# Muennighoff/sgpt

Measured on AMD Instinct MI355X. Metric: encoded sentences/sec (SGPT-125M, seq_len 128, encode + weighted-mean pool + cosine top-10 chunk loop), higher is better.
Workload: dtype f16

## Files before the change

### __graft_entry__.py

```python
import os
import sys

ROOT = os.path.dirname(os.path.abspath(__file__))
if ROOT not in sys.path:
    sys.path.insert(0, ROOT)


def build() -> None:
    from sgpt_amd import build as b
    lib = b.build(force=os.environ.get("SGPT_FORCE_BUILD") == "1", verbose=True)
    assert os.path.exists(lib)
    import sgpt_amd
    from sgpt_amd import _lib
    _lib.load()
    print("built", lib)


def smoke() -> None:
    import numpy as np
    import torch
    assert torch.cuda.is_available(), "smoke() needs cuda:0"
    from oracle import sgpt_oracle as O
    from sgpt_amd import SGPTConfig, SGPTModel, get_context
    kw = dict(vocab_size=211, max_position_embeddings=96, hidden_size=128, num_layers=4, num_heads=2, window_size=8)
    cfg = O.NeoConfig(**kw)
    w = O.synth_weights(cfg, seed=11, std=0.08)
    rng = np.random.default_rng(0)
    seqs = [rng.integers(0, 211, size=int(n)).tolist() for n in (5, 33, 1, 40, 17, 16)]
    want = O.encode(w, cfg, seqs, mode="weightedmean", batch_size=len(seqs))
    for dtype, tol in (("fp32", 1e-3), ("f16", 6e-3), ("bf16", 3.5e-2), ("f16x3", 1e-4)):
        m = (SGPTModel(SGPTConfig(**kw), w, device="cuda:0", dtype="f16", precision="x3") if dtype == "f16x3"
             else SGPTModel(SGPTConfig(**kw), w, device="cuda:0", dtype=dtype))
        got = m.encode_ids(seqs, mode="weightedmean").cpu().numpy()
        err = float(np.abs(got - want).max())
        print(f"smoke encode[{dtype}]: max|emb - oracle| = {err:.3e} (tol {tol:g})")
        assert np.isfinite(got).all() and err < tol
        m.close()
    kw7 = dict(vocab_size=211, max_position_embeddings=96, hidden_size=768, num_layers=2, num_heads=12, window_size=8)
    cfg7 = O.NeoConfig(**kw7)
    w7 = O.synth_weights(cfg7, seed=12, std=0.03)
    m7 = SGPTModel(SGPTConfig(**kw7), w7, device="cuda:0", dtype="f16")
    for qs in ([rng.integers(0, 211, size=18).tolist()], [rng.integers(0, 211, size=int(n)).tolist() for n in (7, 30, 12)]):
        want7 = O.encode(w7, cfg7, qs, mode="weightedmean", batch_size=len(qs), normalize_embeddings=True)
        pb = m7.pack(qs)
        got7 = m7.encode_packed(pb, normalize=True)
        old_policy = m7.ctx.set_tile_policy(2)
        try:
            bulk7 = m7.encode_packed(pb, normalize=True)
        finally:
            m7.ctx.set_tile_policy(old_policy)
        err = float(np.abs(got7.cpu().numpy() - want7).max())
        print(f"smoke query path[f16, {len(qs)} quer{'y' if len(qs) == 1 else 'ies'}, {pb.T_pad} token rows]: max|emb - oracle| = {err:.3e} (tol 1e-3), "
              f"identical to the bulk kernels: {bool(torch.equal(got7, bulk7))}")
        assert pb.T_pad % 32 == 0 and pb.T_pad <= 64 and err < 1e-3 and torch.equal(got7, bulk7)
    m7.close()
    ctx = get_context("cuda:0")
    q = rng.standard_normal((5, 128)).astype(np.float32)
    c = rng.standard_normal((300, 128)).astype(np.float32)
    val, idx, n = ctx.score_topk(ctx.l2_normalize(torch.from_numpy(q)), ctx.l2_normalize(torch.from_numpy(c)), 4)
    ov, oi = O.topk_rows(O.cos_sim(q, c), 4)
    assert n == 4 and np.array_equal(idx.cpu().numpy(), oi) and np.abs(val.cpu().numpy() - ov).max() < 1e-5
    v16, i16, _ = ctx.score_topk(ctx.l2_normalize(torch.from_numpy(q)), ctx.l2_normalize(torch.from_numpy(c)), 4, dtype=torch.float16)
    assert np.abs(v16.cpu().numpy() - ov).max() < 1e-3
    print("smoke score_topk: ok (fp32 exact ids; f16 scores within 1e-3)")


if __name__ == "__main__":
    build()
    if "--smoke" in sys.argv:
        smoke()
```

### include/sgpt_hip.h

```cpp
#ifndef SGPT_HIP_H
#define SGPT_HIP_H

#include <stddef.h>
#include <stdint.h>

#ifdef __cplusplus
extern "C" {
#endif

#define SGPT_ABI_VERSION 19

typedef int sgpt_status;
#define SGPT_OK 0
#define SGPT_ERR_INVALID (-1)
#define SGPT_ERR_HIP (-2)
#define SGPT_ERR_MISSING (-3)
#define SGPT_ERR_OOM (-4)
#define SGPT_ERR_COMM (-6)
#define SGPT_ERR_RANGE (-5)

typedef struct sgpt_ctx sgpt_ctx;
typedef struct sgpt_model sgpt_model;

enum { SGPT_F32 = 0, SGPT_BF16 = 1, SGPT_FP8W = 2, SGPT_F16 = 3, SGPT_FP8M = 4 };
enum { SGPT_ARCH_GPTNEO = 0, SGPT_ARCH_GPTJ = 1, SGPT_ARCH_BLOOM = 2, SGPT_ARCH_BERT = 3, SGPT_ARCH_LLAMA = 4 };
enum { SGPT_POOL_WEIGHTEDMEAN = 0, SGPT_POOL_MEAN = 1, SGPT_POOL_LASTTOKEN = 2, SGPT_POOL_LEARNTMEAN = 3,
       SGPT_POOL_CLS = 4 };
enum { SGPT_COS = 0, SGPT_DOT = 1, SGPT_NEG_L2 = 2 };

typedef struct {
    int32_t arch;
    int32_t n_layers;
    int32_t d_model;
    int32_t n_heads;
    int32_t d_ffn;
    int32_t vocab;
    int32_t max_pos;
    int32_t window;
    float ln_eps;
    float attn_scale;
    int32_t compute_dtype;
    const uint8_t* layer_is_local;
    int32_t rotary_dim;
    int32_t qk_split;
    int32_t split_weights;
    int32_t n_kv_heads;
} sgpt_model_desc;

typedef struct {
    const char* name;
    const float* ptr;
    int64_t numel;
} sgpt_tensor_view;

int sgpt_abi_version(void);
sgpt_status sgpt_ctx_create(int hip_device, sgpt_ctx** out);
void sgpt_ctx_destroy(sgpt_ctx* ctx);
const char* sgpt_last_error(const sgpt_ctx* ctx);

sgpt_status sgpt_model_load(sgpt_ctx* ctx, const sgpt_model_desc* desc,
                            const sgpt_tensor_view* tensors, size_t n_tensors, sgpt_model** out);
void sgpt_model_free(sgpt_model* model);

sgpt_status sgpt_model_calibrate_begin(sgpt_model* model);
sgpt_status sgpt_model_calibrate_end(sgpt_model* model, float margin, float* scales_out);
sgpt_status sgpt_model_set_act_scales(sgpt_model* model, const float* scales, int32_t n_scales);

sgpt_status sgpt_encode(sgpt_model* model, const int32_t* ids, const int32_t* pos,
                        const int32_t* seq_off, const int32_t* seq_len, const int32_t* pad_left,
                        int32_t B, int32_t T_pad, int32_t max_alloc_len,
                        int32_t pool_mode, int32_t n_layers_run, int32_t apply_final_ln,
                        int32_t normalize, float* out, float* hidden_out, void* stream);

sgpt_status sgpt_encode_layers(sgpt_model* model, const int32_t* ids, const int32_t* pos,
                               const int32_t* seq_off, const int32_t* seq_len, const int32_t* pad_left,
                               int32_t B, int32_t T_pad, int32_t max_alloc_len, int32_t pool_mode,
                               int32_t normalize, float* out_layers, float* out_mean, void* stream);

sgpt_status sgpt_model_set_pool_weights(sgpt_model* model, const float* weights, int32_t n);

sgpt_status sgpt_lm_logprobs(sgpt_model* model, const float* hidden, const int32_t* row_idx, const int32_t* targets,
                             int32_t n, float* out_logprob, int32_t* out_greedy, void* stream);

sgpt_status sgpt_pool(sgpt_ctx* ctx, const void* hidden, int32_t hidden_dtype, const int32_t* mask,
                      int32_t B, int32_t S, int32_t d, int32_t pool_mode, float* out, void* stream);
sgpt_status sgpt_pool_learnt(sgpt_ctx* ctx, const void* hidden, int32_t hidden_dtype, const int32_t* mask,
                             int32_t B, int32_t S, int32_t d, const float* pos_weights, float* out, void* stream);

sgpt_status sgpt_l2_normalize(sgpt_ctx* ctx, const float* in, int64_t n, int32_t d,
                              void* out, int32_t out_dtype, void* stream);

sgpt_status sgpt_pairwise_scores(sgpt_ctx* ctx, const float* a, const float* b, int64_t n, int32_t d, int32_t cosine,
                                 float* out, void* stream);
// ... 82 lines not shown
#define SGPT_EVAL_MAX_CUTS 16
sgpt_status sgpt_eval_ranked(sgpt_ctx* ctx, const int64_t* idx, const float* val, int32_t nq, int32_t K,
                             const int32_t* qrel_off, const int64_t* qrel_pos, const int32_t* qrel_rel,
                             const int32_t* ideal_rel, const int32_t* k_values, int32_t nk, int32_t check_order,
                             int32_t* out_hits, int32_t* out_first, float* out_dcg, float* out_idcg, float* out_sp,
                             int32_t* out_R, void* stream);

#define SGPT_EVAL_MAX_GROUP 1024
sgpt_status sgpt_eval_groups(sgpt_ctx* ctx, const float* emb, int32_t n_rows, int32_t d, int32_t mode, const float* scores_in,
                             int32_t G, const int32_t* grp_off, int32_t n_cand, int32_t max_group, const int32_t* q_row,
                             const int32_t* cand_row, const int32_t* cand_rel, const int32_t* R_extra,
                             const int32_t* ideal_off, const int32_t* ideal_rel, int32_t n_ideal, float* out_scores,
                             int32_t* out_order, int32_t* out_hits1, int32_t* out_hits5, int32_t* out_first, int32_t* out_R, float* out_sp,
                             float* out_dcg, float* out_idcg, void* stream);

#define SGPT_EVAL_MAX_PAIRS (1 << 24)
sgpt_status sgpt_eval_pairs(sgpt_ctx* ctx, const float* score, const int32_t* label, int32_t n, int32_t check_nan,
                            int32_t* out_rank2, int64_t* out_n_pos, int64_t* out_n_used, double* out_ap_num, void* stream);

sgpt_status sgpt_linear(sgpt_ctx* ctx, int32_t dtype, int32_t epi, int32_t out_dtype, const void* A, const void* W,
                        const float* bias, const float* resid, void* out, int32_t M, int32_t N, int32_t K, void* stream);

sgpt_status sgpt_linear_query(sgpt_ctx* ctx, int32_t dtype, int32_t epi, const void* A, const float* x, const float* ln_gamma,
                              const float* ln_beta, float ln_eps, const void* W, const float* bias, const float* resid, void* out,
                              void* out_vt, int32_t n_split, int32_t M, int32_t N, int32_t K, void* stream);

sgpt_status sgpt_linear_qkv(sgpt_ctx* ctx, int32_t dtype, const void* A, const void* W, void* out, void* out_vt, int32_t n_split,
                            int32_t M, int32_t N, int32_t K, void* stream);

sgpt_status sgpt_attention(sgpt_ctx* ctx, int32_t dtype, const void* q, const void* k, const void* v, int64_t ldq, int64_t ldvt,
                           void* out, int64_t ldo, const int32_t* seq_off, int32_t B, int32_t T, int32_t H, int32_t dh,
                           int32_t window, float scale, const float* alibi, int32_t max_alloc_len, int32_t out_fp8,
                           float out_scale, int32_t* range_flag, int32_t x3, int64_t qk_lo_delta, int64_t v_lo_delta,
                           int64_t ctx_lo_delta, int64_t ctx_hi2_delta, void* stream);

sgpt_status sgpt_attention_ex(sgpt_ctx* ctx, int32_t dtype, const void* q, const void* k, const void* v, int64_t ldq, int64_t ldvt,
                              void* out, int64_t ldo, const int32_t* seq_off, int32_t B, int32_t T, int32_t H, int32_t dh,
                              int32_t window, float scale, const float* alibi, int32_t max_alloc_len, int32_t out_fp8,
                              float out_scale, int32_t* range_flag, int32_t x3, int64_t qk_lo_delta, int64_t v_lo_delta,
                              int64_t ctx_lo_delta, int64_t ctx_hi2_delta, int32_t causal, const int32_t* seq_len, void* stream);

sgpt_status sgpt_attention_gqa(sgpt_ctx* ctx, int32_t dtype, const void* q, const void* k, const void* v, int64_t ldq, int64_t ldvt,
                               void* out, int64_t ldo, const int32_t* seq_off, int32_t B, int32_t T, int32_t H, int32_t n_kv_heads,
                               int32_t dh, int32_t window, float scale, const float* alibi, int32_t max_alloc_len, int32_t out_fp8,
                               float out_scale, int32_t* range_flag, int32_t x3, int64_t qk_lo_delta, int64_t v_lo_delta,
                               int64_t ctx_lo_delta, int64_t ctx_hi2_delta, void* stream);

sgpt_status sgpt_embed(sgpt_ctx* ctx, const int32_t* ids, const int32_t* pos, const float* wte, const float* wpe, int32_t T,
                       int32_t d, int32_t vocab, int32_t max_pos, float* out, void* stream);
sgpt_status sgpt_layernorm(sgpt_ctx* ctx, const float* x, const float* gamma, const float* beta, int32_t T, int32_t d, float eps,
                           void* out, int32_t out_dtype, float out_mul, int32_t split, void* stream);
sgpt_status sgpt_layernorm_writeback(sgpt_ctx* ctx, float* x, const float* gamma, const float* beta, int32_t T, int32_t d, float eps,
                                     void* out16, int32_t out_dtype, void* stream);
sgpt_status sgpt_rmsnorm(sgpt_ctx* ctx, const float* x, const float* gamma, int32_t T, int32_t d, float eps, void* out, int32_t out_dtype,
                         void* stream);
sgpt_status sgpt_swiglu(sgpt_ctx* ctx, const void* gu, int32_t dtype, int32_t T, int32_t ffn, void* out, void* stream);
sgpt_status sgpt_rope_half(sgpt_ctx* ctx, void* buf, int32_t dtype, int64_t ld, int64_t k_off, const int32_t* pos, const float* sin_t,
                           const float* cos_t, int32_t T, int32_t H, int32_t H_kv, int32_t head_dim, int32_t max_pos, void* stream);
sgpt_status sgpt_qknorm_rope_half(sgpt_ctx* ctx, void* buf, int32_t dtype, int64_t ld, int64_t k_off, const int32_t* pos,
                                  const float* sin_t, const float* cos_t, int32_t T, int32_t H, int32_t H_kv, int32_t head_dim,
                                  int32_t max_pos, const float* q_gamma, const float* k_gamma, float eps, void* stream);
sgpt_status sgpt_lnf_pool_ex(sgpt_ctx* ctx, const float* x, const float* gamma, const float* beta, const int32_t* seq_off,
                             const int32_t* seq_len, const int32_t* pad_left, int32_t B, int32_t d, float eps, int32_t apply_ln,
                             int32_t mode, int32_t normalize, const float* pos_weights, int32_t n_weights, float* out,
                             int32_t* nonfinite_flag, int32_t norm_kind, void* stream);
sgpt_status sgpt_lnf_pool(sgpt_ctx* ctx, const float* x, const float* gamma, const float* beta, const int32_t* seq_off,
                          const int32_t* seq_len, const int32_t* pad_left, int32_t B, int32_t d, float eps, int32_t apply_ln,
                          int32_t mode, int32_t normalize, const float* pos_weights, int32_t n_weights, float* out,
                          int32_t* nonfinite_flag, void* stream);
sgpt_status sgpt_rope(sgpt_ctx* ctx, void* buf, int32_t dtype, int64_t ld, int64_t k_off, const int32_t* pos, const float* sin,
                      const float* cos, int32_t T, int32_t H, int32_t head_dim, int32_t rotary_dim, int32_t max_pos, void* stream);
sgpt_status sgpt_logprob_rows(sgpt_ctx* ctx, const float* logits, int64_t ld, int32_t V, const int32_t* targets, int32_t n,
                              float* out_logprob, int32_t* out_greedy, void* stream);

sgpt_status sgpt_layernorm_fp8(sgpt_ctx* ctx, const float* x, const float* gamma, const float* beta, int32_t T, int32_t d,
                               float eps, uint8_t* codes, float* row_scale, void* stream);
sgpt_status sgpt_linear_fp8(sgpt_ctx* ctx, int32_t epi, int32_t out_dtype, const uint8_t* A, const float* a_scale,
                            float a_scalar, const uint8_t* W, const float* w_scale, const float* bias, const float* resid,
                            void* out, float out_scale, int32_t M, int32_t N, int32_t K, void* stream);

sgpt_status sgpt_prof_enable(sgpt_ctx* ctx, int32_t on);
sgpt_status sgpt_prof_read(sgpt_ctx* ctx, int64_t* launches, double* ms, double* flops, int32_t reset);

int32_t sgpt_ctx_set_gemm_cu_cap(sgpt_ctx* ctx, int32_t n);
int32_t sgpt_ctx_set_low_latency(sgpt_ctx* ctx, int32_t on);
int32_t sgpt_ctx_set_tile_policy(sgpt_ctx* ctx, int32_t policy);
int32_t sgpt_ctx_set_query_tile(sgpt_ctx* ctx, int32_t k);

sgpt_status sgpt_bench_gemm(sgpt_ctx* ctx, int32_t dtype, int32_t epi, int32_t out_dtype,
                            int32_t M, int32_t N, int32_t K, int32_t iters, float* ms_out);

#ifdef __cplusplus
}
#endif
#endif
```

### sgpt_amd/_lib.py

```python
import ctypes as C
import os

HERE = os.path.dirname(os.path.abspath(__file__))
LIB_PATH = os.environ.get("SGPT_HIP_LIB") or os.path.join(HERE, "lib", "libsgpt_hip.so")

SGPT_F32, SGPT_BF16, SGPT_FP8W, SGPT_F16, SGPT_FP8M = 0, 1, 2, 3, 4
SGPT_ABI_VERSION = 19
SGPT_PREC_CLASSES = 5
PC_LN1, PC_ATT, PC_CTX, PC_LN2, PC_H = 0, 1, 2, 3, 4
SGPT_ERR_RANGE = -5
SGPT_ERR_COMM = -6
SGPT_COMM_ID_BYTES = 128
SGPT_EVAL_MAX_CUTS = 16
SGPT_EVAL_MAX_GROUP = 1024
SGPT_EVAL_MAX_PAIRS = 1 << 24
SGPT_COS, SGPT_DOT, SGPT_NEG_L2 = 0, 1, 2
SGPT_ARCH_GPTNEO, SGPT_ARCH_GPTJ, SGPT_ARCH_BLOOM, SGPT_ARCH_BERT, SGPT_ARCH_LLAMA = 0, 1, 2, 3, 4
POOL_MODES = {"weightedmean": 0, "mean": 1, "lasttoken": 2, "learntmean": 3, "cls": 4}
EPI_BIAS_GELU_ERF = 9


class ModelDesc(C.Structure):
    _fields_ = [("arch", C.c_int32), ("n_layers", C.c_int32), ("d_model", C.c_int32), ("n_heads", C.c_int32),
                ("d_ffn", C.c_int32), ("vocab", C.c_int32), ("max_pos", C.c_int32), ("window", C.c_int32),
                ("ln_eps", C.c_float), ("attn_scale", C.c_float), ("compute_dtype", C.c_int32),
                ("layer_is_local", C.POINTER(C.c_uint8)), ("rotary_dim", C.c_int32), ("qk_split", C.c_int32),
                ("split_weights", C.c_int32), ("n_kv_heads", C.c_int32)]


class TensorView(C.Structure):
    _fields_ = [("name", C.c_char_p), ("ptr", C.c_void_p), ("numel", C.c_int64)]


SIGNATURES = {
    "sgpt_abi_version": (C.c_int, []),
    "sgpt_ctx_create": (C.c_int, [C.c_int, C.POINTER(C.c_void_p)]),
    "sgpt_ctx_destroy": (None, [C.c_void_p]),
    "sgpt_last_error": (C.c_char_p, [C.c_void_p]),
    "sgpt_model_load": (C.c_int, [C.c_void_p, C.POINTER(ModelDesc), C.POINTER(TensorView), C.c_size_t,
                                  C.POINTER(C.c_void_p)]),
    "sgpt_model_free": (None, [C.c_void_p]),
    "sgpt_encode": (C.c_int, [C.c_void_p, C.c_void_p, C.c_void_p, C.c_void_p, C.c_void_p, C.c_void_p,
                              C.c_int32, C.c_int32, C.c_int32, C.c_int32, C.c_int32, C.c_int32, C.c_int32,
                              C.c_void_p, C.c_void_p, C.c_void_p]),
    "sgpt_encode_layers": (C.c_int, [C.c_void_p, C.c_void_p, C.c_void_p, C.c_void_p, C.c_void_p, C.c_void_p,
                                     C.c_int32, C.c_int32, C.c_int32, C.c_int32, C.c_int32, C.c_void_p, C.c_void_p,
                                     C.c_void_p]),
    "sgpt_model_set_pool_weights": (C.c_int, [C.c_void_p, C.c_void_p, C.c_int32]),
    "sgpt_pool_learnt": (C.c_int, [C.c_void_p, C.c_void_p, C.c_int32, C.c_void_p, C.c_int32, C.c_int32, C.c_int32,
                                   C.c_void_p, C.c_void_p, C.c_void_p]),
    "sgpt_fp8_quantize_rows": (C.c_int, [C.c_void_p, C.c_void_p, C.c_int64, C.c_int64, C.c_void_p, C.c_void_p,
                                         C.c_void_p]),
    "sgpt_fp8_dequantize_rows": (C.c_int, [C.c_void_p, C.c_void_p, C.c_void_p, C.c_int64, C.c_int64, C.c_void_p,
                                           C.c_int32, C.c_void_p]),
    "sgpt_lm_logprobs": (C.c_int, [C.c_void_p, C.c_void_p, C.c_void_p, C.c_void_p, C.c_int32, C.c_void_p, C.c_void_p,
                                   C.c_void_p]),
    "sgpt_pool": (C.c_int, [C.c_void_p, C.c_void_p, C.c_int32, C.c_void_p, C.c_int32, C.c_int32, C.c_int32,
                            C.c_int32, C.c_void_p, C.c_void_p]),
    "sgpt_l2_normalize": (C.c_int, [C.c_void_p, C.c_void_p, C.c_int64, C.c_int32, C.c_void_p, C.c_int32, C.c_void_p]),
    "sgpt_pairwise_scores": (C.c_int, [C.c_void_p, C.c_void_p, C.c_void_p, C.c_int64, C.c_int32, C.c_int32, C.c_void_p, C.c_void_p]),
    "sgpt_f32_to_bf16": (C.c_int, [C.c_void_p, C.c_void_p, C.c_int64, C.c_void_p, C.c_void_p]),
    "sgpt_f32_to_16": (C.c_int, [C.c_void_p, C.c_void_p, C.c_int64, C.c_void_p, C.c_int32, C.c_void_p]),
    "sgpt_range_check": (C.c_int, [C.c_void_p, C.POINTER(C.c_int32), C.c_int32, C.c_void_p]),
    "sgpt_ctx_generation": (C.c_uint64, [C.c_void_p]),
    "sgpt_ctx_reserve": (C.c_int, [C.c_void_p, C.c_size_t, C.c_size_t]),
    "sgpt_scores": (C.c_int, [C.c_void_p, C.c_void_p, C.c_void_p, C.c_int32, C.c_int64, C.c_int64, C.c_int32,
                              C.c_void_p, C.c_int64, C.c_void_p]),
    "sgpt_score_topk": (C.c_int, [C.c_void_p, C.c_void_p, C.c_void_p, C.c_int32, C.c_int32, C.c_int64, C.c_int32,
                                  C.c_int32, C.c_int64, C.c_void_p, C.c_void_p, C.c_int32, C.POINTER(C.c_int32),
                                  C.c_void_p]),
    "sgpt_score_topk_q8": (C.c_int, [C.c_void_p, C.c_void_p, C.c_void_p, C.c_void_p, C.c_int32, C.c_int64, C.c_int32,
                                     C.c_int32, C.c_int64, C.c_void_p, C.c_void_p, C.c_int32, C.POINTER(C.c_int32),
                                     C.c_void_p]),
    "sgpt_pack_sign_bits": (C.c_int, [C.c_void_p, C.c_void_p, C.c_int64, C.c_int32, C.c_void_p, C.c_void_p, C.c_int64, C.c_void_p]),
    "sgpt_score_topk_bits": (C.c_int, [C.c_void_p, C.c_void_p, C.c_void_p, C.c_int64, C.c_int32, C.c_int64, C.c_int32, C.c_int32,
                                       C.c_int32, C.c_int32, C.c_void_p, C.c_void_p, C.c_int64, C.c_void_p, C.c_void_p, C.c_int32,
                                       C.POINTER(C.c_int32), C.c_void_p]),
    "sgpt_score_overflow_count": (C.c_int, [C.c_void_p, C.POINTER(C.c_int32), C.POINTER(C.c_int32), C.c_void_p]),
    "sgpt_score_topk_refined": (C.c_int, [C.c_void_p, C.c_void_p, C.c_void_p, C.c_void_p, C.c_int32, C.c_int32, C.c_int64, C.c_int32,
                                           C.c_int32, C.c_int64, C.c_float, C.c_void_p, C.c_void_p, C.c_int32, C.c_void_p, C.c_void_p,
                                           C.c_void_p]),
    "sgpt_topk_merge": (C.c_int, [C.c_void_p, C.c_void_p, C.c_void_p, C.c_int32, C.c_int32, C.c_int32, C.c_void_p,
                                  C.c_void_p, C.c_void_p, C.c_void_p]),
    "sgpt_topk": (C.c_int, [C.c_void_p, C.c_void_p, C.c_int32, C.c_int64, C.c_int64, C.c_int32, C.c_int64,
                            C.c_void_p, C.c_void_p, C.c_void_p]),
    "sgpt_eval_ranked": (C.c_int, [C.c_void_p, C.c_void_p, C.c_void_p, C.c_int32, C.c_int32, C.c_void_p, C.c_void_p, C.c_void_p,
                                   C.c_void_p, C.POINTER(C.c_int32), C.c_int32, C.c_int32, C.c_void_p, C.c_void_p, C.c_void_p,
                                   C.c_void_p, C.c_void_p, C.c_void_p, C.c_void_p]),
    "sgpt_eval_groups": (C.c_int, [C.c_void_p, C.c_void_p, C.c_int32, C.c_int32, C.c_int32, C.c_void_p, C.c_int32, C.c_void_p, C.c_int32,
                                   C.c_int32, C.c_void_p, C.c_void_p, C.c_void_p, C.c_void_p, C.c_void_p, C.c_void_p, C.c_int32,
                                   C.c_void_p, C.c_void_p, C.c_void_p, C.c_void_p, C.c_void_p, C.c_void_p, C.c_void_p, C.c_void_p,
                                   C.c_void_p, C.c_void_p]),
    "sgpt_eval_pairs": (C.c_int, [C.c_void_p, C.c_void_p, C.c_void_p, C.c_int32, C.c_int32, C.c_void_p, C.c_void_p, C.c_void_p,
                                  C.c_void_p, C.c_void_p]),
    "sgpt_linear": (C.c_int, [C.c_void_p, C.c_int32, C.c_int32, C.c_int32, C.c_void_p, C.c_void_p, C.c_void_p, C.c_void_p,
                              C.c_void_p, C.c_int32, C.c_int32, C.c_int32, C.c_void_p]),
    "sgpt_linear_query": (C.c_int, [C.c_void_p, C.c_int32, C.c_int32, C.c_void_p, C.c_void_p, C.c_void_p, C.c_void_p, C.c_float, C.c_void_p,
                                    C.c_void_p, C.c_void_p, C.c_void_p, C.c_void_p, C.c_int32, C.c_int32, C.c_int32, C.c_int32, C.c_void_p]),
    "sgpt_linear_qkv": (C.c_int, [C.c_void_p, C.c_int32, C.c_void_p, C.c_void_p, C.c_void_p, C.c_void_p, C.c_int32, C.c_int32, C.c_int32,
                                  C.c_int32, C.c_void_p]),
    "sgpt_model_calibrate_begin": (C.c_int, [C.c_void_p]),
    "sgpt_model_calibrate_end": (C.c_int, [C.c_void_p, C.c_float, C.c_void_p]),
    "sgpt_model_set_act_scales": (C.c_int, [C.c_void_p, C.c_void_p, C.c_int32]),
    "sgpt_layernorm_fp8": (C.c_int, [C.c_void_p, C.c_void_p, C.c_void_p, C.c_void_p, C.c_int32, C.c_int32, C.c_float, C.c_void_p,
                                     C.c_void_p, C.c_void_p]),
    "sgpt_linear_fp8": (C.c_int, [C.c_void_p, C.c_int32, C.c_int32, C.c_void_p, C.c_void_p, C.c_float, C.c_void_p, C.c_void_p,
                                  C.c_void_p, C.c_void_p, C.c_void_p, C.c_float, C.c_int32, C.c_int32, C.c_int32, C.c_void_p]),
    "sgpt_comm_unique_id": (C.c_int, [C.c_void_p]),
    "sgpt_comm_init": (C.c_int, [C.c_void_p, C.c_void_p, C.c_int32, C.c_int32]),
    "sgpt_comm_destroy": (C.c_int, [C.c_void_p]),
    "sgpt_comm_world": (C.c_int32, [C.c_void_p]),
    "sgpt_comm_rank": (C.c_int32, [C.c_void_p]),
    "sgpt_allgather_rows": (C.c_int, [C.c_void_p, C.c_void_p, C.c_void_p, C.c_int64, C.c_void_p, C.c_void_p]),
    "sgpt_allgather_rows_padded": (C.c_int, [C.c_void_p, C.c_void_p, C.c_void_p, C.c_int64, C.c_void_p, C.c_void_p]),
    "sgpt_exchange_topk": (C.c_int, [C.c_void_p, C.c_void_p, C.c_void_p, C.c_int32, C.c_int32, C.c_int32, C.c_void_p,
                                     C.c_void_p, C.c_void_p, C.c_void_p]),
    "sgpt_fold_gathered_topk": (C.c_int, [C.c_void_p, C.c_void_p, C.c_void_p, C.c_int32, C.c_int32, C.c_int32, C.c_int32,
                                          C.c_void_p, C.c_void_p, C.c_void_p, C.c_void_p]),
    "sgpt_ctx_set_low_latency": (C.c_int32, [C.c_void_p, C.c_int32]),
    "sgpt_ctx_set_tile_policy": (C.c_int32, [C.c_void_p, C.c_int32]),
    "sgpt_ctx_set_gemm_cu_cap": (C.c_int32, [C.c_void_p, C.c_int32]),
    "sgpt_ctx_set_query_tile": (C.c_int32, [C.c_void_p, C.c_int32]),
    "sgpt_model_range_check": (C.c_int, [C.c_void_p, C.POINTER(C.c_int32), C.c_int32, C.c_void_p]),
    "sgpt_model_range_adapt": (C.c_int, [C.c_void_p, C.POINTER(C.c_int32), C.c_void_p]),
    "sgpt_model_get_range_shifts": (C.c_int, [C.c_void_p, C.c_void_p, C.c_int32]),
    "sgpt_model_set_range_shifts": (C.c_int, [C.c_void_p, C.c_void_p, C.c_int32]),
    "sgpt_model_set_precision": (C.c_int, [C.c_void_p, C.c_void_p, C.c_int32]),
    "sgpt_model_get_precision": (C.c_int, [C.c_void_p, C.c_void_p, C.c_int32]),
    "sgpt_model_release_split_weights": (C.c_int, [C.c_void_p, C.c_void_p]),
    "sgpt_model_precision_probe_begin": (C.c_int, [C.c_void_p]),
    "sgpt_model_precision_probe_end": (C.c_int, [C.c_void_p, C.c_void_p]),
    "sgpt_row_crest": (C.c_int, [C.c_void_p, C.c_void_p, C.c_int32, C.c_int64, C.c_int32, C.c_int64, C.POINTER(C.c_float), C.c_void_p]),
    "sgpt_split16": (C.c_int, [C.c_void_p, C.c_void_p, C.c_int64, C.c_int32, C.c_int32, C.c_void_p, C.c_int32, C.c_void_p]),
    "sgpt_linear_split": (C.c_int, [C.c_void_p, C.c_int32, C.c_int32, C.c_void_p, C.c_void_p, C.c_void_p, C.c_void_p,
                                    C.c_int64, C.c_int64, C.c_int64, C.c_int32, C.c_int32, C.c_int32, C.c_void_p]),
    "sgpt_attention": (C.c_int, [C.c_void_p, C.c_int32, C.c_void_p, C.c_void_p, C.c_void_p, C.c_int64, C.c_int64,
                                 C.c_void_p, C.c_int64, C.c_void_p, C.c_int32, C.c_int32, C.c_int32, C.c_int32,
                                 C.c_int32, C.c_float, C.c_void_p, C.c_int32, C.c_int32,
                                 C.c_float, C.c_void_p, C.c_int32, C.c_int64, C.c_int64,
                                 C.c_int64, C.c_int64, C.c_void_p]),
    "sgpt_attention_ex": (C.c_int, [C.c_void_p, C.c_int32, C.c_void_p, C.c_void_p, C.c_void_p, C.c_int64, C.c_int64,
                                    C.c_void_p, C.c_int64, C.c_void_p, C.c_int32, C.c_int32, C.c_int32, C.c_int32,
                                    C.c_int32, C.c_float, C.c_void_p, C.c_int32, C.c_int32,
                                    C.c_float, C.c_void_p, C.c_int32, C.c_int64, C.c_int64,
                                    C.c_int64, C.c_int64, C.c_int32, C.c_void_p, C.c_void_p]),
    "sgpt_attention_gqa": (C.c_int, [C.c_void_p, C.c_int32, C.c_void_p, C.c_void_p, C.c_void_p, C.c_int64, C.c_int64,
                                     C.c_void_p, C.c_int64, C.c_void_p, C.c_int32, C.c_int32, C.c_int32, C.c_int32, C.c_int32,
                                     C.c_int32, C.c_float, C.c_void_p, C.c_int32, C.c_int32,
                                     C.c_float, C.c_void_p, C.c_int32, C.c_int64, C.c_int64,
                                     C.c_int64, C.c_int64, C.c_void_p]),
    "sgpt_rmsnorm": (C.c_int, [C.c_void_p, C.c_void_p, C.c_void_p, C.c_int32, C.c_int32, C.c_float, C.c_void_p, C.c_int32, C.c_void_p]),
    "sgpt_swiglu": (C.c_int, [C.c_void_p, C.c_void_p, C.c_int32, C.c_int32, C.c_int32, C.c_void_p, C.c_void_p]),
    "sgpt_rope_half": (C.c_int, [C.c_void_p, C.c_void_p, C.c_int32, C.c_int64, C.c_int64, C.c_void_p, C.c_void_p, C.c_void_p,
                                 C.c_int32, C.c_int32, C.c_int32, C.c_int32, C.c_int32, C.c_void_p]),
    "sgpt_qknorm_rope_half": (C.c_int, [C.c_void_p, C.c_void_p, C.c_int32, C.c_int64, C.c_int64, C.c_void_p, C.c_void_p, C.c_void_p,
                                        C.c_int32, C.c_int32, C.c_int32, C.c_int32, C.c_int32, C.c_void_p, C.c_void_p, C.c_float,
                                        C.c_void_p]),
    "sgpt_lnf_pool_ex": (C.c_int, [C.c_void_p, C.c_void_p, C.c_void_p, C.c_void_p, C.c_void_p, C.c_void_p, C.c_void_p, C.c_int32,
                                   C.c_int32, C.c_float, C.c_int32, C.c_int32, C.c_int32, C.c_void_p, C.c_int32, C.c_void_p,
                                   C.c_void_p, C.c_int32, C.c_void_p]),
    "sgpt_layernorm_writeback": (C.c_int, [C.c_void_p, C.c_void_p, C.c_void_p, C.c_void_p, C.c_int32, C.c_int32, C.c_float, C.c_void_p,
                                           C.c_int32, C.c_void_p]),
    "sgpt_embed": (C.c_int, [C.c_void_p, C.c_void_p, C.c_void_p, C.c_void_p, C.c_void_p, C.c_int32, C.c_int32, C.c_int32, C.c_int32,
                             C.c_void_p, C.c_void_p]),
    "sgpt_layernorm": (C.c_int, [C.c_void_p, C.c_void_p, C.c_void_p, C.c_void_p, C.c_int32, C.c_int32, C.c_float, C.c_void_p,
                                 C.c_int32, C.c_float, C.c_int32, C.c_void_p]),
    "sgpt_lnf_pool": (C.c_int, [C.c_void_p, C.c_void_p, C.c_void_p, C.c_void_p, C.c_void_p, C.c_void_p, C.c_void_p, C.c_int32,
                                C.c_int32, C.c_float, C.c_int32, C.c_int32, C.c_int32, C.c_void_p, C.c_int32, C.c_void_p,
                                C.c_void_p, C.c_void_p]),
    "sgpt_rope": (C.c_int, [C.c_void_p, C.c_void_p, C.c_int32, C.c_int64, C.c_int64, C.c_void_p, C.c_void_p, C.c_void_p,
                            C.c_int32, C.c_int32, C.c_int32, C.c_int32, C.c_int32, C.c_void_p]),
    "sgpt_logprob_rows": (C.c_int, [C.c_void_p, C.c_void_p, C.c_int64, C.c_int32, C.c_void_p, C.c_int32, C.c_void_p, C.c_void_p,
                                    C.c_void_p]),
    "sgpt_bench_gemm": (C.c_int, [C.c_void_p, C.c_int32, C.c_int32, C.c_int32, C.c_int32, C.c_int32, C.c_int32,
                                  C.c_int32, C.POINTER(C.c_float)]),
    "sgpt_prof_enable": (C.c_int, [C.c_void_p, C.c_int32]),
    "sgpt_prof_read": (C.c_int, [C.c_void_p, C.POINTER(C.c_int64), C.POINTER(C.c_double), C.POINTER(C.c_double),
                                 C.c_int32]),
}

_lib = None


class SgptHipError(RuntimeError):
    pass


class SgptRangeError(SgptHipError):
    """dtype='f16': a weight is outside the IEEE-half range, or an activation class is beyond every power-of-two range
    shift (use dtype='bf16'); dtype='fp8mfma': an e4m3 code saturated (re-calibrate)."""

EXPERIMENT_SIGNATURES = {
    "sgpt_exp_set_gemm_skew": (C.c_int32, [C.c_int32]),
    "sgpt_exp_set_gemm_w": (C.c_int32, [C.c_int32]),
}


def load():
    global _lib
    if _lib is not None:
        return _lib
    if not os.path.exists(LIB_PATH):
        raise SgptHipError(f"{LIB_PATH} is missing: build it with `python -m sgpt_amd.build` "
                           "(hipcc --offload-arch=gfx950); there is no CPU/PyTorch fallback")
    lib = C.CDLL(LIB_PATH)
# ... 26 lines not shown
```

### sgpt_amd/beir.py

```python
import logging
import os
import pathlib
import pickle
from concurrent.futures import ThreadPoolExecutor
from typing import Dict, List, Optional, Tuple, Union

import numpy as np
import torch

from .model import SGPTModel
from .runtime import get_context
from .families import family_of
from .tokenization import TextPipeline, load_tokenizer

logger = logging.getLogger(__name__)

SCORE_SPLIT_CREST = 10.0
SINGLE_LAYER_METHODS = ("mean", "weightedmean", "lasttoken", "cls")
ALL_LAYER_METHODS = {"meanmean": "mean", "lasttokenmean": "lasttoken"}


class CustomEmbedder:

    def __init__(self, model_name="EleutherAI/gpt-neo-1.3B", batch_size=250, device="cuda:0", save_emb=False,
# ... 17 lines not shown
        self.base_path = f"embeddings/{model_name.split('/')[-1]}/{self.method}/{dataset}"
        if save_emb:
            pathlib.Path(self.base_path).parent.mkdir(parents=True, exist_ok=True)

    def tokenize(self, sentences: List[str], is_query: bool) -> List[List[int]]:
        before = (self.pipe.docs_truncated, self.pipe.toks_truncated)
        seqs = self.pipe.batch(sentences, is_query)
        if self.pipe.docs_truncated > before[0]:
            logging.warning(f"Truncated {self.pipe.docs_truncated - before[0]} out of {len(sentences)} documents "
                            f"by {self.pipe.toks_truncated - before[1]} tokens.")
        return seqs

    def tokenize_corpus(self, corpus) -> List[List[int]]:
        return self.tokenize([t for (_, t) in self._corpus_texts(corpus)], False)

    def embed_device(self, sentences: List[str], is_query: bool, normalize: bool = False) -> torch.Tensor:
        return self.embed_ids_device(self.tokenize(sentences, is_query), normalize=normalize)

    def embed_ids_device(self, seqs: List[List[int]], normalize: bool = False) -> torch.Tensor:
        L = self.model.cfg.num_layers
        if abs(self.layeridx) > L + 1:
            raise ValueError(f"Layer Idx {self.layeridx} is larger than the {L + 1} hidden states")
        if self.method in SINGLE_LAYER_METHODS:
            return self.model.encode_ids(seqs, mode=self.method, normalize=normalize, layer_idx=self.layeridx)
        acc = self.model.encode_ids_all_layers(seqs, mode=ALL_LAYER_METHODS[self.method])
        return get_context(self.model.device).l2_normalize(acc) if normalize else acc

    def embed_batcher(self, texts: List[Tuple[int, str]], is_query, out_name=None, **kwargs) -> Dict:
        ids, sentences = zip(*texts)
        emb = self.embed_device(list(sentences), is_query).cpu().numpy()
        all_embeddings = {i: e for i, e in zip(ids, emb)}
        assert len(texts) == len(all_embeddings)
        if self.save_emb:
            pickle.dump(all_embeddings, open(out_name, "wb"))
        return all_embeddings

    def encode_queries(self, queries: List[Tuple[str, str]], batch_size: int = None, **kwargs) -> np.ndarray:
        path = f"{self.base_path}_queries.pickle"
        if os.path.exists(path):
            embeddings = pickle.load(open(path, "rb"))
        else:
            embeddings = self.embed_batcher(texts=queries, out_name=path, is_query=True, **kwargs)
        embeddings = np.array([embeddings[i] for (i, _) in queries])
        logger.info(f"Produced embeddings of shape {embeddings.shape}")
        return embeddings

    @staticmethod
    def _corpus_texts(corpus):
        return [(i, (d["title"] + " " + d["text"]).strip() if "title" in d else d["text"].strip()) for (i, d) in corpus]

    def encode_corpus(self, corpus: List[Tuple[str, Dict[str, str]]], batch_size: int = None, batch_num="",
                      **kwargs) -> np.ndarray:
        path = f"{self.base_path}_corpus{batch_num}.pickle"
        if os.path.exists(path):
            embeddings = pickle.load(open(path, "rb"))
        else:
            embeddings = self.embed_batcher(texts=self._corpus_texts(corpus), out_name=path, is_query=False, **kwargs)
        embeddings = np.array([embeddings[i] for (i, _) in corpus])
        logger.info(f"Produced embeddings of shape {embeddings.shape}")
        return embeddings

    def encode_queries_device(self, queries, normalize=False, use_cache=True):
        if use_cache and (os.path.exists(f"{self.base_path}_queries.pickle") or self.save_emb):
            emb = torch.from_numpy(self.encode_queries(queries)).to(self.model.device)
            return get_context(self.model.device).l2_normalize(emb) if normalize else emb
        return self.embed_device([q for (_, q) in queries], True, normalize=normalize)

    def uses_embedding_cache(self, batch_num="") -> bool:
        return os.path.exists(f"{self.base_path}_corpus{batch_num}.pickle") or self.save_emb

    def encode_corpus_device(self, corpus, batch_num="", normalize=False, seqs=None):
        if self.uses_embedding_cache(batch_num):
            emb = torch.from_numpy(self.encode_corpus(corpus, batch_num=batch_num)).to(self.model.device)
            return get_context(self.model.device).l2_normalize(emb) if normalize else emb
        if seqs is None:
            seqs = self.tokenize_corpus(corpus)
        return self.embed_ids_device(seqs, normalize=normalize)


class DenseRetrievalExactSearch:

    def __init__(self, model, batch_size: int = 128, corpus_chunk_size: int = 50000, score_dtype=torch.float32,
                 prefetch_tokenize: bool = True, ctx=None, group=None, distributed: Optional[bool] = None,
                 score_split: Optional[bool] = None, exact_scorer: str = "brute", **kwargs):
        self.model = model
        self.prefetch_tokenize = prefetch_tokenize
        self.batch_size = batch_size
        self.score_function_desc = {"cos_sim": "Cosine Similarity", "dot": "Dot Product"}
        self.corpus_chunk_size = corpus_chunk_size
        self.show_progress_bar = True
        self.convert_to_tensor = True
        self.score_dtype = score_dtype
        if exact_scorer not in ("refined", "brute"):
            raise ValueError("exact_scorer must be 'refined' or 'brute'")
        self.exact_scorer = exact_scorer
        self.ctx = ctx
        self.group = group
        self.distributed = distributed
        self.score_split = score_split
        self.last_score_split = False
        self.results = {}
        self.last_shard = None

    def _to_dev(self, ctx, x):
        if not isinstance(x, torch.Tensor):
            x = torch.as_tensor(np.asarray(x))
        return x.to(device=ctx.device, dtype=torch.float32)

    def _encode_queries(self, ctx, qlist, use_cache=True):
        if not qlist:
            return None
        if hasattr(self.model, "encode_queries_device"):
            q_emb = self.model.encode_queries_device(qlist, use_cache=use_cache)
        else:
            q_emb = self.model.encode_queries(qlist, batch_size=self.batch_size,
                                              show_progress_bar=self.show_progress_bar,
                                              convert_to_tensor=self.convert_to_tensor)
        return self._to_dev(ctx, q_emb)

    def search(self, corpus: Dict[str, Dict[str, str]], queries: Dict[str, str], top_k: int, score_function: str,
               return_sorted: bool = False, **kwargs) -> Dict[str, Dict[str, float]]:
        self.results = {qid: {} for qid in queries}
        ranked = self.search_ranked(corpus, queries, top_k, score_function, **kwargs)
        if ranked.val.shape[1] > 0:
            self.results = assemble_results(ranked.query_ids, ranked.corpus_ids, ranked.val.cpu().numpy(), ranked.idx.cpu().numpy())
        return self.results

    def search_ranked(self, corpus: Dict[str, Dict[str, str]], queries: Dict[str, str], top_k: int, score_function: str,
                      **kwargs):
        if score_function not in self.score_function_desc:
            raise ValueError(
                "score function: {} must be either (cos_sim) for cosine similarity or (dot) for dot product".format(
                    score_function))
        from .dist import balanced_cuts, get_comm, is_distributed
        ctx = self.ctx if self.ctx is not None else get_context(getattr(getattr(self.model, "model", None), "device", None))
        import torch.distributed as tdist
        sharded = is_distributed(self.group) if self.distributed is None else (
            bool(self.distributed) and tdist.is_available() and tdist.is_initialized())
        comm = get_comm(ctx, self.group) if sharded else None
        world, rank = (comm.world, comm.rank) if comm is not None else (1, 0)

        logger.info("Encoding Queries...")
        query_ids = list(queries.keys())
        nq = len(query_ids)
        qlist = [(qid, queries[qid]) for qid in queries]
        sgpt = getattr(self.model, "model", None)
        if comm is not None and hasattr(sgpt, "sync_precision") and hasattr(self.model, "tokenize") and qlist:
            from .dist import max_reducer
            own = qlist[rank::world][:64] or qlist[:64]
            sgpt.sync_precision(self.model.tokenize([q for (_, q) in own], True), max_reducer(ctx, self.group))
        if getattr(sgpt, "precision_report", None):
            rep = sgpt.precision_report
            logger.info("Encoder precision: %s (%s; %d operand classes flagged)", rep["decided"], rep["probed"], rep["flagged"])
        if comm is not None and (nq >= 4 * world or world == 1):
            qcuts = balanced_cuts([len(q[1]) + 1 for q in qlist], world, min_one=True)
            q_loc = self._encode_queries(ctx, qlist[qcuts[rank]: qcuts[rank + 1]], use_cache=False)
            q_emb = comm.all_gather_rows(q_loc, np.diff(qcuts).tolist())
        else:
            q_emb = self._encode_queries(ctx, qlist)
        if score_function == "cos_sim":
            q_emb = ctx.l2_normalize(q_emb)
        split = False
        if self.score_dtype in (torch.float16, torch.bfloat16) and score_function == "cos_sim" and hasattr(ctx, "split16"):
            split = (ctx.row_crest(q_emb) > SCORE_SPLIT_CREST) if self.score_split is None else bool(self.score_split)
        self.last_score_split = split
        q_op = ctx.split16(q_emb, "query", self.score_dtype) if split else q_emb

        logger.info("Sorting Corpus by document length (Longest first)...")
        doc_len = {k: len(corpus[k].get("title", "") + corpus[k].get("text", "")) for k in corpus}
        corpus_ids = sorted(corpus, key=doc_len.__getitem__, reverse=True)
        pos_of = {cid: i for i, cid in enumerate(corpus_ids)}
        self_idx = torch.tensor([pos_of.get(qid, -1) for qid in query_ids], dtype=torch.int64, device=ctx.device)
        if comm is not None:
            ccuts = balanced_cuts([doc_len[c] + 1 for c in corpus_ids], world)
            lo, hi = int(ccuts[rank]), int(ccuts[rank + 1])
        else:
            lo, hi = 0, len(corpus_ids)
        self.last_shard = (rank, world, lo, hi)
        clist = [(cid, corpus[cid]) for cid in corpus_ids[lo:hi]]

        run_val = run_idx = None
        itr = range(0, len(clist), self.corpus_chunk_size)
        ahead = self.prefetch_tokenize and hasattr(self.model, "tokenize_corpus")
        pool = ThreadPoolExecutor(max_workers=1) if ahead else None
        fut = None
        tag = (lambda b: b) if comm is None else (lambda b: f"_r{rank}of{world}_{b}")

        def tokens_for(batch_num, start):
            if not ahead or self.model.uses_embedding_cache(tag(batch_num)) or start >= len(clist):
                return None
            return pool.submit(self.model.tokenize_corpus, clist[start: start + self.corpus_chunk_size])
        try:
            fut = tokens_for(0, 0)
            for batch_num, start in enumerate(itr):
                logger.info("Encoding Batch {}/{}...".format(batch_num + 1, len(itr)))
                end = min(start + self.corpus_chunk_size, len(clist))
                if ahead:
                    seqs = fut.result() if fut is not None else None
                    fut = tokens_for(batch_num + 1, end)
                    sub = self.model.encode_corpus_device(clist[start:end], batch_num=tag(batch_num), seqs=seqs)
                elif hasattr(self.model, "encode_corpus_device"):
                    sub = self.model.encode_corpus_device(clist[start:end], batch_num=tag(batch_num))
                else:
                    sub = self.model.encode_corpus(clist[start:end], batch_size=self.batch_size,
                                                   show_progress_bar=self.show_progress_bar,
                                                   convert_to_tensor=self.convert_to_tensor, batch_num=tag(batch_num))
                sub = self._to_dev(ctx, sub)
                kk = min(top_k + 1, end - start)
                refined = (self.score_dtype == torch.float32 and self.exact_scorer == "refined" and score_function == "cos_sim"
                           and hasattr(ctx, "score_topk_refined") and sub.shape[1] % 8 == 0)
                if score_function == "cos_sim":
                    sub = (ctx.split16(ctx.l2_normalize(sub), "doc", self.score_dtype) if split
                           else ctx.l2_normalize(sub, out_dtype=self.score_dtype))
                if refined:
                    val, idx, _ = ctx.score_topk_refined(q_op, sub, None, kk, idx_base=lo + start)
                else:
                    val, idx, _ = ctx.score_topk(q_op, sub, kk, idx_base=lo + start, dtype=self.score_dtype)
                if run_val is None:
                    cand_v, cand_i = val, idx
                else:
                    cand_v, cand_i = torch.cat([run_val, val], dim=1), torch.cat([run_idx, idx], dim=1)
                keep = min(top_k + 1, cand_v.shape[1])
                run_val, run_idx = ctx.topk_merge(cand_v, cand_i, keep, exclude_idx=self_idx)
        finally:
            if pool is not None:
                if fut is not None:
                    fut.cancel()
                pool.shutdown(wait=True)

        if comm is not None:
            k1 = top_k + 1
            pv = torch.full((nq, k1), float("-inf"), dtype=torch.float32, device=ctx.device)
            pi = torch.full((nq, k1), -1, dtype=torch.int64, device=ctx.device)
            if run_val is not None:
                pv[:, : run_val.shape[1]] = run_val
                pi[:, : run_idx.shape[1]] = run_idx
            run_val, run_idx = comm.exchange_topk(pv, pi, min(k1, len(corpus_ids)), exclude_idx=self_idx)
        if run_val is None:
            run_val = torch.empty((nq, 0), dtype=torch.float32, device=ctx.device)
            run_idx = torch.empty((nq, 0), dtype=torch.int64, device=ctx.device)
        from .evaluation import RankedLists
        return RankedLists(query_ids, corpus_ids, run_val, run_idx, pos_of)


def _host_ext():
    global _HOST_EXT
    if _HOST_EXT is None:
        _HOST_EXT = False
        path = os.path.join(os.path.dirname(os.path.abspath(__file__)), "lib", "_sgpt_host.so")
        if os.path.exists(path):
            import importlib.util
            try:
                spec = importlib.util.spec_from_file_location("_sgpt_host", path)
                mod = importlib.util.module_from_spec(spec)
                spec.loader.exec_module(mod)
                _HOST_EXT = mod
            except Exception as e:
                logger.warning("host extension %s not loadable (%s): result dicts are assembled in Python", path, e)
    return _HOST_EXT or None


_HOST_EXT = None


def assemble_results(query_ids, corpus_ids, vals: np.ndarray, idxs: np.ndarray, native: Optional[bool] = None) -> Dict[str, Dict[str, float]]:
    ext = _host_ext() if native in (None, True) else None
    if native is True and ext is None:
        raise RuntimeError("assemble_results(native=True): sgpt_amd/lib/_sgpt_host.so is not built (python -m sgpt_amd.build)")
    if ext is not None and len(query_ids) > 0:
        qs = query_ids if isinstance(query_ids, list) else list(query_ids)
        cs = corpus_ids if isinstance(corpus_ids, list) else list(corpus_ids)
        return ext.assemble(qs, cs, np.ascontiguousarray(vals, dtype=np.float32), np.ascontiguousarray(idxs, dtype=np.int64))
    cid = np.asarray(corpus_ids, dtype=object)
    ok_all = idxs >= 0
    full = bool(ok_all.all())
    out = {}
    for qi, qid in enumerate(query_ids):
        if full:
            out[qid] = dict(zip(cid[idxs[qi]].tolist(), vals[qi].tolist()))
        else:
            ok = ok_all[qi]
            out[qid] = dict(zip(cid[idxs[qi][ok]].tolist(), vals[qi][ok].tolist()))
    return out


class SentenceBERTBOSEOS:

    def __init__(self, model_path=None, sep: str = " ", speca=False, specb=False, model: Optional[SGPTModel] = None,
                 tokenizer=None, max_seq_length: int = 300, method: str = "weightedmean", dtype="f16",
                 device="cuda:0", frame=None, **kwargs):
        self.sep = sep
        self.speca, self.specb = speca, specb
        if not (specb or speca):
            raise NameError("name 'sentences' is not defined")
        self.model = model if model is not None else SGPTModel.from_pretrained(model_path, device=device, dtype=dtype)
        tok = tokenizer if tokenizer is not None else load_tokenizer(model_path)
        self.pipe = TextPipeline(tok, max_seq_length, specb=specb and not speca, speca=speca, st_path=True,
                                 family=family_of(self.model), frame=frame)
        if speca and max(self.pipe.bos_q + self.pipe.eos_q + self.pipe.bos_d + self.pipe.eos_d) >= self.model.cfg.vocab_size:
            raise ValueError("speca: the checkpoint's embedding table has no rows for the added [SOS]/[EOS]/{SOS}/{EOS} ids")
# ... 54 lines not shown
```

### sgpt_amd/csrc/common.h

```cpp
#pragma once
#include <hip/hip_runtime.h>
#include <stdint.h>

typedef uint16_t bf16_t;
struct f16_t { uint16_t bits; };
typedef __attribute__((ext_vector_type(8))) __bf16 bf16x8;
typedef __attribute__((ext_vector_type(8))) _Float16 f16x8;
typedef __attribute__((ext_vector_type(4))) float f32x4;
typedef __attribute__((ext_vector_type(16))) float f32x16;

constexpr int DT_F32 = 0, DT_BF16 = 1, DT_FP8W = 2, DT_F16 = 3;
__host__ __device__ constexpr bool dt_is16(int dt) { return dt == DT_BF16 || dt == DT_F16; }

#define WAVE 64

typedef uint2 __attribute__((may_alias)) uint2_a;
typedef uint4 __attribute__((may_alias)) uint4_a;
typedef float4 __attribute__((may_alias)) float4_a;

__device__ __forceinline__ float bf16_to_f32(bf16_t v) { return __uint_as_float(((uint32_t)v) << 16); }

typedef __attribute__((ext_vector_type(2))) __bf16 bf16x2_t;
typedef __attribute__((ext_vector_type(2))) float f32x2_t;
__device__ __forceinline__ uint32_t pack_bf16x2(float lo, float hi) {
// ... 252 lines not shown
bool score64q8_shape_ok(int M, long N, int K, const void* codes, long ldw);
void launch_score64q8(int epi, const Score8Args& a, hipStream_t s);
void launch_scorebits(int epi, const GemmArgs& g, int d, int qw, long ldb, hipStream_t s, bool spread = false);
void launch_gemm256w(int dtype, int epi, const GemmArgs& a, hipStream_t s, bool deep_a);

struct AttnArgs {
    const void* q;
    const void* k;
    const void* v;
    void* ctx;
    const int* seq_off;
    int B, H, dh;
    long ldq, ldvt, ldo;
    int window;
    float scale;
    int max_alloc_len;
    const float* alibi;
    int dtype;
    int out_fp8;
    float out_scale;
    int* range_flag;
    int x3;
    long qk_lo_delta, v_lo_delta, ctx_lo_delta, ctx_hi2_delta;
    int noncausal;
    const int* seq_len;
    int kv_group = 1;
};
inline bool attn_x3_supported(int dh) { return dh == 64 || dh == 128; }
void launch_attn_bf16(const AttnArgs& a, hipStream_t s);
void launch_attn_f32(const AttnArgs& a, hipStream_t s);

void launch_embed(const int* ids, const int* pos, const float* wte, const float* wpe, float* x, int T, int d, int vocab,
                  int max_pos, hipStream_t s);
void launch_layernorm(const float* x, const float* g, const float* b, void* out, int out_dtype, int T, int d,
                      float eps, hipStream_t s, float out_mul = 1.0f);
void launch_layernorm_writeback(float* x, const float* g, const float* b, void* out16, int out_dtype, int T, int d, float eps,
                                int* range_flag, hipStream_t s);
void launch_layernorm_split(const float* x, const float* g, const float* b, void* out, int out_dtype, int T, int d,
                            float eps, hipStream_t s, float out_mul);
void launch_rmsnorm(const float* x, const float* g, void* out, int out_dtype, int T, int d, float eps, int* range_flag, hipStream_t s);
void launch_swiglu(const void* gu, void* h, int dtype, int T, int ffn, int* range_flag, hipStream_t s);
void launch_pack_split_rows(const float* src, long rows, long cols, void* dst, int out_dtype, hipStream_t s);
void launch_crest16(const void* in, int T, int cols, long ld, int dtype, unsigned* out_bits, hipStream_t s);
void launch_split16_rows(const float* in, long n, int d, int layout, void* out, int out_dtype, hipStream_t s);
void launch_layernorm_q8(const float* x, const float* g, const float* b, void* q, float* scale, void* out16, int out16_dtype,
                         int T, int d, float eps, hipStream_t s);
void launch_absmax16(const void* in, long numel, int dtype, unsigned* out_bits, hipStream_t s);
void launch_lnf_pool(const float* x, const float* g, const float* b, const int* seq_off, const int* seq_len,
                     const int* pad_left, int B, int d, float eps, int apply_ln, int mode, int normalize,
                     const float* pos_weights, int pos_weights_n, float* out, hipStream_t s,
                     int* nonfinite_flag = nullptr,
                     int norm_kind = 0);
void launch_pool(const void* hidden, int dtype, const int* mask, int B, int S, int d, int mode,
                 const float* pos_weights, float* out, hipStream_t s);
void launch_fp8_quant_rows(const float* w, long rows, long cols, void* q, float* scale, hipStream_t s);
void launch_fp8_dequant_rows(const void* q, const float* scale, long rows, long cols, void* out, int out_dtype,
                             hipStream_t s);
void launch_l2norm(const float* in, long n, int d, void* out, int out_dtype, hipStream_t s);
void launch_pack_sign_bits(const float* x, long n, int d, const float* center, uint8_t* bits, long ldb, hipStream_t s);
void launch_pairwise(const float* a, const float* b, long n, int d, bool cosine, float* out, hipStream_t s);
void launch_gather_rows(const float* src, const int* row_idx, int n, int d, float* dst, hipStream_t s);
void launch_logprob_rows(const float* logits, long ld, int V, const int* targets, int n, float* out_lp, int* out_arg,
                         hipStream_t s);
void launch_mean_over_axis0(const float* in, int n0, long n, float* out, hipStream_t s);
void launch_f32_to_bf16(const float* in, long numel, void* out, hipStream_t s);
void launch_f32_to_16(const float* in, long numel, void* out, int out_dtype, hipStream_t s);
void launch_absmax(const float* in, long numel, unsigned* out_bits, hipStream_t s);
void launch_fill_f32(float* p, long n, float v, hipStream_t s);
void launch_rope(void* qk, int dtype, long ld, long k_off, const int* pos, const float* sin_t, const float* cos_t, int T,
                 int H, int dh, int rotary_dim, int max_pos, hipStream_t s);
void launch_rope_half(void* qk, int dtype, long ld, long k_off, const int* pos, const float* sin_t, const float* cos_t, int T,
                      int H, int H_kv, int dh, int max_pos, hipStream_t s);
void launch_qknorm_rope_half(void* qk, int dtype, long ld, long k_off, const int* pos, const float* sin_t, const float* cos_t,
                             const float* q_g, const float* k_g, float eps, int T, int H, int H_kv, int dh, int max_pos, int* range_flag,
                             hipStream_t s);
void launch_qkv_deinterleave(const float* src, float* dst, int H, int dh, long row_len, hipStream_t s);
void launch_fill_rand(void* p, long n, int dtype, unsigned seed, float scale, hipStream_t s);

void launch_topk_select(const float* scores, long ld, long n, long idx_base, const float* prev_val,
                        const int64_t* prev_idx, int n_prev, long prev_ld, int nq, int k, int nan_to_m1,
                        const int64_t* exclude_idx, float* out_val, int64_t* out_idx, hipStream_t s,
                        const int* pred = nullptr, float* thr_out = nullptr,
                        int gather_k = 0);
void launch_rescore(const float* q, const float* corpus, const int64_t* idx, long ld_idx, int nq, int m, int d, long idx_base,
                    long n_docs, float* out_val, int64_t* out_idx, long ld_out, hipStream_t s);
void launch_rescore_bits(int mode, const float* q, const uint8_t* bits, long ldb, const uint8_t* codes, long ld8, const float* scale,
                         const float* val1, const int64_t* idx, long ld_idx, int nq, int m, int d, long idx_base, long n_docs,
                         float* out_val, int64_t* out_idx, long ld_out, hipStream_t s);
void launch_refine_check(const float* v16, int k, int kp, float margin, int nq, int* flag, hipStream_t s);
void launch_list_append(const float* in_val, const int64_t* in_idx, long ld_in, int n_run, int nq, float* out_val, int64_t* out_idx,
                        long ld_out, int col0, hipStream_t s);
void launch_score_prep(const void* q, void* qpad, long q_bytes, long qpad_bytes, int* counters, long n_counters, long long* idx_list,
                       long n_idx, hipStream_t s);
void launch_thr_below(const float* list, int k, int nq, float* thr, hipStream_t s);
void launch_cand_merge(const float* run_val, const int64_t* run_idx, const float* cand_val, const int64_t* cand_idx,
                       int* cand_cnt, int cap, int nq, int k, float* out_val, int64_t* out_idx, int* overflow,
                       hipStream_t s, float* thr_io = nullptr);
```

### sgpt_amd/csrc/ctx.h

```cpp
#pragma once
#include <hip/hip_runtime.h>

#include <string>
#include <utility>
#include <vector>

struct sgpt_ctx {
    int device = 0;
    std::string err;
    void* ws = nullptr; size_t ws_bytes = 0;
    void* ws2 = nullptr; size_t ws2_bytes = 0;
    void* ws3 = nullptr; size_t ws3_bytes = 0;
    void* ws4 = nullptr; size_t ws4_bytes = 0;
    void* ws5 = nullptr; size_t ws5_bytes = 0;
    void* ws6 = nullptr; size_t ws6_bytes = 0;
    size_t filt_flag_off = 0; int filt_chunks = 0;
    void* comm = nullptr;
    int comm_rank = 0, comm_world = 0;
    uint64_t generation = 0;
    int* range_flag = nullptr;
    int kgroups = 1;
    int force256 = 0;
    int no_qpath = 0;
    int cu_cap = 0;
    int qtile = 0;
    bool prof = false;
    std::vector<std::pair<hipEvent_t, hipEvent_t>> ev_pool;
    size_t ev_used = 0;
    std::vector<double> ev_flops;
    int64_t prof_launches = 0; double prof_ms = 0, prof_flops = 0;
};
```

### sgpt_amd/csrc/ctx.hip

```cpp
#include "host.h"

namespace sgpt_host {

sgpt_status ensure(sgpt_ctx* c, void** p, size_t* have, size_t need) {
    if (*have >= need) return SGPT_OK;
    if (*p) { HIPC(c, hipDeviceSynchronize()); HIPC(c, hipFree(*p)); *p = nullptr; *have = 0; }
    need = align_up(need + (need >> 3), 1 << 20);
    if (hipMalloc(p, need) != hipSuccess) { *p = nullptr; return fail(c, SGPT_ERR_OOM, "hipMalloc workspace failed"); }
    HIPC(c, hipMemset(*p, 0, need));
    *have = need;
    c->generation++;
    return SGPT_OK;
}

void gemm(sgpt_ctx* c, int dtype, int epi, int out_dtype, const GemmArgs& a0, hipStream_t s) {
    Prof p(c, s, 2.0 * (double)a0.m_valid * a0.N * (a0.k_algo > 0 ? a0.k_algo : a0.K));
    GemmArgs a = a0;
    a.kgroups = c->kgroups; a.force256 = c->force256; a.cu_cap = c->cu_cap;
    launch_gemm(dtype, epi, out_dtype, a, s);
}

bool qgemm(sgpt_ctx* c, int dtype, int epi, int out_dtype, const QGemmArgs& a, hipStream_t s) {
    Prof p(c, s, 2.0 * (double)a.g.m_valid * a.g.N * a.g.K);
    return launch_qgemm(dtype, epi, out_dtype, a, s);
}

}

extern "C" {

int sgpt_abi_version(void) { return SGPT_ABI_VERSION; }

sgpt_status sgpt_ctx_create(int hip_device, sgpt_ctx** out) {
    if (!out) return SGPT_ERR_INVALID;
    *out = nullptr;
    int n = 0;
    if (hipGetDeviceCount(&n) != hipSuccess || hip_device < 0 || hip_device >= n) return SGPT_ERR_HIP;
    if (hipSetDevice(hip_device) != hipSuccess) return SGPT_ERR_HIP;
    sgpt_ctx* c = new sgpt_ctx();
    c->device = hip_device;
    if (hipMalloc((void**)&c->range_flag, 256) != hipSuccess || hipMemset(c->range_flag, 0, 256) != hipSuccess) {
        delete c;
        return SGPT_ERR_OOM;
    }
    *out = c;
    return SGPT_OK;
}

void sgpt_ctx_destroy(sgpt_ctx* c) {
    if (!c) return;
    (void)hipSetDevice(c->device);
    (void)hipDeviceSynchronize();
    if (c->ws) (void)hipFree(c->ws);
    if (c->ws2) (void)hipFree(c->ws2);
    (void)sgpt_comm_destroy(c);
    if (c->ws3) (void)hipFree(c->ws3);
    if (c->ws4) (void)hipFree(c->ws4);
    if (c->ws5) (void)hipFree(c->ws5);
    if (c->ws6) (void)hipFree(c->ws6);
    if (c->range_flag) (void)hipFree(c->range_flag);
    for (auto& e : c->ev_pool) { (void)hipEventDestroy(e.first); (void)hipEventDestroy(e.second); }
    delete c;
}

const char* sgpt_last_error(const sgpt_ctx* c) { return c ? c->err.c_str() : "null ctx"; }

uint64_t sgpt_ctx_generation(const sgpt_ctx* c) { return c ? c->generation : 0; }

sgpt_status sgpt_ctx_reserve(sgpt_ctx* c, size_t encode_bytes, size_t score_bytes) {
    if (!c) return SGPT_ERR_INVALID;
    HIPC(c, hipSetDevice(c->device));
    sgpt_status st = ensure(c, &c->ws, &c->ws_bytes, encode_bytes);
    if (st != SGPT_OK) return st;
    return ensure(c, &c->ws2, &c->ws2_bytes, score_bytes);
}

sgpt_status sgpt_range_check(sgpt_ctx* c, int32_t* flagged, int32_t reset, void* stream) {
    if (!c || !flagged) return SGPT_ERR_INVALID;
    HIPC(c, hipSetDevice(c->device));
    hipStream_t s = (hipStream_t)stream;
    int h = 0;
    HIPC(c, hipMemcpyAsync(&h, c->range_flag, sizeof(int), hipMemcpyDeviceToHost, s));
    HIPC(c, hipStreamSynchronize(s));
    if (reset && h) HIPC(c, hipMemsetAsync(c->range_flag, 0, sizeof(int), s));
    *flagged = h;
    return SGPT_OK;
}

sgpt_status sgpt_prof_enable(sgpt_ctx* c, int32_t on) {
    if (!c) return SGPT_ERR_INVALID;
    c->prof = on != 0;
    return SGPT_OK;
}

sgpt_status sgpt_prof_read(sgpt_ctx* c, int64_t* launches, double* ms, double* flops, int32_t reset) {
    if (!c) return SGPT_ERR_INVALID;
    HIPC(c, hipSetDevice(c->device));
    HIPC(c, hipDeviceSynchronize());
    for (size_t i = 0; i < c->ev_used; ++i) {
        float t = 0;
        HIPC(c, hipEventElapsedTime(&t, c->ev_pool[i].first, c->ev_pool[i].second));
        c->prof_ms += t;
        c->prof_flops += c->ev_flops[i];
        c->prof_launches++;
    }
    c->ev_used = 0;
    if (launches) *launches = c->prof_launches;
    if (ms) *ms = c->prof_ms;
    if (flops) *flops = c->prof_flops;
    if (reset) { c->prof_launches = 0; c->prof_ms = 0; c->prof_flops = 0; }
    return SGPT_OK;
}

int32_t sgpt_ctx_set_low_latency(sgpt_ctx* c, int32_t on) {
    if (!c) return 0;
    const int old = c->kgroups > 1 ? 1 : 0;
    c->kgroups = on ? 2 : 1;
    return old;
}
int32_t sgpt_ctx_set_gemm_cu_cap(sgpt_ctx* c, int32_t n) {
    if (!c) return 0;
    const int old = c->cu_cap;
    c->cu_cap = n > 0 ? n : 0;
    return old;
}
int32_t sgpt_ctx_set_tile_policy(sgpt_ctx* c, int32_t policy) {
    if (!c) return 0;
    const int old = c->force256 ? 1 : c->no_qpath ? 2 : 0;
    c->force256 = policy == 1 ? 1 : 0;
    c->no_qpath = policy == 2 ? 1 : 0;
    return old;
}
int32_t sgpt_ctx_set_query_tile(sgpt_ctx* c, int32_t k) {
    if (!c || k < 0 || k > 7) return -1;
    const int old = c->qtile;
    c->qtile = k;
    return old;
}
#ifdef SGPT_EXPERIMENTS
int32_t sgpt_exp_set_gemm_skew(int32_t cycles) { return set_gemm_skew(cycles); }
int32_t sgpt_exp_set_gemm_w(int32_t on) { return set_gemm_use_w(on); }
#endif

}
```

### sgpt_amd/csrc/elementwise.hip

```cpp
#include "common.h"
#include "rowln.h"


namespace {

__global__ __launch_bounds__(256) void embed_kernel(const int* __restrict__ ids, const int* __restrict__ pos,
                                                    const float* __restrict__ wte, const float* __restrict__ wpe,
                                                    float* __restrict__ x, int T, int d, int vocab, int max_pos) {
    const int row = blockIdx.x * 4 + (threadIdx.x >> 6);
    if (row >= T) return;
    const int lane = threadIdx.x & 63;
    int id = ids[row]; id = id < 0 ? 0 : (id >= vocab ? vocab - 1 : id);
    const float4* a = reinterpret_cast<const float4*>(wte + (long)id * d);
    float4* o = reinterpret_cast<float4*>(x + (long)row * d);
    if (wpe == nullptr) {
        for (int c = lane; c < d / 4; c += 64) o[c] = a[c];
        return;
    }
    int ps = pos[row]; ps = ps < 0 ? 0 : (ps >= max_pos ? max_pos - 1 : ps);
    const float4* b = reinterpret_cast<const float4*>(wpe + (long)ps * d);
    for (int c = lane; c < d / 4; c += 64) {
        const float4 u = a[c], v = b[c];
        o[c] = make_float4(u.x + v.x, u.y + v.y, u.z + v.z, u.w + v.w);
    }
// ... 492 lines not shown
__device__ __forceinline__ uint32_t e4m3fn_encode(float x) {
    const uint32_t sign = (__float_as_uint(x) >> 24) & 0x80u;
    const float a = fabsf(x);
    if (!(a < 464.f)) return sign | (a != a ? 0x7fu : 0x7eu);
    if (a < 0.015625f) return sign | (uint32_t)rintf(a * 512.f);
    uint32_t u = __float_as_uint(a);
    u += 0x7ffffu + ((u >> 20) & 1u);
    u >>= 20;
    const uint32_t code = u - (120u << 3);
    return sign | (code > 0x7eu ? 0x7eu : code);
}
__device__ __forceinline__ float e4m3fn_decode(uint32_t c) {
    const uint32_t e = (c >> 3) & 15u, m = c & 7u;
    const float a = e ? __uint_as_float(((e + 120u) << 23) | (m << 20)) : (float)m * 0.001953125f;
    if ((c & 0x7fu) == 0x7fu) return __uint_as_float(0x7fc00000u);
    return (c & 0x80u) ? -a : a;
}

__global__ __launch_bounds__(256) void fp8_quant_rows_kernel(const float* __restrict__ w, long rows, long cols,
                                                             uint8_t* __restrict__ q, float* __restrict__ scale) {
    const long row = (long)blockIdx.x * 4 + (threadIdx.x >> 6);
    if (row >= rows) return;
    const int lane = threadIdx.x & 63;
    const float* wr = w + row * cols;
    float amax = 0.f;
    for (long c = lane; c < cols; c += 64) amax = fmaxf(amax, fabsf(wr[c]));
#pragma unroll
    for (int off = 32; off > 0; off >>= 1) amax = fmaxf(amax, __shfl_xor(amax, off));
    float sc = 1.0f;
    if (amax > 0.f && amax < 3.0e38f) {
        const uint32_t u = __float_as_uint(amax);
        const int e = (int)((u >> 23) & 0xffu) - 127;
        const uint32_t frac = u & 0x7fffffu;
        int k = e - (frac > 0x600000u ? 7 : 8);
        k = k < -126 ? -126 : (k > 127 ? 127 : k);
        sc = __uint_as_float((uint32_t)(k + 127) << 23);
    }
    if (lane == 0) scale[row] = sc;
    const float inv = 1.0f / sc;
    for (long c = lane; c < cols; c += 64) q[row * cols + c] = (uint8_t)e4m3fn_encode(wr[c] * inv);
}

__global__ __launch_bounds__(256) void pack_sign_bits_kernel(const float* __restrict__ x, long n, int d, const float* __restrict__ center,
                                                             uint8_t* __restrict__ bits, long ldb) {
    const long total = n * ldb, stride = (long)gridDim.x * 256;
    for (long o = (long)blockIdx.x * 256 + threadIdx.x; o < total; o += stride) {
        const long r = o / ldb;
        const int i0 = (int)(o - r * ldb) * 8;
        const float* xr = x + r * d;
        uint32_t b = 0;
#pragma unroll
        for (int j = 0; j < 8; ++j) {
            const int i = i0 + j;
            if (i < d) {
                const float v = center ? xr[i] - center[i] : xr[i];
                const uint32_t u = __float_as_uint(v);
                b |= (u - 1u < 0x7f800000u ? 1u : 0u) << (7 - j);
            }
        }
        bits[o] = (uint8_t)b;
    }
}

template <typename OutT>
__global__ __launch_bounds__(256) void fp8_dequant_rows_kernel(const uint8_t* __restrict__ q, const float* __restrict__ scale,
                                                               long rows, long cols, OutT* __restrict__ out) {
    const long n4 = rows * cols / 4, stride = (long)gridDim.x * 256;
    for (long i = (long)blockIdx.x * 256 + threadIdx.x; i < n4; i += stride) {
        const uint32_t u = reinterpret_cast<const uint32_t*>(q)[i];
        const float sc = scale[i * 4 / cols];
        const float v0 = e4m3fn_decode(u & 0xffu) * sc, v1 = e4m3fn_decode((u >> 8) & 0xffu) * sc;
        const float v2 = e4m3fn_decode((u >> 16) & 0xffu) * sc, v3 = e4m3fn_decode(u >> 24) * sc;
        if constexpr (sizeof(OutT) == 4) reinterpret_cast<float4*>(out)[i] = make_float4(v0, v1, v2, v3);
        else reinterpret_cast<uint2*>(out)[i] = make_uint2(Half<OutT>::pack2(v0, v1), Half<OutT>::pack2(v2, v3));
    }
}

template <typename H>
__global__ __launch_bounds__(256) void cvt16_kernel(const float* __restrict__ in, long numel, uint16_t* __restrict__ out) {
    const long stride = (long)gridDim.x * 256;
    for (long i = (long)blockIdx.x * 256 + threadIdx.x; i < numel; i += stride) out[i] = f32_to_h<H>(in[i]);
}

__global__ __launch_bounds__(256) void absmax_kernel(const float* __restrict__ in, long numel, unsigned* __restrict__ out_bits) {
    const long stride = (long)gridDim.x * 256;
    unsigned m = 0;
    for (long i = (long)blockIdx.x * 256 + threadIdx.x; i < numel; i += stride) {
        const unsigned b = __float_as_uint(in[i]) & 0x7fffffffu;
        m = b > m ? b : m;
    }
#pragma unroll
    for (int o = 32; o > 0; o >>= 1) { const unsigned t = __shfl_xor(m, o, 64); m = t > m ? t : m; }
    if ((threadIdx.x & 63) == 0 && m) atomicMax(out_bits, m);
}

__global__ __launch_bounds__(256) void mean_axis0_kernel(const float* __restrict__ in, int n0, long n,
                                                         float* __restrict__ out) {
    const long i = (long)blockIdx.x * 256 + threadIdx.x;
    if (i >= n) return;
    float acc = 0.f;
    for (int j = 0; j < n0; ++j) acc += in[(long)j * n + i];
    out[i] = acc / (float)n0;
}

__global__ __launch_bounds__(256) void gather_rows_kernel(const float* __restrict__ src, const int* __restrict__ row_idx, int n,
                                                          int d, float* __restrict__ dst) {
    const int r = blockIdx.x * 4 + (threadIdx.x >> 6);
    if (r >= n) return;
    const int lane = threadIdx.x & 63;
    const float4* s4 = reinterpret_cast<const float4*>(src + (long)row_idx[r] * d);
    float4* d4 = reinterpret_cast<float4*>(dst + (long)r * d);
    for (int c = lane; c < d / 4; c += 64) d4[c] = s4[c];
}

__global__ __launch_bounds__(256) void logprob_rows_kernel(const float* __restrict__ logits, long ld, int V,
                                                           const int* __restrict__ targets, float* __restrict__ out_lp,
                                                           int* __restrict__ out_arg) {
    __shared__ float s_f[4];
    __shared__ int s_i[4];
    const int r = blockIdx.x, t = threadIdx.x, lane = t & 63, wave = t >> 6;
    const float* x = logits + (long)r * ld;
    float mx = -INFINITY;
    int am = 0x7fffffff;
    for (int i = t; i < V; i += 256) {
        const float v = x[i];
        if (v > mx || (v == mx && i < am)) { mx = v; am = i; }
    }
#pragma unroll
    for (int o = 32; o > 0; o >>= 1) {
        const float ov = __shfl_xor(mx, o, 64);
        const int oi = __shfl_xor(am, o, 64);
        if (ov > mx || (ov == mx && oi < am)) { mx = ov; am = oi; }
    }
    if (lane == 0) { s_f[wave] = mx; s_i[wave] = am; }
    __syncthreads();
    mx = s_f[0]; am = s_i[0];
#pragma unroll
    for (int w = 1; w < 4; ++w)
        if (s_f[w] > mx || (s_f[w] == mx && s_i[w] < am)) { mx = s_f[w]; am = s_i[w]; }
    __syncthreads();
    float sum = 0.f;
    for (int i = t; i < V; i += 256) sum += expf(x[i] - mx);
    sum = wave_sum(sum);
    if (lane == 0) s_f[wave] = sum;
    __syncthreads();
    if (t == 0) {
        const float tot = (s_f[0] + s_f[1]) + (s_f[2] + s_f[3]);
        int tg = targets[r]; tg = tg < 0 ? 0 : (tg >= V ? V - 1 : tg);
        out_lp[r] = (x[tg] - mx) - logf(tot);
        if (out_arg) out_arg[r] = am;
    }
}

__global__ __launch_bounds__(256) void fill_kernel(float* __restrict__ p, long n, float v) {
    const long stride = (long)gridDim.x * 256;
    for (long i = (long)blockIdx.x * 256 + threadIdx.x; i < n; i += stride) p[i] = v;
}

template <typename T>
__global__ __launch_bounds__(256) void fill_rand_kernel(T* __restrict__ p, long n, unsigned seed, float scale) {
    const long stride = (long)gridDim.x * 256;
    for (long i = (long)blockIdx.x * 256 + threadIdx.x; i < n; i += stride) {
        unsigned h = (unsigned)i * 2654435761u ^ seed;
        h ^= h >> 16; h *= 0x85ebca6bu; h ^= h >> 13; h *= 0xc2b2ae35u; h ^= h >> 16;
        const float v = ((float)(h >> 8) * (1.0f / 8388608.0f) - 1.0f) * scale;
        if constexpr (sizeof(T) == 4) p[i] = v; else reinterpret_cast<uint16_t*>(p)[i] = f32_to_h<T>(v);
// ... 182 lines not shown
#define LP_CASE(NV)                                                                                              \
    if (norm_kind == 1)                                                                                          \
        hipLaunchKernelGGL((lnf_pool_kernel<NV, true>), dim3(B), dim3(256), sm, s, x, g, b, seq_off, seq_len, pad_left, d, \
                           eps, apply_ln, mode, normalize, pos_weights, pos_weights_n, out, nonfinite_flag);     \
    else                                                                                                         \
    hipLaunchKernelGGL((lnf_pool_kernel<NV>), dim3(B), dim3(256), sm, s, x, g, b, seq_off, seq_len, pad_left, d, \
                       eps, apply_ln, mode, normalize, pos_weights, pos_weights_n, out, nonfinite_flag);
    const int nv = (d + 255) / 256;
    if (nv <= 1) { LP_CASE(1) } else if (nv <= 2) { LP_CASE(2) } else if (nv <= 3) { LP_CASE(3) }
    else if (nv <= 4) { LP_CASE(4) } else if (nv <= 8) { LP_CASE(8) } else if (nv <= 10) { LP_CASE(10) }
    else { LP_CASE(16) }
#undef LP_CASE
}

void launch_pool(const void* hidden, int dtype, const int* mask, int B, int S, int d, int mode,
                 const float* pos_weights, float* out, hipStream_t s) {
    dim3 grid(B, (d / 4 + 255) / 256);
    if (dtype == DT_BF16)
        hipLaunchKernelGGL(pool_kernel<bf16_t>, grid, dim3(256), 0, s, (const bf16_t*)hidden, mask, S, d, mode, pos_weights, out);
    else if (dtype == DT_F16)
        hipLaunchKernelGGL(pool_kernel<f16_t>, grid, dim3(256), 0, s, (const f16_t*)hidden, mask, S, d, mode, pos_weights, out);
    else
        hipLaunchKernelGGL(pool_kernel<float>, grid, dim3(256), 0, s, (const float*)hidden, mask, S, d, mode, pos_weights, out);
}

void launch_pack_sign_bits(const float* x, long n, int d, const float* center, uint8_t* bits, long ldb, hipStream_t s) {
    const long blocks = (n * ldb + 255) / 256;
    hipLaunchKernelGGL(pack_sign_bits_kernel, dim3((unsigned)(blocks < 1 ? 1 : (blocks > 65536 ? 65536 : blocks))), dim3(256), 0, s, x, n, d,
                       center, bits, ldb);
}

void launch_fp8_quant_rows(const float* w, long rows, long cols, void* q, float* scale, hipStream_t s) {
    hipLaunchKernelGGL(fp8_quant_rows_kernel, dim3((unsigned)((rows + 3) / 4)), dim3(256), 0, s, w, rows, cols,
                       (uint8_t*)q, scale);
}

void launch_fp8_dequant_rows(const void* q, const float* scale, long rows, long cols, void* out, int out_dtype,
                             hipStream_t s) {
    const int grid = cap_grid((rows * cols / 4 + 255) / 256);
    if (out_dtype == 1)
        hipLaunchKernelGGL(fp8_dequant_rows_kernel<bf16_t>, dim3(grid), dim3(256), 0, s, (const uint8_t*)q, scale, rows,
                           cols, (bf16_t*)out);
    else if (out_dtype == DT_F16)
        hipLaunchKernelGGL(fp8_dequant_rows_kernel<f16_t>, dim3(grid), dim3(256), 0, s, (const uint8_t*)q, scale, rows,
                           cols, (f16_t*)out);
    else
        hipLaunchKernelGGL(fp8_dequant_rows_kernel<float>, dim3(grid), dim3(256), 0, s, (const uint8_t*)q, scale, rows,
                           cols, (float*)out);
}

void launch_gather_rows(const float* src, const int* row_idx, int n, int d, float* dst, hipStream_t s) {
    hipLaunchKernelGGL(gather_rows_kernel, dim3((n + 3) / 4), dim3(256), 0, s, src, row_idx, n, d, dst);
}

void launch_logprob_rows(const float* logits, long ld, int V, const int* targets, int n, float* out_lp, int* out_arg,
                         hipStream_t s) {
    hipLaunchKernelGGL(logprob_rows_kernel, dim3(n), dim3(256), 0, s, logits, ld, V, targets, out_lp, out_arg);
}

void launch_mean_over_axis0(const float* in, int n0, long n, float* out, hipStream_t s) {
    hipLaunchKernelGGL(mean_axis0_kernel, dim3((unsigned)((n + 255) / 256)), dim3(256), 0, s, in, n0, n, out);
}

void launch_pairwise(const float* a, const float* b, long n, int d, bool cosine, float* out, hipStream_t s) {
    const unsigned grid = (unsigned)((n + 3) / 4);
    if (cosine) hipLaunchKernelGGL(pairwise_kernel<true>, dim3(grid), dim3(256), 0, s, a, b, n, d, out);
    else hipLaunchKernelGGL(pairwise_kernel<false>, dim3(grid), dim3(256), 0, s, a, b, n, d, out);
}

void launch_l2norm(const float* in, long n, int d, void* out, int out_dtype, hipStream_t s) {
    const int grid = (int)((n + 3) / 4);
    if (out_dtype == DT_BF16) hipLaunchKernelGGL(l2norm_kernel<bf16_t>, dim3(grid), dim3(256), 0, s, in, n, d, (bf16_t*)out);
    else if (out_dtype == DT_F16) hipLaunchKernelGGL(l2norm_kernel<f16_t>, dim3(grid), dim3(256), 0, s, in, n, d, (f16_t*)out);
    else hipLaunchKernelGGL(l2norm_kernel<float>, dim3(grid), dim3(256), 0, s, in, n, d, (float*)out);
}

void launch_f32_to_16(const float* in, long numel, void* out, int out_dtype, hipStream_t s) {
    const int grid = cap_grid((numel + 255) / 256);
    if (out_dtype == DT_F16) hipLaunchKernelGGL(cvt16_kernel<f16_t>, dim3(grid), dim3(256), 0, s, in, numel, (uint16_t*)out);
    else hipLaunchKernelGGL(cvt16_kernel<bf16_t>, dim3(grid), dim3(256), 0, s, in, numel, (uint16_t*)out);
}
void launch_f32_to_bf16(const float* in, long numel, void* out, hipStream_t s) { launch_f32_to_16(in, numel, out, DT_BF16, s); }

void launch_absmax(const float* in, long numel, unsigned* out_bits, hipStream_t s) {
    hipLaunchKernelGGL(absmax_kernel, dim3(cap_grid((numel + 255) / 256)), dim3(256), 0, s, in, numel, out_bits);
}

void launch_fill_f32(float* p, long n, float v, hipStream_t s) {
    hipLaunchKernelGGL(fill_kernel, dim3(cap_grid((n + 255) / 256)), dim3(256), 0, s, p, n, v);
}

void launch_fill_rand(void* p, long n, int dtype, unsigned seed, float scale, hipStream_t s) {
    if (dtype == DT_BF16)
        hipLaunchKernelGGL(fill_rand_kernel<bf16_t>, dim3(cap_grid((n + 255) / 256)), dim3(256), 0, s, (bf16_t*)p, n, seed, scale);
    else if (dtype == DT_F16)
        hipLaunchKernelGGL(fill_rand_kernel<f16_t>, dim3(cap_grid((n + 255) / 256)), dim3(256), 0, s, (f16_t*)p, n, seed, scale);
    else
        hipLaunchKernelGGL(fill_rand_kernel<float>, dim3(cap_grid((n + 255) / 256)), dim3(256), 0, s, (float*)p, n, seed, scale);
}

void launch_rope(void* qk, int dtype, long ld, long k_off, const int* pos, const float* sin_t, const float* cos_t, int T,
                 int H, int dh, int rotary_dim, int max_pos, hipStream_t s) {
    const int half = rotary_dim / 2;
    const long n = (long)T * H * half;
    const int grid = (int)((n + 255) / 256);
    if (dtype == DT_BF16)
        hipLaunchKernelGGL(rope_kernel<bf16_t>, dim3(grid), dim3(256), 0, s, (bf16_t*)qk, ld, k_off, pos, sin_t, cos_t, T, H, dh, half, max_pos);
    else if (dtype == DT_F16)
        hipLaunchKernelGGL(rope_kernel<f16_t>, dim3(grid), dim3(256), 0, s, (f16_t*)qk, ld, k_off, pos, sin_t, cos_t, T, H, dh, half, max_pos);
    else
        hipLaunchKernelGGL(rope_kernel<float>, dim3(grid), dim3(256), 0, s, (float*)qk, ld, k_off, pos, sin_t, cos_t, T, H, dh, half, max_pos);
}

void launch_rope_half(void* qk, int dtype, long ld, long k_off, const int* pos, const float* sin_t, const float* cos_t, int T,
                      int H, int H_kv, int dh, int max_pos, hipStream_t s) {
    const long n = (long)T * (H + H_kv) * (dh / 8);
    const int grid = (int)((n + 255) / 256);
    if (dtype == DT_BF16)
        hipLaunchKernelGGL(rope_half_kernel<bf16_t>, dim3(grid), dim3(256), 0, s, (bf16_t*)qk, ld, k_off, pos, sin_t, cos_t, T, H, H_kv, dh, max_pos);
    else if (dtype == DT_F16)
        hipLaunchKernelGGL(rope_half_kernel<f16_t>, dim3(grid), dim3(256), 0, s, (f16_t*)qk, ld, k_off, pos, sin_t, cos_t, T, H, H_kv, dh, max_pos);
    else
        hipLaunchKernelGGL(rope_half_kernel<float>, dim3(grid), dim3(256), 0, s, (float*)qk, ld, k_off, pos, sin_t, cos_t, T, H, H_kv, dh, max_pos);
}

void launch_qknorm_rope_half(void* qk, int dtype, long ld, long k_off, const int* pos, const float* sin_t, const float* cos_t,
                             const float* q_g, const float* k_g, float eps, int T, int H, int H_kv, int dh, int max_pos, int* range_flag,
                             hipStream_t s) {
    const long n = (long)T * (H + H_kv) * (dh / 8);
    const int grid = (int)((n + 255) / 256);
#define SGPT_QKNORM(TT, DH)                                                                                                          \
    hipLaunchKernelGGL((qknorm_rope_half_kernel<TT, DH>), dim3(grid), dim3(256), 0, s, (TT*)qk, ld, k_off, pos, sin_t, cos_t, q_g, k_g, \
                       eps, T, H, H_kv, max_pos, range_flag)
    if (dh != 64 && dh != 128) return;
    if (dtype == DT_BF16) { if (dh == 64) SGPT_QKNORM(bf16_t, 64); else SGPT_QKNORM(bf16_t, 128); }
    else if (dtype == DT_F16) { if (dh == 64) SGPT_QKNORM(f16_t, 64); else SGPT_QKNORM(f16_t, 128); }
    else { if (dh == 64) SGPT_QKNORM(float, 64); else SGPT_QKNORM(float, 128); }
#undef SGPT_QKNORM
}

void launch_qkv_deinterleave(const float* src, float* dst, int H, int dh, long row_len, hipStream_t s) {
    hipLaunchKernelGGL(qkv_deinterleave_kernel, dim3(3 * H * dh), dim3(256), 0, s, src, dst, H, dh, row_len);
}
```

### sgpt_amd/csrc/score.hip

```cpp
#include "host.h"
#include "score_plan.h"

extern "C" {

sgpt_status sgpt_l2_normalize(sgpt_ctx* c, const float* in, int64_t n, int32_t d, void* out, int32_t out_dtype,
                              void* stream) {
    if (!c || !in || !out || n <= 0 || d <= 0) return fail(c, SGPT_ERR_INVALID, "sgpt_l2_normalize: bad arguments");
    HIPC(c, hipSetDevice(c->device));
    launch_l2norm(in, n, d, out, out_dtype, (hipStream_t)stream);
    HIPC(c, hipGetLastError());
    return SGPT_OK;
}

sgpt_status sgpt_pairwise_scores(sgpt_ctx* c, const float* a, const float* b, int64_t n, int32_t d, int32_t cosine, float* out,
                                 void* stream) {
    if (!c || !a || !b || !out || n <= 0 || d <= 0) return fail(c, SGPT_ERR_INVALID, "sgpt_pairwise_scores: bad arguments");
    HIPC(c, hipSetDevice(c->device));
    launch_pairwise(a, b, n, d, cosine != 0, out, (hipStream_t)stream);
    HIPC(c, hipGetLastError());
    return SGPT_OK;
}

static sgpt_status check_score_dims(sgpt_ctx* c, int dtype, int d) {
    if (dtype != SGPT_F32 && dtype != SGPT_BF16 && dtype != SGPT_F16) return fail(c, SGPT_ERR_INVALID, "score: bad dtype");
// ... 63 lines not shown
    const void *q, *qpad;
    int nq, d, k; long idx_base;
    float* sc;
    float* tv[2]; int64_t* ti[2];
    float* sav_v; int64_t* sav_i;
};

static void score_tile(const ScoreRun& r, long c0, long nc, long ld, const int* pred, long row_stride = 1, bool sample = false) {
    GemmArgs g{};
    g.A = r.q; g.lda = r.d; g.M = r.nq; g.m_valid = r.nq; g.K = r.d; g.pred = pred;
    g.W = (const char*)r.cp.base + (size_t)c0 * r.cp.rowb; g.ldw = r.cp.ldw1 * row_stride; g.N = (int)nc;
    g.out = r.sc; g.ldo = ld;
    if (r.p.any_n) { corpus_gemm(r.c, r.cp, EPI_SCORE, g, c0, row_stride, sample, r.s); return; }
    const long na = r.p.fast ? nc / 256 * 256 : 0;
    const bool fold = r.p.tile_folds(na, nc, ld, row_stride, r.d);
    if (na > 0) {
        GemmArgs h = g;
        h.A = r.qpad; h.M = r.p.nq_pad; h.N = (int)(fold ? na + 256 : na); h.n_valid = fold ? (int)nc : 0;
        corpus_gemm(r.c, r.cp, EPI_SCORE, h, c0, row_stride, false, r.s);
    }
    if (na < nc && !fold) {
        g.W = (const char*)r.cp.base + (size_t)(c0 + na) * r.cp.rowb; g.N = (int)(nc - na); g.out = r.sc + na;
        corpus_gemm(r.c, r.cp, EPI_SCORE, g, c0 + na, 1, false, r.s);
    }
}

static sgpt_status classic(const ScoreRun& r, long lo, long hi, const float* pv, const int64_t* pi, int have, float* fin_v, int64_t* fin_i,
                           const int* pred) {
    sgpt_ctx* c = r.c;
    const long chunk = r.p.chunk;
    const int nq = r.nq, k = r.k;
    int cur = (pv == r.tv[0]) ? 1 : 0;
    for (long c0 = lo; c0 < hi; c0 += chunk) {
        const long nc = (hi - c0) < chunk ? (hi - c0) : chunk;
        score_tile(r, c0, nc, chunk, pred);
        const bool last = c0 + nc >= hi;
        if (last && pv == fin_v) {
            launch_topk_select(r.sc, chunk, nc, r.idx_base + c0, pv, pi, have, k, nq, k, 0, nullptr, r.tv[cur], r.ti[cur], r.s, pred);
            HIPC(c, hipMemcpyAsync(fin_v, r.tv[cur], (size_t)nq * k * 4, hipMemcpyDeviceToDevice, r.s));
            HIPC(c, hipMemcpyAsync(fin_i, r.ti[cur], (size_t)nq * k * 8, hipMemcpyDeviceToDevice, r.s));
        } else {
            launch_topk_select(r.sc, chunk, nc, r.idx_base + c0, pv, pi, have, k, nq, k, 0, nullptr,
                               last ? fin_v : r.tv[cur], last ? fin_i : r.ti[cur], r.s, pred);
        }
        pv = r.tv[cur]; pi = r.ti[cur];
        have = k;
        cur ^= 1;
    }
    return SGPT_OK;
}

static void recompute(const ScoreRun& r, long lo, long hi, const float* pv, const int64_t* pi, float* fin_v, int64_t* fin_i, const int* pred) {
    const long fchunk = r.p.fchunk;
    const long P = (hi - lo + fchunk - 1) / fchunk;
    for (long pc = 0; pc < P; ++pc) {
        const long c0 = lo + pc * fchunk, nc = (hi - c0) < fchunk ? (hi - c0) : fchunk;
        const bool to_fin = (P - 1 - pc) % 2 == 0;
        float* dv = to_fin ? fin_v : r.sav_v;
        int64_t* di = to_fin ? fin_i : r.sav_i;
        score_tile(r, c0, nc, fchunk, pred);
        launch_topk_select(r.sc, fchunk, nc, r.idx_base + c0, pv, pi, r.k, r.k, r.nq, r.k, 0, nullptr, dv, di, r.s, pred);
        pv = dv; pi = di;
    }
}

static inline int32_t list_fill(int32_t n_run, int64_t N, int32_t k) { const int64_t tot = (int64_t)n_run + N; return (int32_t)(tot < k ? tot : k); }

#ifndef SGPT_SAMPLE_MULT
#define SGPT_SAMPLE_MULT 1.0
#endif
#ifndef SGPT_FOLD_TAIL_SCORE
#define SGPT_FOLD_TAIL_SCORE 1
#endif
#ifndef SGPT_FOLD_TAIL
#define SGPT_FOLD_TAIL 1
#endif
#ifndef SGPT_SAMPLE_TOP2
#define SGPT_SAMPLE_TOP2 1
#endif
#ifndef SGPT_CAP_SHORT
#define SGPT_CAP_SHORT 512
#endif

static sgpt_status score_topk_impl(sgpt_ctx* c, const void* q, const Corpus& cp, int32_t nq, int64_t N, int32_t k, int64_t idx_base,
                                   const float* in_val, const int64_t* in_idx, float* run_val, int64_t* run_idx, int32_t n_run,
                                   int32_t* n_out, void* stream, const int* pred_all) {
    const int d = cp.d;
    if (!c || !q || !cp.base || !run_val || !run_idx || nq <= 0 || N <= 0 || k <= 0 || n_run < 0 || n_run > k)
        return fail(c, SGPT_ERR_INVALID, "sgpt_score_topk: bad arguments");
    sgpt_status st = cp.kind == SCORE_CORPUS_BITS ? SGPT_OK : check_score_dims(c, cp.dtype, d);
    if (st != SGPT_OK) return st;
    if (cp.kind == SCORE_CORPUS_BITS && (nq > 64 || d <= 0)) return fail(c, SGPT_ERR_INVALID, "score (binary corpus): at most 64 queries per pass");
    if (cp.kind == SCORE_CORPUS_FP8 && !(nq <= 64 && score64q8_shape_ok(64, 256, d, cp.base, d)))
        return fail(c, SGPT_ERR_INVALID, "score (fp8 corpus): shape not served by the streaming tile");
    HIPC(c, hipSetDevice(c->device));
    hipStream_t s = (hipStream_t)stream;
    static const ScoreSwitches sw{exp_env("SGPT_SCORE_NO64") != nullptr, exp_env("SGPT_SCORE_CLASSIC") != nullptr, exp_env("SGPT_GEMM128") != nullptr,
                                  SGPT_SAMPLE_MULT, SGPT_FOLD_TAIL != 0, SGPT_FOLD_TAIL_SCORE != 0, SGPT_SAMPLE_TOP2 != 0, SGPT_CAP_SHORT};
    ScorePlan p;
    plan_score_topk(ScorePlanIn{nq, (long)N, d, k, n_run, cp.kind, pred_all != nullptr, sw}, p);

    st = ensure(c, &c->ws2, &c->ws2_bytes, p.total);
    if (st != SGPT_OK) return st;
    if (cp.ws6_bytes) {
        st = ensure(c, &c->ws6, &c->ws6_bytes, cp.ws6_bytes);
        if (st != SGPT_OK) return st;
    }
    char* base = (char*)c->ws2;
    auto at = [&](const ScorePlan::Region& r) { return r.bytes ? base + r.off : nullptr; };
    void* qpad = p.pad_queries ? at(p.qpad) : (p.fast ? const_cast<void*>(q) : nullptr);
    const ScoreRun r{c, s, p, cp, q, qpad, nq, d, k, (long)idx_base, (float*)at(p.sc), {(float*)at(p.tv[0]), (float*)at(p.tv[1])},
                     {(int64_t*)at(p.ti[0]), (int64_t*)at(p.ti[1])}, (float*)at(p.sav_v), (int64_t*)at(p.sav_i)};
    float* const* tv = r.tv; int64_t* const* ti = r.ti;
    float* cand_v = (float*)at(p.cand_v);
    long long* cand_i = (long long*)at(p.cand_i);
    int* cand_cnt = (int*)at(p.cand_cnt);
    int* flag = p.filt ? cand_cnt + p.nq_pad : nullptr;
    float* th_v = (float*)at(p.th_v); int64_t* th_i = (int64_t*)at(p.th_i);
    float* thr_dense = (float*)at(p.thr);
    const int nq_pad = p.nq_pad;
    const long n_clear = p.filt ? (long)(nq_pad + p.n_flags) : 0;
    if (p.fast && (!p.pad_queries || (d % 8 == 0 && ((size_t)q & 15) == 0))) {
        launch_score_prep(q, qpad, p.pad_queries ? (long)nq * d * 2 : 0, p.pad_queries ? (long)nq_pad * d * 2 : 0, cand_cnt, n_clear,
                          p.fresh_list ? (long long*)ti[0] : nullptr, p.fresh_list ? (long)nq * k : 0, s);
    } else {
        if (p.pad_queries) {
            if (nq_pad > nq) HIPC(c, hipMemsetAsync((char*)qpad + (size_t)nq * d * 2, 0, (size_t)(nq_pad - nq) * d * 2, s));
            HIPC(c, hipMemcpyAsync(qpad, q, (size_t)nq * d * 2, hipMemcpyDeviceToDevice, s));
        }
        if (p.filt) HIPC(c, hipMemsetAsync(cand_cnt, 0, (size_t)n_clear * 4, s));
        if (p.fresh_list) HIPC(c, hipMemsetAsync(ti[0], 0xff, (size_t)nq * k * 8, s));
    }

    const float* bv = n_run > 0 ? in_val : nullptr;
    const int64_t* bi = n_run > 0 ? in_idx : nullptr;
    int have = n_run;
    c->filt_chunks = 0;
    if (p.filt) {
        static const bool no_fallback = exp_env("SGPT_SCORE_NOFALLBACK") != nullptr;
        int cur = 0, chunk_i = 0;
        if (p.sampled) {
            if (n_run > 0) {
                launch_topk_select(in_val, k, 0, 0, in_val, in_idx, n_run, k, nq, k, 0, nullptr, tv[0], ti[0], s);
            }
            if (p.sample_top2) {
                const long ld2 = 8 * (p.S / 256);
                GemmArgs h{};
                h.A = qpad; h.lda = d; h.M = nq_pad; h.m_valid = nq; h.K = d;
                h.W = cp.base; h.ldw = cp.ldw1 * p.s_stride; h.N = (int)p.S; h.out = r.sc; h.ldo = ld2;
                corpus_gemm(c, cp, EPI_SCORE_TOP2, h, 0, p.s_stride, true, s);
                launch_topk_select(r.sc, ld2, ld2, 0, tv[0], ti[0], k, k, nq, k, 0, nullptr, th_v, th_i, s, nullptr, thr_dense);
            } else {
                score_tile(r, 0, p.S, p.S, nullptr, p.s_stride, true);
                launch_topk_select(r.sc, p.S, p.S, 0, tv[0], ti[0], k, k, nq, k, 0, nullptr, th_v, th_i, s, nullptr, thr_dense);
            }
        } else {
            st = classic(r, 0, p.first, bv, bi, n_run, tv[0], ti[0], nullptr);
            if (st != SGPT_OK) return st;
        }
        for (const ScoreChunk& ch : p.chunks) {
            GemmArgs g{};
            g.A = qpad; g.lda = d; g.M = nq_pad; g.m_valid = nq; g.K = d;
            g.W = (const char*)cp.base + (size_t)ch.doc0 * cp.rowb; g.ldw = cp.ldw1;
            g.N = (int)(ch.fold_tail ? (p.any_n ? ch.n_valid : ch.len + 256) : ch.len); g.n_valid = (int)ch.n_valid;
            if (p.sampled) { g.thr = thr_dense; g.thr_ld = 1; }
            else { g.thr = tv[cur] + (k - 1); g.thr_ld = k; }
            g.cand_val = cand_v; g.cand_idx = cand_i; g.cand_cnt = cand_cnt; g.cand_cap = p.cap; g.idx_base = idx_base + ch.doc0;
            corpus_gemm(c, cp, EPI_SCORE_FILTER, g, ch.doc0, 1, false, s);
            g.n_valid = 0;
            long seen = ch.fold_tail ? (long)N : ch.doc0 + ch.len;
            if (ch.tail_launch) {
                g.W = (const char*)cp.base + (size_t)seen * cp.rowb; g.N = (int)(N - seen); g.idx_base = idx_base + seen;
                corpus_gemm(c, cp, EPI_SCORE_FILTER, g, seen, 1, false, s);
                seen = N;
            }
            const bool fin = seen >= N;
            int* cflag = flag + (chunk_i < p.n_flags ? chunk_i : p.n_flags - 1);
            float* ov = fin ? run_val : tv[cur ^ 1];
            int64_t* oi = fin ? run_idx : ti[cur ^ 1];
            launch_cand_merge(tv[cur], ti[cur], cand_v, (const int64_t*)cand_i, cand_cnt, p.cap, nq, k, ov, oi, cflag, s,
                              p.sampled ? thr_dense : nullptr);
            if (!no_fallback) recompute(r, ch.doc0, seen, tv[cur], ti[cur], ov, oi, cflag);
            cur ^= 1;
            ++chunk_i;
        }
        c->filt_flag_off = (size_t)((char*)flag - base); c->filt_chunks = (int)(chunk_i < p.n_flags ? (long)chunk_i : p.n_flags);
        bv = tv[cur]; bi = ti[cur]; have = k;
    }
    if (p.rest > 0) {
        st = classic(r, N - p.rest, N, bv, bi, have, run_val, run_idx, pred_all);
        if (st != SGPT_OK) return st;
    }
    if (n_out) *n_out = list_fill(n_run, N, k);
    HIPC(c, hipGetLastError());
    return SGPT_OK;
}

sgpt_status sgpt_score_topk(sgpt_ctx* c, const void* q, const void* corpus, int32_t dtype, int32_t nq, int64_t N,
                            int32_t d, int32_t k, int64_t idx_base, float* run_val, int64_t* run_idx, int32_t n_run,
                            int32_t* n_out, void* stream) {
    return score_topk_impl(c, q, corpus_rows(corpus, dtype, d), nq, N, k, idx_base, run_val, run_idx, run_val, run_idx, n_run, n_out, stream, nullptr);
}

sgpt_status sgpt_score_topk_q8(sgpt_ctx* c, const void* q, const uint8_t* codes, const float* scale, int32_t nq, int64_t N, int32_t d,
                               int32_t k, int64_t idx_base, float* run_val, int64_t* run_idx, int32_t n_run, int32_t* n_out, void* stream) {
    if (!c || !q || !codes || !scale || !run_val || !run_idx || nq <= 0 || N <= 0 || d <= 0 || d % 8 || k <= 0 || n_run < 0 || n_run > k ||
        ((size_t)q & 15) || ((size_t)codes & 3))
        return fail(c, SGPT_ERR_INVALID, "sgpt_score_topk_q8: bad arguments (d % 8 == 0, 0 <= n_run <= k, q 16-byte aligned)");
    if (nq <= 64 && score64q8_shape_ok(64, 256, d, codes, d))
        return score_topk_impl(c, q, corpus_fp8(codes, scale, d), nq, N, k, idx_base, run_val, run_idx, run_val, run_idx, n_run, n_out, stream, nullptr);
    const int64_t blk = 131072;
    HIPC(c, hipSetDevice(c->device));
    sgpt_status st = ensure(c, &c->ws6, &c->ws6_bytes, (size_t)(N < blk ? N : blk) * d * 2);
    if (st != SGPT_OK) return st;
    int32_t have = n_run;
    for (int64_t b0 = 0; b0 < N; b0 += blk) {
        const int64_t nb = N - b0 < blk ? N - b0 : blk;
        launch_fp8_dequant_rows(codes + (size_t)b0 * d, scale + b0, nb, d, c->ws6, SGPT_F16, (hipStream_t)stream);
        st = score_topk_impl(c, q, corpus_rows(c->ws6, SGPT_F16, d), nq, nb, k, idx_base + b0, run_val, run_idx, run_val, run_idx, have, &have, stream, nullptr);
        if (st != SGPT_OK) return st;
    }
    if (n_out) *n_out = have;
    return SGPT_OK;
}

struct TwoStage {
    char *head, *tail;
    float* lv; int64_t* li;
    float* cv; int64_t* ci;
    int ldc;
};
static sgpt_status two_stage_carve(sgpt_ctx* c, size_t head_b, size_t tail_b, int nq, int kp, int k, TwoStage& t) {
    t.ldc = kp + k;
    const size_t lv_b = align_up((size_t)nq * kp * 4, 256), li_b = align_up((size_t)nq * kp * 8, 256);
    const size_t cv_b = align_up((size_t)nq * t.ldc * 4, 256), ci_b = align_up((size_t)nq * t.ldc * 8, 256);
    sgpt_status st = ensure(c, &c->ws4, &c->ws4_bytes, head_b + lv_b + li_b + cv_b + ci_b + tail_b);
    if (st != SGPT_OK) return st;
    char* b = (char*)c->ws4;
    t.head = b; b += head_b;
    t.lv = (float*)b; b += lv_b;
    t.li = (int64_t*)b; b += li_b;
    t.cv = (float*)b; b += cv_b;
    t.ci = (int64_t*)b; b += ci_b;
    t.tail = b;
    return SGPT_OK;
}
static void two_stage_finish(const TwoStage& t, float* run_val, int64_t* run_idx, int k, int n_run, int nq, int kp, hipStream_t s) {
    launch_list_append(run_val, run_idx, k, n_run, nq, t.cv, t.ci, t.ldc, kp, s);
    launch_topk_select(t.cv, t.ldc, 0, 0, t.cv, t.ci, kp + n_run, t.ldc, nq, k, 0, nullptr, run_val, run_idx, s);
}

sgpt_status sgpt_score_topk_bits(sgpt_ctx* c, const float* q, const uint8_t* bits, int64_t ldb, int32_t nq, int64_t N, int32_t d, int32_t k,
                                 int32_t kp, int32_t mode, const uint8_t* codes, const float* scale, int64_t idx_base, float* run_val,
                                 int64_t* run_idx, int32_t n_run, int32_t* n_out, void* stream) {
    if (!c || !q || !bits || !run_val || !run_idx || nq <= 0 || N <= 0 || d <= 0 || ldb % 4 || ldb < 4 * (((int64_t)d + 31) / 32) ||
        k <= 0 || kp < k || kp > 1024 || mode < 0 || mode > 2 || (mode == 0 && kp != k) || (mode == 2 && (!codes || !scale)) ||
        n_run < 0 || n_run > k || ((size_t)bits & 3))
        return fail(c, SGPT_ERR_INVALID, "sgpt_score_topk_bits: bad arguments (ldb % 4 == 0, ldb >= 4 ceil(d / 32), 0 < k <= kp <= 1024, "
                                         "mode 0 with kp == k, mode 2 with codes and scale, 0 <= n_run <= k)");
    HIPC(c, hipSetDevice(c->device));
    hipStream_t s = (hipStream_t)stream;
    const int qw = (d + 127) / 128 * 4;
    TwoStage t;
    sgpt_status st = two_stage_carve(c, align_up((size_t)nq * qw * 4, 256), 0, nq, kp, k, t);
    if (st != SGPT_OK) return st;
    uint32_t* qbits = (uint32_t*)t.head;
    launch_pack_sign_bits(q, nq, d, nullptr, (uint8_t*)qbits, (long)qw * 4, s);
    const int64_t blk = (int64_t)1 << 30;
    for (int32_t g0 = 0; g0 < nq; g0 += 64) {
        const int32_t gn = nq - g0 < 64 ? nq - g0 : 64;
        float* gv = t.lv + (size_t)g0 * kp;
        int64_t* gi = t.li + (size_t)g0 * kp;
        int32_t have = 0;
        for (int64_t b0 = 0; b0 < N; b0 += blk) {
            const int64_t nb = N - b0 < blk ? N - b0 : blk;
            st = score_topk_impl(c, qbits + (size_t)g0 * qw, corpus_bits(bits + (size_t)b0 * ldb, (long)ldb, qw, d), gn, nb, kp, idx_base + b0,
                                 gv, gi, gv, gi, have, &have, stream, nullptr);
            if (st != SGPT_OK) return st;
        }
    }
    launch_rescore_bits(mode, q, bits, (long)ldb, codes, ((long)d + 7) / 8 * 8, scale, t.lv, t.li, kp, nq, kp, d, idx_base, N, t.cv, t.ci, t.ldc, s);
    two_stage_finish(t, run_val, run_idx, k, n_run, nq, kp, s);
    if (n_out) *n_out = list_fill(n_run, N, k);
    HIPC(c, hipGetLastError());
    return SGPT_OK;
}

sgpt_status sgpt_pack_sign_bits(sgpt_ctx* c, const float* x, int64_t n, int32_t d, const float* center, uint8_t* bits, int64_t ldb,
                                void* stream) {
    if (!c || !x || !bits || n <= 0 || d <= 0 || ldb % 4 || ldb < 4 * (((int64_t)d + 31) / 32))
        return fail(c, SGPT_ERR_INVALID, "sgpt_pack_sign_bits: bad arguments (ldb % 4 == 0, ldb >= 4 ceil(d / 32))");
    HIPC(c, hipSetDevice(c->device));
    launch_pack_sign_bits(x, n, d, center, bits, ldb, (hipStream_t)stream);
    HIPC(c, hipGetLastError());
    return SGPT_OK;
}

sgpt_status sgpt_score_overflow_count(sgpt_ctx* c, int32_t* n_chunks, int32_t* n_overflowed, void* stream) {
    if (!c || !n_chunks || !n_overflowed) return fail(c, SGPT_ERR_INVALID, "sgpt_score_overflow_count: bad arguments");
    HIPC(c, hipSetDevice(c->device));
    *n_chunks = c->filt_chunks; *n_overflowed = 0;
    if (c->ws2 && c->filt_chunks > 0) {
        std::vector<int> f(c->filt_chunks);
        HIPC(c, hipMemcpyAsync(f.data(), (const char*)c->ws2 + c->filt_flag_off, (size_t)c->filt_chunks * 4, hipMemcpyDeviceToHost, (hipStream_t)stream));
        HIPC(c, hipStreamSynchronize((hipStream_t)stream));
        for (int v : f) *n_overflowed += v != 0;
    }
    return SGPT_OK;
}

sgpt_status sgpt_score_topk_refined(sgpt_ctx* c, const float* q, const float* corpus32, const void* corpus16, int32_t dtype16,
                                    int32_t nq, int64_t N, int32_t d, int32_t k, int64_t idx_base, float margin,
                                    float* run_val, int64_t* run_idx, int32_t n_run, int32_t* n_out, int32_t* fallback_flag_out,
                                    void* stream) {
    if (!c || !q || !corpus32 || !corpus16 || !run_val || !run_idx || nq <= 0 || N <= 0 || k <= 0 || n_run < 0 || n_run > k ||
        !(margin > 0.f) || (dtype16 != SGPT_F16 && dtype16 != SGPT_BF16) || d % 8)
        return fail(c, SGPT_ERR_INVALID, "sgpt_score_topk_refined: bad arguments (16-bit stage-1 rows, d % 8 == 0, margin > 0)");
    HIPC(c, hipSetDevice(c->device));
    hipStream_t s = (hipStream_t)stream;
    const Corpus rows32 = corpus_rows(corpus32, SGPT_F32, d);
    int kp = k <= 56 ? 64 : k + (k / 8 > 8 ? k / 8 : 8);
    if (kp > 1024 && k <= 1024) kp = 1024;
    if ((int64_t)kp > N) kp = (int)N;
    if (kp <= k || kp > 1024) {
        if (fallback_flag_out) *fallback_flag_out = -1;
        return score_topk_impl(c, q, rows32, nq, N, k, idx_base, run_val, run_idx, run_val, run_idx, n_run, n_out, stream, nullptr);
    }
    const size_t sv_b = align_up((size_t)nq * k * 4, 256), si_b = align_up((size_t)nq * k * 8, 256);
    TwoStage t;
    sgpt_status st = two_stage_carve(c, align_up((size_t)nq * d * 2, 256), sv_b + si_b + 256, nq, kp, k, t);
    if (st != SGPT_OK) return st;
    void* q16 = t.head;
    float* sv = (float*)t.tail;
    int64_t* si = (int64_t*)(t.tail + sv_b);
    int* flag = (int*)(t.tail + sv_b + si_b);
    HIPC(c, hipMemsetAsync(flag, 0, 4, s));
    launch_f32_to_16(q, (int64_t)nq * d, q16, dtype16, s);
    int32_t n1 = 0;
    st = score_topk_impl(c, q16, corpus_rows(corpus16, dtype16, d), nq, N, kp, idx_base, t.lv, t.li, t.lv, t.li, 0, &n1, stream, nullptr);
    if (st != SGPT_OK) return st;
    launch_refine_check(t.lv, k, kp, margin, nq, flag, s);
    if (n_run > 0) {
        HIPC(c, hipMemcpy2DAsync(sv, (size_t)k * 4, run_val, (size_t)k * 4, (size_t)n_run * 4, nq, hipMemcpyDeviceToDevice, s));
        HIPC(c, hipMemcpy2DAsync(si, (size_t)k * 8, run_idx, (size_t)k * 8, (size_t)n_run * 8, nq, hipMemcpyDeviceToDevice, s));
    }
    launch_rescore(q, corpus32, t.li, kp, nq, kp, d, idx_base, N, t.cv, t.ci, t.ldc, s);
    two_stage_finish(t, run_val, run_idx, k, n_run, nq, kp, s);
    st = score_topk_impl(c, q, rows32, nq, N, k, idx_base, sv, si, run_val, run_idx, n_run, nullptr, stream, flag);
    if (st != SGPT_OK) return st;
    if (fallback_flag_out) {
        HIPC(c, hipMemcpyAsync(fallback_flag_out, flag, 4, hipMemcpyDeviceToHost, s));
        HIPC(c, hipStreamSynchronize(s));
    }
    if (n_out) *n_out = list_fill(n_run, N, k);
    HIPC(c, hipGetLastError());
    return SGPT_OK;
}

sgpt_status sgpt_topk_merge(sgpt_ctx* c, const float* val, const int64_t* idx, int32_t nq, int32_t mcand, int32_t k,
                            const int64_t* exclude_idx, float* out_val, int64_t* out_idx, void* stream) {
    if (!c || !val || !idx || !out_val || !out_idx || nq <= 0 || mcand <= 0 || k <= 0)
        return fail(c, SGPT_ERR_INVALID, "sgpt_topk_merge: bad arguments");
    HIPC(c, hipSetDevice(c->device));
    launch_topk_select(val, mcand, 0, 0, val, idx, mcand, mcand, nq, k, 0, exclude_idx, out_val, out_idx,
                       (hipStream_t)stream);
    HIPC(c, hipGetLastError());
    return SGPT_OK;
}

sgpt_status sgpt_topk(sgpt_ctx* c, const float* scores, int32_t nq, int64_t n, int64_t ld, int32_t k, int64_t idx_base,
                      float* out_val, int64_t* out_idx, void* stream) {
    if (!c || !scores || !out_val || !out_idx || nq <= 0 || n <= 0 || ld < n || k <= 0)
        return fail(c, SGPT_ERR_INVALID, "sgpt_topk: bad arguments");
    HIPC(c, hipSetDevice(c->device));
    launch_topk_select(scores, ld, n, idx_base, nullptr, nullptr, 0, 0, nq, k, 1, nullptr, out_val, out_idx,
                       (hipStream_t)stream);
    HIPC(c, hipGetLastError());
    return SGPT_OK;
}

}
```

### sgpt_amd/csrc/topk.hip

```cpp
#include <cstdlib>

#include "common.h"

namespace {

__device__ __forceinline__ uint32_t f2key(float f) {
    const uint32_t u = __float_as_uint(f);
    return (u & 0x80000000u) ? ~u : (u | 0x80000000u);
}
__device__ __forceinline__ uint32_t f2key_order(float f) { return f2key(f + 0.0f); }

constexpr int TK_THREADS = 256;
constexpr int TK_SORT_MAX = 2048;
constexpr int TK_FAST_KMAX = 64;
constexpr int TK_MERGE_KMAX = 1024;
constexpr long TK_FAST_MIN_ROW = 4096;

struct Row {
    const float* sc; long n; long idx_base;
    const float* pv; const int64_t* pi; int n_prev; int nan_to_m1; int64_t excl;
    int gk; long gstride;
    __device__ __forceinline__ long total() const { return n + n_prev; }
    __device__ __forceinline__ long paddr(long j) const { return gk > 0 ? (j / gk) * gstride + (j % gk) : j; }
    __device__ __forceinline__ float val(long i) const {
        const bool isp = i >= n;
        const long j = isp ? i - n : 0;
        float v;
        if (isp) {
            const long a = paddr(j);
            const int64_t id = pi[a];
            v = (id < 0 || id == excl) ? -INFINITY : pv[a];
        } else {
            v = sc[i];
        }
        if (nan_to_m1 && v != v) v = -1.0f;
        return v;
    }
    __device__ __forceinline__ int64_t idx(long i) const {
        if (i < n) return idx_base + i;
        const int64_t id = pi[paddr(i - n)];
        return id == excl ? -1 : id;
    }
};

__device__ __forceinline__ bool is_score(float v) { return v > -INFINITY || v != v; }
__device__ __forceinline__ int64_t out_id(float v, int64_t id) { return is_score(v) ? id : (int64_t)-1; }

__device__ __forceinline__ bool sorts_before(float va, int64_t ia, float vb, int64_t ib) {
    const uint32_t ka = f2key(va + 0.0f), kb = f2key(vb + 0.0f);
    return ka > kb || (ka == kb && ia < ib);
}

template <int CTRL>
__device__ __forceinline__ void argmax_step_dpp(float& bv, int64_t& bi, int& bp) {
    const float ov = __uint_as_float((unsigned)__builtin_amdgcn_update_dpp(0, (int)__float_as_uint(bv), CTRL, 0xf, 0xf, false));
    const unsigned lo = (unsigned)__builtin_amdgcn_update_dpp(0, (int)(unsigned)((unsigned long long)bi & 0xffffffffull), CTRL, 0xf, 0xf, false);
    const unsigned hi = (unsigned)__builtin_amdgcn_update_dpp(0, (int)(unsigned)((unsigned long long)bi >> 32), CTRL, 0xf, 0xf, false);
    const int op = __builtin_amdgcn_update_dpp(0, bp, CTRL, 0xf, 0xf, false);
    const int64_t oi = (int64_t)(((unsigned long long)hi << 32) | lo);
    if (op >= 0 && (bp < 0 || sorts_before(ov, oi, bv, bi))) { bv = ov; bi = oi; bp = op; }
}
template <bool ROW32>
__device__ __forceinline__ void argmax_step_rows(float& bv, int64_t& bi, int& bp) {
    auto other = [](unsigned x) -> unsigned {
        const auto r = ROW32 ? __builtin_amdgcn_permlane32_swap(x, x, false, false) : __builtin_amdgcn_permlane16_swap(x, x, false, false);
        const unsigned lane = __builtin_amdgcn_mbcnt_hi(~0u, __builtin_amdgcn_mbcnt_lo(~0u, 0u));
        const bool upper = ROW32 ? (lane & 32u) != 0 : (lane & 16u) != 0;
        return upper ? r[0] : r[1];
    };
    const float ov = __uint_as_float(other(__float_as_uint(bv)));
    const unsigned lo = other((unsigned)((unsigned long long)bi & 0xffffffffull));
    const unsigned hi = other((unsigned)((unsigned long long)bi >> 32));
    const int op = (int)other((unsigned)bp);
    const int64_t oi = (int64_t)(((unsigned long long)hi << 32) | lo);
    if (op >= 0 && (bp < 0 || sorts_before(ov, oi, bv, bi))) { bv = ov; bi = oi; bp = op; }
}
__device__ __forceinline__ void wave_argmax(float& bv, int64_t& bi, int& bp) {
    argmax_step_dpp<0xB1>(bv, bi, bp);
    argmax_step_dpp<0x4E>(bv, bi, bp);
    argmax_step_dpp<0x141>(bv, bi, bp);
    argmax_step_dpp<0x140>(bv, bi, bp);
    argmax_step_rows<false>(bv, bi, bp);
    argmax_step_rows<true>(bv, bi, bp);
}

// ... 389 lines not shown
                                                               int* __restrict__ overflow, float* __restrict__ thr_io) {
    __shared__ float s_val[TK_SORT_MAX];
    __shared__ int64_t s_idx[TK_SORT_MAX];
    __shared__ float r_val[TK_MERGE_KMAX];
    __shared__ int64_t r_idx[TK_MERGE_KMAX];
    const int q = blockIdx.x, t = threadIdx.x;
    const int raw = cand_cnt[q];
    const int cnt = raw < cap ? raw : cap;
    int np2 = 1;
    while (np2 < cnt) np2 <<= 1;
    for (int i = t; i < np2; i += TK_THREADS) {
        const bool ok = i < cnt;
        s_val[i] = ok ? cand_val[(long)q * cap + i] : -INFINITY;
        s_idx[i] = ok ? cand_idx[(long)q * cap + i] : 0x7fffffffffffffffLL;
    }
    int nrun = 0;
    for (int i = t; i < k; i += TK_THREADS) {
        const int64_t id = run_idx[(long)q * k + i];
        r_val[i] = id >= 0 ? run_val[(long)q * k + i] : -INFINITY;
        r_idx[i] = id >= 0 ? id : 0x7fffffffffffffffLL;
    }
    __syncthreads();
    if (t == 0) {
        cand_cnt[q] = 0;
        if (raw > cap) atomicOr(overflow, 1);
    }
    const float* cv = s_val;
    const int64_t* ci = s_idx;
    int ccnt = cnt;
    if (k <= TK_FAST_KMAX && cnt > 2 * k) {
        float* tv_ = r_val + TK_MERGE_KMAX / 2;
        int64_t* ti_ = r_idx + TK_MERGE_KMAX / 2;
        const bool keys_ok = idx_fit_keys(s_idx, cnt, t, TK_THREADS);
        if (t < 64 && keys_ok) {
            wave_topk_keys_any(s_val, s_idx, cnt, k, t, [&](int round, float bv, int64_t bi, bool valid) {
                tv_[round] = valid ? bv : -INFINITY; ti_[round] = valid ? bi : 0x7fffffffffffffffLL;
            });
        } else if (t < 64) {
            for (int round = 0; round < k; ++round) {
                float bv = -INFINITY; int64_t bi = 0x7fffffffffffffffLL; int bp = -1;
                for (int c0 = t; c0 < cnt; c0 += 64) {
                    const float v = s_val[c0]; const int64_t id = s_idx[c0];
                    if (sorts_before(v, id, bv, bi)) { bv = v; bi = id; bp = c0; }
                }
                wave_argmax(bv, bi, bp);
                if (t == 0) { tv_[round] = bv; ti_[round] = bi; if (bp >= 0) { s_val[bp] = -INFINITY; s_idx[bp] = 0x7fffffffffffffffLL; } }
            }
        }
        __syncthreads();
        cv = tv_; ci = ti_; ccnt = k;
    } else if (cnt > 1) {
        bitonic_desc<true>(s_val, s_idx, np2, t);
    }
    nrun = count_before(r_val, r_idx, k, -INFINITY, 0x7fffffffffffffffLL);
    const int total = nrun + ccnt;
    for (int i = t; i < nrun; i += TK_THREADS) {
        const int pos = i + count_before(cv, ci, ccnt, r_val[i], r_idx[i]);
        if (pos < k) { out_val[(long)q * k + pos] = r_val[i]; out_idx[(long)q * k + pos] = r_idx[i]; }
        if (pos == k - 1 && thr_io != nullptr && r_val[i] > thr_io[q]) thr_io[q] = r_val[i];
    }
    for (int j = t; j < ccnt; j += TK_THREADS) {
        const int pos = j + count_before(r_val, r_idx, nrun, cv[j], ci[j]);
        if (pos < k) { out_val[(long)q * k + pos] = cv[j]; out_idx[(long)q * k + pos] = ci[j]; }
        if (pos == k - 1 && thr_io != nullptr && cv[j] > thr_io[q]) thr_io[q] = cv[j];
    }
    for (int i = total + t; i < k; i += TK_THREADS) { out_val[(long)q * k + i] = -INFINITY; out_idx[(long)q * k + i] = -1; }
}

__global__ __launch_bounds__(256) void thr_below_kernel(const float* __restrict__ list, int k, int nq, float* __restrict__ thr) {
    const int q = blockIdx.x * 256 + threadIdx.x;
    if (q >= nq) return;
    thr[q] = thr_below(list[(long)q * k + (k - 1)]);
}

__global__ __launch_bounds__(256) void score_prep_kernel(const uint4* __restrict__ q, uint4* __restrict__ qpad, long q_vec, long qpad_vec,
                                                         int* __restrict__ counters, long n_counters, long long* __restrict__ idx_list,
                                                         long n_idx) {
    const long stride = (long)gridDim.x * 256;
    for (long i = (long)blockIdx.x * 256 + threadIdx.x; i < qpad_vec; i += stride) qpad[i] = i < q_vec ? q[i] : make_uint4(0, 0, 0, 0);
    for (long i = (long)blockIdx.x * 256 + threadIdx.x; i < n_counters; i += stride) counters[i] = 0;
    for (long i = (long)blockIdx.x * 256 + threadIdx.x; i < n_idx; i += stride) idx_list[i] = -1;
}

__global__ __launch_bounds__(256) void rescore_kernel(const float* __restrict__ q, const float* __restrict__ corpus,
                                                      const int64_t* __restrict__ idx, long ld_idx, int m, int d, long idx_base,
                                                      long n_docs, float* __restrict__ out_val, int64_t* __restrict__ out_idx, long ld_out) {
    const int j = blockIdx.x * 4 + (threadIdx.x >> 6), qi = blockIdx.y, lane = threadIdx.x & 63;
    if (j >= m) return;
    const int64_t id = idx[(long)qi * ld_idx + j];
    const long row = (long)(id - idx_base);
    float v = -INFINITY;
    if (id >= 0 && row >= 0 && row < n_docs) {
        const float4* a = reinterpret_cast<const float4*>(q + (long)qi * d);
        const float4* b = reinterpret_cast<const float4*>(corpus + row * d);
        float acc = 0.f;
        for (int c = lane; c < d / 4; c += 64) {
            const float4 x = a[c], y = b[c];
            acc = __builtin_fmaf(x.x, y.x, acc); acc = __builtin_fmaf(x.y, y.y, acc);
            acc = __builtin_fmaf(x.z, y.z, acc); acc = __builtin_fmaf(x.w, y.w, acc);
        }
#pragma unroll
        for (int o = 32; o > 0; o >>= 1) acc += __shfl_xor(acc, o, 64);
        v = acc != acc ? -1.0f : acc;
    }
    if (lane == 0) {
        out_val[(long)qi * ld_out + j] = v;
        out_idx[(long)qi * ld_out + j] = v > -INFINITY ? id : (int64_t)-1;
    }
}

template <int MODE>
__global__ __launch_bounds__(256) void rescore_bits_kernel(const float* __restrict__ q, const uint8_t* __restrict__ rows, long ld_rows,
                                                           const float* __restrict__ scale, const int64_t* __restrict__ idx, long ld_idx,
                                                           int m, int d, long idx_base, long n_docs, float* __restrict__ out_val,
                                                           int64_t* __restrict__ out_idx, long ld_out) {
    const int j = blockIdx.x * 4 + (threadIdx.x >> 6), qi = blockIdx.y, lane = threadIdx.x & 63;
    if (j >= m) return;
    const int64_t id = idx[(long)qi * ld_idx + j];
    const long row = (long)(id - idx_base);
    float v = -INFINITY;
    if (id >= 0 && row >= 0 && row < n_docs) {
        const float* a = q + (long)qi * d;
        const uint8_t* b = rows + row * ld_rows;
        float acc = 0.f;
        for (int i = lane; i < d; i += 64) {
            if constexpr (MODE == 1) {
                const bool pos = (b[i >> 3] >> (7 - (i & 7))) & 1;
                acc += pos ? a[i] : -a[i];
            } else {
                acc = __builtin_fmaf(a[i], __builtin_amdgcn_cvt_f32_fp8((int)b[i], 0), acc);
            }
        }
#pragma unroll
        for (int o = 32; o > 0; o >>= 1) acc += __shfl_xor(acc, o, 64);
        if constexpr (MODE == 1) acc = acc / sqrtf((float)d);
        else acc *= scale[row];
        v = acc != acc ? -1.0f : acc;
    }
    if (lane == 0) {
        out_val[(long)qi * ld_out + j] = v;
        out_idx[(long)qi * ld_out + j] = v > -INFINITY ? id : (int64_t)-1;
    }
}

__global__ __launch_bounds__(256) void agreement_div_kernel(const float* __restrict__ val1, const int64_t* __restrict__ idx, long ld_idx,
                                                            int nq, int m, int d, float* __restrict__ out_val,
                                                            int64_t* __restrict__ out_idx, long ld_out) {
    const long i = (long)blockIdx.x * 256 + threadIdx.x;
    if (i >= (long)nq * m) return;
    const long qi = i / m, j = i - qi * m;
    const int64_t id = idx[qi * ld_idx + j];
    out_val[qi * ld_out + j] = id >= 0 ? __fdiv_rn(val1[qi * ld_idx + j], (float)d) : -INFINITY;
    out_idx[qi * ld_out + j] = id >= 0 ? id : (int64_t)-1;
}

__global__ __launch_bounds__(256) void refine_check_kernel(const float* __restrict__ v16, int k, int kp, float margin, int nq,
                                                           int* __restrict__ flag) {
    const int qi = blockIdx.x * 256 + threadIdx.x;
    if (qi >= nq) return;
    const float t = v16[(long)qi * kp + (k - 1)], u = v16[(long)qi * kp + (kp - 1)];
    if (u > -INFINITY && !(u < t - margin)) atomicOr(flag, 1);
}

__global__ __launch_bounds__(256) void list_append_kernel(const float* __restrict__ in_val, const int64_t* __restrict__ in_idx, long ld_in,
                                                          int n_run, int nq, float* __restrict__ out_val, int64_t* __restrict__ out_idx,
                                                          long ld_out, int col0) {
    const long i = (long)blockIdx.x * 256 + threadIdx.x;
    if (i >= (long)nq * n_run) return;
    const long qi = i / n_run, j = i - qi * n_run;
    out_val[qi * ld_out + col0 + j] = in_val[qi * ld_in + j];
    out_idx[qi * ld_out + col0 + j] = in_idx[qi * ld_in + j];
}

}

void launch_rescore(const float* q, const float* corpus, const int64_t* idx, long ld_idx, int nq, int m, int d, long idx_base,
                    long n_docs, float* out_val, int64_t* out_idx, long ld_out, hipStream_t s) {
    hipLaunchKernelGGL(rescore_kernel, dim3((m + 3) / 4, nq), dim3(256), 0, s, q, corpus, idx, ld_idx, m, d, idx_base, n_docs,
                       out_val, out_idx, ld_out);
}

void launch_rescore_bits(int mode, const float* q, const uint8_t* bits, long ldb, const uint8_t* codes, long ld8, const float* scale,
                         const float* val1, const int64_t* idx, long ld_idx, int nq, int m, int d, long idx_base, long n_docs,
                         float* out_val, int64_t* out_idx, long ld_out, hipStream_t s) {
    if (mode == 0)
        hipLaunchKernelGGL(agreement_div_kernel, dim3((unsigned)(((long)nq * m + 255) / 256)), dim3(256), 0, s, val1, idx, ld_idx, nq, m, d,
                           out_val, out_idx, ld_out);
    else if (mode == 1)
        hipLaunchKernelGGL(rescore_bits_kernel<1>, dim3((m + 3) / 4, nq), dim3(256), 0, s, q, bits, ldb, (const float*)nullptr, idx, ld_idx,
                           m, d, idx_base, n_docs, out_val, out_idx, ld_out);
    else
        hipLaunchKernelGGL(rescore_bits_kernel<2>, dim3((m + 3) / 4, nq), dim3(256), 0, s, q, codes, ld8, scale, idx, ld_idx, m, d,
                           idx_base, n_docs, out_val, out_idx, ld_out);
}

void launch_refine_check(const float* v16, int k, int kp, float margin, int nq, int* flag, hipStream_t s) {
    hipLaunchKernelGGL(refine_check_kernel, dim3((nq + 255) / 256), dim3(256), 0, s, v16, k, kp, margin, nq, flag);
}

void launch_list_append(const float* in_val, const int64_t* in_idx, long ld_in, int n_run, int nq, float* out_val, int64_t* out_idx,
                        long ld_out, int col0, hipStream_t s) {
    if (n_run <= 0) return;
    hipLaunchKernelGGL(list_append_kernel, dim3((unsigned)(((long)nq * n_run + 255) / 256)), dim3(256), 0, s, in_val, in_idx, ld_in,
                       n_run, nq, out_val, out_idx, ld_out, col0);
}

void launch_score_prep(const void* q, void* qpad, long q_bytes, long qpad_bytes, int* counters, long n_counters, long long* idx_list,
                       long n_idx, hipStream_t s) {
    long work = qpad_bytes / 16;
    if (n_counters > work) work = n_counters;
    if (n_idx > work) work = n_idx;
    const long blocks = (work + 255) / 256;
    hipLaunchKernelGGL(score_prep_kernel, dim3((unsigned)(blocks < 1 ? 1 : (blocks > 2048 ? 2048 : blocks))), dim3(256), 0, s,
                       (const uint4*)q, (uint4*)qpad, q_bytes / 16, qpad_bytes / 16, counters, n_counters, idx_list, n_idx);
}

void launch_thr_below(const float* list, int k, int nq, float* thr, hipStream_t s) {
    hipLaunchKernelGGL(thr_below_kernel, dim3((nq + 255) / 256), dim3(256), 0, s, list, k, nq, thr);
}

void launch_topk_select(const float* scores, long ld, long n, long idx_base, const float* prev_val,
                        const int64_t* prev_idx, int n_prev, long prev_ld, int nq, int k, int nan_to_m1,
                        const int64_t* exclude_idx, float* out_val, int64_t* out_idx, hipStream_t s, const int* pred,
                        float* thr_out, int gather_k) {
    hipLaunchKernelGGL(topk_select_kernel, dim3(nq), dim3(TK_THREADS), 0, s, scores, ld, n, idx_base, prev_val,
                       prev_idx, n_prev, prev_ld, k, nan_to_m1, exclude_idx, out_val, out_idx, pred, thr_out, gather_k, nq);
}

void launch_cand_merge(const float* run_val, const int64_t* run_idx, const float* cand_val, const int64_t* cand_idx,
                       int* cand_cnt, int cap, int nq, int k, float* out_val, int64_t* out_idx, int* overflow,
                       hipStream_t s, float* thr_io) {
    hipLaunchKernelGGL(cand_merge_kernel, dim3(nq), dim3(TK_THREADS), 0, s, run_val, run_idx, cand_val, cand_idx, cand_cnt,
                       cap, k, out_val, out_idx, overflow, thr_io);
}
```

### sgpt_amd/runtime.py

```python
import ctypes as C
from dataclasses import dataclass
from typing import Optional, Tuple

import numpy as np
import torch

from . import _lib
from ._lib import SGPT_BF16, SGPT_F16, SGPT_F32, POOL_MODES

DT_CODE = {torch.float32: SGPT_F32, torch.bfloat16: SGPT_BF16, torch.float16: SGPT_F16}


def _stream_ptr(device) -> C.c_void_p:
    return C.c_void_p(torch.cuda.current_stream(device).cuda_stream)


def _p(t: Optional[torch.Tensor]) -> C.c_void_p:
    return C.c_void_p(0 if t is None else t.data_ptr())


@dataclass
class QuantizedCorpus:
    codes: torch.Tensor
    scale: torch.Tensor
# ... 95 lines not shown
        out = torch.empty((B, d), dtype=torch.float32, device=self.device)
        dt = DT_CODE[hidden.dtype]
        if mode == "learntmean":
            if position_weights is None or position_weights.numel() < S:
                raise ValueError("learntmean needs position_weights covering the sequence length")
            pw = position_weights.to(device=self.device, dtype=torch.float32).contiguous()
            self._chk(self.lib.sgpt_pool_learnt(self.handle, _p(hidden), dt, _p(m), B, S, d, _p(pw), _p(out),
                                                _stream_ptr(self.device)), "sgpt_pool_learnt")
            return out
        self._chk(self.lib.sgpt_pool(self.handle, _p(hidden), dt, _p(m), B, S, d, POOL_MODES[mode], _p(out),
                                     _stream_ptr(self.device)), "sgpt_pool")
        return out

    def l2_normalize(self, x: torch.Tensor, out_dtype=torch.float32) -> torch.Tensor:
        x = self._dev_f32(x)
        n, d = x.shape
        out = torch.empty((n, d), dtype=out_dtype, device=self.device)
        self._chk(self.lib.sgpt_l2_normalize(self.handle, _p(x), n, d, _p(out), DT_CODE[out_dtype],
                                             _stream_ptr(self.device)), "sgpt_l2_normalize")
        return out

    def pairwise_scores(self, a: torch.Tensor, b: torch.Tensor, cosine: bool) -> torch.Tensor:
        a, b = self._dev_f32(a), self._dev_f32(b)
        if a.shape != b.shape or a.dim() != 2:
            raise ValueError(f"pairwise scores need two [n, d] matrices of one shape, got {tuple(a.shape)} and {tuple(b.shape)}")
        n, d = a.shape
        out = torch.empty((n,), dtype=torch.float32, device=self.device)
        if n:
            self._chk(self.lib.sgpt_pairwise_scores(self.handle, _p(a), _p(b), n, d, 1 if cosine else 0, _p(out),
                                                    _stream_ptr(self.device)), "sgpt_pairwise_scores")
        return out

    def to_16(self, x: torch.Tensor, dtype=torch.float16, out: Optional[torch.Tensor] = None) -> torch.Tensor:
        x = x.to(device=self.device, dtype=torch.float32).contiguous()
        if out is None:
            out = torch.empty(x.shape, dtype=dtype, device=self.device)
        self._chk(self.lib.sgpt_f32_to_16(self.handle, _p(x), x.numel(), _p(out), DT_CODE[dtype],
                                          _stream_ptr(self.device)), "sgpt_f32_to_16")
        return out

    def row_crest(self, x: torch.Tensor) -> float:
        if x.dtype not in (torch.float16, torch.bfloat16):
            x = self.to_16(self._dev_f32(x), torch.float16)
        x = x.to(self.device).contiguous()
        n, d = x.shape
        out = C.c_float(0)
        self._chk(self.lib.sgpt_row_crest(self.handle, _p(x), DT_CODE[x.dtype], n, d, d, C.byref(out),
                                          _stream_ptr(self.device)), "sgpt_row_crest")
        return float(out.value)

    def split16(self, x: torch.Tensor, role: str, dtype=torch.float16) -> torch.Tensor:
        if role not in ("doc", "query"):
            raise ValueError("role must be 'doc' or 'query'")
        x = self._dev_f32(x)
        n, d = x.shape
        out = torch.empty((n, 3 * d), dtype=dtype, device=self.device)
        self._chk(self.lib.sgpt_split16(self.handle, _p(x), n, d, 0 if role == "doc" else 1, _p(out), DT_CODE[dtype],
                                        _stream_ptr(self.device)), "sgpt_split16")
        return out

    def to_bf16(self, x: torch.Tensor) -> torch.Tensor:
        return self.to_16(x, torch.bfloat16)

    def range_check(self, reset: bool = True) -> int:
        flagged = C.c_int32(0)
        self._chk(self.lib.sgpt_range_check(self.handle, C.byref(flagged), 1 if reset else 0, _stream_ptr(self.device)),
                  "sgpt_range_check")
        return int(flagged.value)

    def generation(self) -> int:
        return int(self.lib.sgpt_ctx_generation(self.handle))

    def set_low_latency(self, on: bool) -> bool:
        return bool(self.lib.sgpt_ctx_set_low_latency(self.handle, 1 if on else 0))

    def set_gemm_cu_cap(self, n: int) -> int:
        return int(self.lib.sgpt_ctx_set_gemm_cu_cap(self.handle, int(n)))

    def set_tile_policy(self, force_256) -> int:
        return int(self.lib.sgpt_ctx_set_tile_policy(self.handle, int(force_256)))

    def set_query_tile(self, k: int) -> int:
        return int(self.lib.sgpt_ctx_set_query_tile(self.handle, int(k)))

    def reserve(self, encode_bytes: int = 0, score_bytes: int = 0) -> None:
        self._chk(self.lib.sgpt_ctx_reserve(self.handle, encode_bytes, score_bytes), "sgpt_ctx_reserve")

    def fp8_quantize_rows(self, w: torch.Tensor) -> Tuple[torch.Tensor, torch.Tensor]:
        w = w.to(device=self.device, dtype=torch.float32).contiguous()
        rows, cols = w.shape
        codes = torch.empty((rows, cols), dtype=torch.uint8, device=self.device)
        scale = torch.empty((rows,), dtype=torch.float32, device=self.device)
        self._chk(self.lib.sgpt_fp8_quantize_rows(self.handle, _p(w), rows, cols, _p(codes), _p(scale),
                                                  _stream_ptr(self.device)), "sgpt_fp8_quantize_rows")
        return codes, scale

    def fp8_dequantize_rows(self, codes: torch.Tensor, scale: torch.Tensor, out_dtype=torch.float32) -> torch.Tensor:
        codes = codes.to(device=self.device, dtype=torch.uint8).contiguous()
        scale = scale.to(device=self.device, dtype=torch.float32).contiguous()
        rows, cols = codes.shape
        out = torch.empty((rows, cols), dtype=out_dtype, device=self.device)
        self._chk(self.lib.sgpt_fp8_dequantize_rows(self.handle, _p(codes), _p(scale), rows, cols, _p(out),
                                                    DT_CODE[out_dtype],
                                                    _stream_ptr(self.device)), "sgpt_fp8_dequantize_rows")
        return out

    def quantize_corpus(self, emb, normalize: bool = True, block_rows: int = 65536) -> QuantizedCorpus:
        if not isinstance(emb, torch.Tensor):
            emb = torch.as_tensor(np.asarray(emb))
        if emb.dim() != 2 or emb.shape[0] == 0 or emb.shape[1] == 0:
            raise ValueError(f"quantize_corpus needs a non-empty [N, d] matrix, got {tuple(emb.shape)}")
        N, d0 = emb.shape
        d = (d0 + 7) // 8 * 8
        codes = torch.empty((N, d), dtype=torch.uint8, device=self.device)
        scale = torch.empty((N,), dtype=torch.float32, device=self.device)
        for r0 in range(0, N, block_rows):
            n = min(block_rows, N - r0)
            blk = self._dev_f32(emb[r0:r0 + n])
            if normalize:
                blk = self.l2_normalize(blk)
            if d != d0:
                blk = torch.nn.functional.pad(blk, (0, d - d0))
            self._chk(self.lib.sgpt_fp8_quantize_rows(self.handle, _p(blk), n, d, _p(codes[r0:r0 + n]), _p(scale[r0:r0 + n]),
                                                      _stream_ptr(self.device)), "sgpt_fp8_quantize_rows")
        return QuantizedCorpus(codes, scale, bool(normalize), d0)

    def pack_sign_bits(self, x, center: Optional[torch.Tensor] = None, out: Optional[torch.Tensor] = None) -> torch.Tensor:
        x = self._dev_f32(x)
        n, d = x.shape
        if n == 0 or d == 0:
            raise ValueError(f"pack_sign_bits needs a non-empty [n, d] matrix, got {tuple(x.shape)}")
        ldb = 4 * ((d + 31) // 32)
        if center is not None:
            center = center.to(device=self.device, dtype=torch.float32).contiguous()
            if tuple(center.shape) != (d,):
                raise ValueError(f"pack_sign_bits: center must be [{d}], got {tuple(center.shape)}")
        if out is None:
            out = torch.empty((n, ldb), dtype=torch.uint8, device=self.device)
        elif (out.dtype != torch.uint8 or tuple(out.shape) != (n, ldb) or out.device != self.device or not out.is_contiguous()):
            raise ValueError(f"pack_sign_bits: out must be a contiguous uint8 [{n}, {ldb}] tensor on {self.device}, got {out.dtype} "
                             f"{tuple(out.shape)} on {out.device}")
        self._chk(self.lib.sgpt_pack_sign_bits(self.handle, _p(x), n, d, _p(center), _p(out), ldb, _stream_ptr(self.device)),
                  "sgpt_pack_sign_bits")
        return out

    def binarize_corpus(self, emb, normalize: bool = True, center=None, keep_fp8: bool = False,
                        block_rows: int = 65536) -> BinaryCorpus:
        if keep_fp8 and center is not None:
            raise ValueError("binarize_corpus: keep_fp8 with a centre is refused -- fp8 re-scoring needs the raw query, the centred bits "
                             "q - center, and the search call takes one query matrix (score_topk)")
        if not normalize:
            raise ValueError("binarize_corpus: normalize=False is refused -- sign bits carry no norms, the search is a cosine search")
        if not isinstance(emb, torch.Tensor):
            emb = torch.as_tensor(np.asarray(emb))
        if emb.dim() != 2 or emb.shape[0] == 0 or emb.shape[1] == 0:
            raise ValueError(f"binarize_corpus needs a non-empty [N, d] matrix, got {tuple(emb.shape)}")
        N, d = emb.shape
        if isinstance(center, str):
            if center != "mean":
                raise ValueError(f"binarize_corpus: center must be None, 'mean' or a [d] tensor, got {center!r}")
            acc = torch.zeros((d,), dtype=torch.float64, device=self.device)
            for r0 in range(0, N, block_rows):
                acc += self.l2_normalize(self._dev_f32(emb[r0:r0 + block_rows])).sum(dim=0, dtype=torch.float64)
            center = (acc / N).to(torch.float32)
        elif center is not None:
            center = torch.as_tensor(center).to(device=self.device, dtype=torch.float32).contiguous()
# ... 239 lines not shown
            if mode not in POOL_MODES:
                raise ValueError(f"unknown pooling mode {mode}")
            B, d = seq_len.numel(), x.shape[1]
            pw = self._f32c(position_weights)
            n_w = (0 if pw is None else pw.numel()) if n_weights is None else int(n_weights)
            out = torch.empty((B, d), dtype=torch.float32, device=self.device)
            self._chk(self.lib.sgpt_lnf_pool_ex(self.handle, _p(x), _p(self._f32c(rms[0])), None, _p(seq_off), _p(seq_len), _p(pad_left), B, d,
                                                float(rms[1]), 1, POOL_MODES[mode], 1 if normalize else 0, _p(pw), n_w, _p(out),
                                                _p(nonfinite_flag), 1, _stream_ptr(self.device)), "sgpt_lnf_pool_ex")
            return out
        if mode not in POOL_MODES:
            raise ValueError(f"unknown pooling mode {mode}")
        B, d = seq_len.numel(), x.shape[1]
        g, b, eps = (self._f32c(ln[0]), self._f32c(ln[1]), float(ln[2])) if ln is not None else (None, None, 0.0)
        pw = self._f32c(position_weights)
        n_w = (0 if pw is None else pw.numel()) if n_weights is None else int(n_weights)
        out = torch.empty((B, d), dtype=torch.float32, device=self.device)
        self._chk(self.lib.sgpt_lnf_pool(self.handle, _p(x), _p(g), _p(b), _p(seq_off), _p(seq_len), _p(pad_left), B, d, eps,
                                         0 if ln is None else 1, POOL_MODES[mode], 1 if normalize else 0, _p(pw), n_w, _p(out),
                                         _p(nonfinite_flag), _stream_ptr(self.device)), "sgpt_lnf_pool")
        return out

    def rope(self, buf: torch.Tensor, pos: torch.Tensor, sin: torch.Tensor, cos: torch.Tensor, H: int, head_dim: int,
             rotary_dim: int, k_off: int, T: Optional[int] = None, max_pos: Optional[int] = None) -> torch.Tensor:
        if buf.dtype not in DT_CODE or buf.stride(1) != 1:
            raise ValueError("rope: buf is fp32, bf16 or f16 with a unit column stride")
        if sin.stride() != (rotary_dim // 2, 1) or cos.stride() != (rotary_dim // 2, 1):
            raise ValueError("rope: sin / cos are row-contiguous [max_pos, rotary_dim / 2]")
        self._chk(self.lib.sgpt_rope(self.handle, _p(buf), DT_CODE[buf.dtype], buf.stride(0), int(k_off), _p(pos), _p(sin), _p(cos),
                                     buf.shape[0] if T is None else int(T), H, head_dim, rotary_dim,
                                     sin.shape[0] if max_pos is None else int(max_pos), _stream_ptr(self.device)), "sgpt_rope")
        return buf

    def logprob_rows(self, logits: torch.Tensor, targets: torch.Tensor, V: Optional[int] = None, greedy: bool = True):
        if logits.dtype != torch.float32 or logits.stride(1) != 1:
            raise ValueError("logprob_rows: logits are fp32 rows with a unit column stride")
        n = logits.shape[0]
        lp = torch.empty((n,), dtype=torch.float32, device=self.device)
        am = torch.empty((n,), dtype=torch.int32, device=self.device) if greedy else None
        self._chk(self.lib.sgpt_logprob_rows(self.handle, _p(logits), logits.stride(0), logits.shape[1] if V is None else int(V),
                                             _p(targets), n, _p(lp), _p(am), _stream_ptr(self.device)), "sgpt_logprob_rows")
        return lp, am

    def layernorm_fp8(self, x: torch.Tensor, gamma: torch.Tensor, beta: torch.Tensor, eps: float = 1e-5):
        x = x.to(device=self.device, dtype=torch.float32).contiguous()
        T, d = x.shape
        codes = torch.empty((T, d), dtype=torch.uint8, device=self.device)
        scale = torch.empty((T,), dtype=torch.float32, device=self.device)
        g = gamma.to(device=self.device, dtype=torch.float32).contiguous()
        b = beta.to(device=self.device, dtype=torch.float32).contiguous()
        self._chk(self.lib.sgpt_layernorm_fp8(self.handle, _p(x), _p(g), _p(b), T, d, eps, _p(codes), _p(scale),
                                              _stream_ptr(self.device)), "sgpt_layernorm_fp8")
        return codes, scale

    def linear_fp8(self, a8: torch.Tensor, w8: torch.Tensor, w_scale: torch.Tensor, bias: torch.Tensor, epi: str,
                   a_scale: Optional[torch.Tensor] = None, a_scalar: float = 1.0, resid: Optional[torch.Tensor] = None,
                   out_scale: float = 1.0, out_dtype=None) -> torch.Tensor:
        M, K = a8.shape
        N = w8.shape[0]
        code = {"store": 0, "gelu": 1, "resid": 2, "vt": 4}[epi]
        odt = {"gelu": torch.uint8, "resid": torch.float32}.get(epi, out_dtype if out_dtype is not None else torch.bfloat16)
        out = torch.empty((N, M) if epi == "vt" else (M, N), dtype=odt, device=self.device)
        r = None if resid is None else resid.to(device=self.device, dtype=torch.float32).contiguous()
        b = None if bias is None else bias.contiguous()
        self._chk(self.lib.sgpt_linear_fp8(self.handle, code, DT_CODE.get(odt, 0), _p(a8.contiguous()), _p(a_scale), a_scalar,
                                           _p(w8.contiguous()), _p(w_scale.contiguous()), _p(b), _p(r), _p(out),
                                           out_scale, M, N, K, _stream_ptr(self.device)), "sgpt_linear_fp8")
        return out

    def scores(self, a: torch.Tensor, b: torch.Tensor, dtype=torch.float32) -> torch.Tensor:
        a, b = self._operand(a, dtype), self._operand(b, dtype)
        na, d = a.shape
        nb, d2 = b.shape
        if d != d2:
            raise ValueError(f"embedding dims differ: {d} vs {d2}")
        ldo = (nb + 3) // 4 * 4
        out = torch.empty((na, ldo), dtype=torch.float32, device=self.device)
        self._chk(self.lib.sgpt_scores(self.handle, _p(a), _p(b), DT_CODE[dtype],
                                       na, nb, d, _p(out), ldo, _stream_ptr(self.device)), "sgpt_scores")
        return out[:, :nb]

    def score_topk(self, q: torch.Tensor, corpus: torch.Tensor, k: int, idx_base: int = 0,
                   run: Optional[Tuple[torch.Tensor, torch.Tensor, int]] = None,
                   dtype=None, rescore: str = "sign", rescore_multiplier=4) -> Tuple[torch.Tensor, torch.Tensor, int]:
        if isinstance(corpus, BinaryCorpus):
            return self._score_topk_bits(q, corpus, k, idx_base, run, rescore, rescore_multiplier)
        if rescore != "sign" or rescore_multiplier != 4:
            raise ValueError("score_topk: rescore / rescore_multiplier apply to a BinaryCorpus only")
        if isinstance(corpus, QuantizedCorpus):
            if dtype not in (None, torch.float16):
                raise ValueError(f"a QuantizedCorpus is scored with f16 queries: dtype must be None or torch.float16, got {dtype}")
            if q.shape[1] != corpus.codes.shape[1] and q.shape[1] == corpus.dim:
                q = torch.nn.functional.pad(q, (0, corpus.codes.shape[1] - q.shape[1]))
            q = self._operand(q, torch.float16)
            codes = corpus.codes.to(self.device).contiguous()
            scale = corpus.scale.to(device=self.device, dtype=torch.float32).contiguous()
            nq, d = q.shape
            N, d2 = codes.shape
            if d != d2:
                raise ValueError(f"embedding dims differ: {d} vs {d2}")
            if run is None:
                val = torch.empty((nq, k), dtype=torch.float32, device=self.device)
                idx = torch.empty((nq, k), dtype=torch.int64, device=self.device)
                n_run = 0
            else:
                val, idx, n_run = run
            n_out = C.c_int32(0)
            self._chk(self.lib.sgpt_score_topk_q8(self.handle, _p(q), _p(codes), _p(scale), nq, N, d, k, idx_base, _p(val), _p(idx),
                                                  n_run, C.byref(n_out), _stream_ptr(self.device)), "sgpt_score_topk_q8")
            return val, idx, int(n_out.value)
        if dtype is None:
            dtype = corpus.dtype if corpus.dtype in DT_CODE else torch.float32
        q, corpus = self._operand(q, dtype), self._operand(corpus, dtype)
        nq, d = q.shape
        N, d2 = corpus.shape
        if d != d2:
            raise ValueError(f"embedding dims differ: {d} vs {d2}")
        if run is None:
            val = torch.empty((nq, k), dtype=torch.float32, device=self.device)
            idx = torch.empty((nq, k), dtype=torch.int64, device=self.device)
            n_run = 0
        else:
            val, idx, n_run = run
        n_out = C.c_int32(0)
        self._chk(self.lib.sgpt_score_topk(self.handle, _p(q), _p(corpus), DT_CODE[dtype], nq, N, d, k,
                                           idx_base, _p(val), _p(idx), n_run, C.byref(n_out),
                                           _stream_ptr(self.device)), "sgpt_score_topk")
        return val, idx, int(n_out.value)

    REFINE_MARGIN_UNIT_F16 = 2.5e-3

    def score_topk_refined(self, q: torch.Tensor, corpus32: torch.Tensor, corpus16: Optional[torch.Tensor], k: int,
                           idx_base: int = 0, run: Optional[Tuple[torch.Tensor, torch.Tensor, int]] = None,
                           margin: Optional[float] = None, report: bool = False):
        q = q.to(device=self.device, dtype=torch.float32).contiguous()
        corpus32 = corpus32.to(device=self.device, dtype=torch.float32).contiguous()
        if corpus16 is None:
            corpus16 = self.to_16(corpus32, torch.float16)
        if corpus16.dtype not in (torch.float16, torch.bfloat16) or corpus16.shape != corpus32.shape or not corpus16.is_contiguous():
            raise ValueError("corpus16 must be the contiguous 16-bit rounding of corpus32")
        if margin is None:
            if corpus16.dtype != torch.float16:
                raise ValueError("the default margin is the bound for IEEE-half copies of unit rows: pass margin= for bf16 copies")
            margin = self.REFINE_MARGIN_UNIT_F16
        nq, d = q.shape
        N = corpus32.shape[0]
        if run is None:
            val = torch.empty((nq, k), dtype=torch.float32, device=self.device)
            idx = torch.empty((nq, k), dtype=torch.int64, device=self.device)
            n_run = 0
        else:
            val, idx, n_run = run
        n_out, fb = C.c_int32(0), C.c_int32(0)
        self._chk(self.lib.sgpt_score_topk_refined(self.handle, _p(q), _p(corpus32), _p(corpus16), DT_CODE[corpus16.dtype], nq, N, d, k,
                                                   idx_base, float(margin), _p(val), _p(idx), n_run, C.byref(n_out),
                                                   C.byref(fb) if report else None, _stream_ptr(self.device)), "sgpt_score_topk_refined")
        return (val, idx, int(n_out.value), int(fb.value)) if report else (val, idx, int(n_out.value))

    def topk_merge(self, val: torch.Tensor, idx: torch.Tensor, k: int,
                   exclude_idx: Optional[torch.Tensor] = None) -> Tuple[torch.Tensor, torch.Tensor]:
        val = val.to(device=self.device, dtype=torch.float32).contiguous()
        idx = idx.to(device=self.device, dtype=torch.int64).contiguous()
        nq, m = val.shape
        ov = torch.empty((nq, k), dtype=torch.float32, device=self.device)
        oi = torch.empty((nq, k), dtype=torch.int64, device=self.device)
        ex = None if exclude_idx is None else exclude_idx.to(device=self.device, dtype=torch.int64).contiguous()
        self._chk(self.lib.sgpt_topk_merge(self.handle, _p(val), _p(idx), nq, m, k, _p(ex), _p(ov), _p(oi),
                                           _stream_ptr(self.device)), "sgpt_topk_merge")
        return ov, oi

    def fold_gathered_topk(self, gathered_val: torch.Tensor, gathered_idx: torch.Tensor, k_out: int,
                           exclude_idx: Optional[torch.Tensor] = None) -> Tuple[torch.Tensor, torch.Tensor]:
        gv = gathered_val.to(device=self.device, dtype=torch.float32).contiguous()
        gi = gathered_idx.to(device=self.device, dtype=torch.int64).contiguous()
        world, nq, k = gv.shape
        ov = torch.empty((nq, k_out), dtype=torch.float32, device=self.device)
        oi = torch.empty((nq, k_out), dtype=torch.int64, device=self.device)
        ex = None if exclude_idx is None else exclude_idx.to(device=self.device, dtype=torch.int64).contiguous()
        self._chk(self.lib.sgpt_fold_gathered_topk(self.handle, _p(gv), _p(gi), world, nq, k, k_out, _p(ex), _p(ov), _p(oi),
                                                   _stream_ptr(self.device)), "sgpt_fold_gathered_topk")
        return ov, oi

    def topk(self, scores: torch.Tensor, k: int, idx_base: int = 0) -> Tuple[torch.Tensor, torch.Tensor]:
        scores = scores.to(device=self.device, dtype=torch.float32)
        if scores.stride(1) != 1:
            scores = scores.contiguous()
        nq, n = scores.shape
        ov = torch.empty((nq, k), dtype=torch.float32, device=self.device)
        oi = torch.empty((nq, k), dtype=torch.int64, device=self.device)
        self._chk(self.lib.sgpt_topk(self.handle, _p(scores), nq, n, scores.stride(0), k, idx_base, _p(ov), _p(oi),
                                     _stream_ptr(self.device)), "sgpt_topk")
        return ov, oi

    def eval_ranked(self, idx: torch.Tensor, val: Optional[torch.Tensor], qrel_off, qrel_pos, qrel_rel, ideal_rel, k_values,
                    check_order: bool = True) -> dict:
        idx = idx.to(device=self.device, dtype=torch.int64).contiguous()
        nq, K = idx.shape
        if val is not None:
            val = val.to(device=self.device, dtype=torch.float32).contiguous()
            if val.shape != idx.shape:
                raise ValueError(f"eval_ranked: val {tuple(val.shape)} and idx {tuple(idx.shape)} differ in shape")
        i32 = lambda a: torch.as_tensor(np.ascontiguousarray(a, dtype=np.int32)).to(self.device) if not isinstance(a, torch.Tensor) \
            else a.to(device=self.device, dtype=torch.int32).contiguous()
        off, rel, ideal = i32(qrel_off), i32(qrel_rel), i32(ideal_rel)
        pos = (qrel_pos if isinstance(qrel_pos, torch.Tensor) else torch.as_tensor(np.ascontiguousarray(qrel_pos, dtype=np.int64)))
        pos = pos.to(device=self.device, dtype=torch.int64).contiguous()
        if off.numel() != nq + 1 or not (pos.numel() == rel.numel() == ideal.numel()):
            raise ValueError("eval_ranked: qrel_off has nq + 1 entries; qrel_pos, qrel_rel and ideal_rel have one length")
        if pos.numel() == 0:
            pos, rel, ideal = (torch.zeros((1,), dtype=t.dtype, device=self.device) for t in (pos, rel, ideal))
# ... 97 lines not shown
```

Before: 38940.

## Add certified two-stage f16 prefilter with fp32 rescore for exact fp32 top-k scoring

Exact fp32 score_topk can now take a two-stage path by default. Each super-chunk of the corpus is converted to f16 together with per-row norm statistics, a wider candidate list is selected with the f16 scorer, and those candidates are rescored in fp32. A per-query error bound checks whether the f16 ranking can be trusted; queries that fail are gathered and rerun with brute-force fp32, or the whole chunk is when too many fail or the f16 conversion overflows. The aim is to replace the full fp32 scoring pass with a cheaper f16 one, at the cost of a conversion pass, extra kernels, a 768 MB workspace and a more complex fallback path. The rescore kernel is also rewritten as a one-thread-per-candidate chain.

```diff
diff --git a/__graft_entry__.py b/__graft_entry__.py
--- a/__graft_entry__.py
+++ b/__graft_entry__.py
@@ -10,6 +10,10 @@
     from sgpt_amd import build as b
     lib = b.build(force=os.environ.get("SGPT_FORCE_BUILD") == "1", verbose=True)
     assert os.path.exists(lib)
+    import subprocess
+    subprocess.run([sys.executable, "-m", "sgpt_amd.build"] + (["--force"] if os.environ.get("SGPT_FORCE_BUILD") == "1" else []),
+                   cwd=ROOT, env={**os.environ, "SGPT_EXPERIMENTS": "1"}, check=True, stdout=subprocess.DEVNULL)
+    assert os.path.exists(os.path.join(ROOT, "sgpt_amd", "lib", "libsgpt_hip_exp.so"))
     import sgpt_amd
     from sgpt_amd import _lib
     _lib.load()
diff --git a/include/sgpt_hip.h b/include/sgpt_hip.h
--- a/include/sgpt_hip.h
+++ b/include/sgpt_hip.h
@@ -8,7 +8,7 @@
 extern "C" {
 #endif
 
-#define SGPT_ABI_VERSION 19
+#define SGPT_ABI_VERSION 20
 
 typedef int sgpt_status;
 #define SGPT_OK 0
@@ -257,6 +257,9 @@
 sgpt_status sgpt_prof_enable(sgpt_ctx* ctx, int32_t on);
 sgpt_status sgpt_prof_read(sgpt_ctx* ctx, int64_t* launches, double* ms, double* flops, int32_t reset);
 
+enum { SGPT_EXACT_AUTO = 0, SGPT_EXACT_BRUTE = 1, SGPT_EXACT_TWO_STAGE = 2 };
+int32_t sgpt_ctx_set_exact_scorer(sgpt_ctx* ctx, int32_t mode);
+sgpt_status sgpt_score_fallback_count(sgpt_ctx* ctx, int32_t* n_super_chunks, int32_t* n_queries, int32_t* n_chunk_wide, void* stream);
 int32_t sgpt_ctx_set_gemm_cu_cap(sgpt_ctx* ctx, int32_t n);
 int32_t sgpt_ctx_set_low_latency(sgpt_ctx* ctx, int32_t on);
 int32_t sgpt_ctx_set_tile_policy(sgpt_ctx* ctx, int32_t policy);
diff --git a/sgpt_amd/_lib.py b/sgpt_amd/_lib.py
--- a/sgpt_amd/_lib.py
+++ b/sgpt_amd/_lib.py
@@ -5,7 +5,7 @@
 LIB_PATH = os.environ.get("SGPT_HIP_LIB") or os.path.join(HERE, "lib", "libsgpt_hip.so")
 
 SGPT_F32, SGPT_BF16, SGPT_FP8W, SGPT_F16, SGPT_FP8M = 0, 1, 2, 3, 4
-SGPT_ABI_VERSION = 19
+SGPT_ABI_VERSION = 20
 SGPT_PREC_CLASSES = 5
 PC_LN1, PC_ATT, PC_CTX, PC_LN2, PC_H = 0, 1, 2, 3, 4
 SGPT_ERR_RANGE = -5
@@ -121,6 +121,8 @@
     "sgpt_ctx_set_tile_policy": (C.c_int32, [C.c_void_p, C.c_int32]),
     "sgpt_ctx_set_gemm_cu_cap": (C.c_int32, [C.c_void_p, C.c_int32]),
     "sgpt_ctx_set_query_tile": (C.c_int32, [C.c_void_p, C.c_int32]),
+    "sgpt_ctx_set_exact_scorer": (C.c_int32, [C.c_void_p, C.c_int32]),
+    "sgpt_score_fallback_count": (C.c_int, [C.c_void_p, C.POINTER(C.c_int32), C.POINTER(C.c_int32), C.POINTER(C.c_int32), C.c_void_p]),
     "sgpt_model_range_check": (C.c_int, [C.c_void_p, C.POINTER(C.c_int32), C.c_int32, C.c_void_p]),
     "sgpt_model_range_adapt": (C.c_int, [C.c_void_p, C.POINTER(C.c_int32), C.c_void_p]),
     "sgpt_model_get_range_shifts": (C.c_int, [C.c_void_p, C.c_void_p, C.c_int32]),
diff --git a/sgpt_amd/beir.py b/sgpt_amd/beir.py
--- a/sgpt_amd/beir.py
+++ b/sgpt_amd/beir.py
@@ -123,7 +123,7 @@
 
     def __init__(self, model, batch_size: int = 128, corpus_chunk_size: int = 50000, score_dtype=torch.float32,
                  prefetch_tokenize: bool = True, ctx=None, group=None, distributed: Optional[bool] = None,
-                 score_split: Optional[bool] = None, exact_scorer: str = "brute", **kwargs):
+                 score_split: Optional[bool] = None, exact_scorer: str = "auto", **kwargs):
         self.model = model
         self.prefetch_tokenize = prefetch_tokenize
         self.batch_size = batch_size
@@ -132,8 +132,8 @@
         self.show_progress_bar = True
         self.convert_to_tensor = True
         self.score_dtype = score_dtype
-        if exact_scorer not in ("refined", "brute"):
-            raise ValueError("exact_scorer must be 'refined' or 'brute'")
+        if exact_scorer not in ("auto", "refined", "brute"):
+            raise ValueError("exact_scorer must be 'auto', 'refined' or 'brute'")
         self.exact_scorer = exact_scorer
         self.ctx = ctx
         self.group = group
@@ -256,7 +256,13 @@
                 if refined:
                     val, idx, _ = ctx.score_topk_refined(q_op, sub, None, kk, idx_base=lo + start)
                 else:
-                    val, idx, _ = ctx.score_topk(q_op, sub, kk, idx_base=lo + start, dtype=self.score_dtype)
+                    brute = self.exact_scorer == "brute" and hasattr(ctx, "set_exact_scorer")
+                    prev = ctx.set_exact_scorer("brute") if brute else None
+                    try:
+                        val, idx, _ = ctx.score_topk(q_op, sub, kk, idx_base=lo + start, dtype=self.score_dtype)
+                    finally:
+                        if brute:
+                            ctx.set_exact_scorer(prev)
                 if run_val is None:
                     cand_v, cand_i = val, idx
                 else:
diff --git a/sgpt_amd/csrc/common.h b/sgpt_amd/csrc/common.h
--- a/sgpt_amd/csrc/common.h
+++ b/sgpt_amd/csrc/common.h
@@ -358,12 +358,20 @@
                         const int64_t* exclude_idx, float* out_val, int64_t* out_idx, hipStream_t s,
                         const int* pred = nullptr, float* thr_out = nullptr,
                         int gather_k = 0);
-void launch_rescore(const float* q, const float* corpus, const int64_t* idx, long ld_idx, int nq, int m, int d, long idx_base,
-                    long n_docs, float* out_val, int64_t* out_idx, long ld_out, hipStream_t s);
 void launch_rescore_bits(int mode, const float* q, const uint8_t* bits, long ldb, const uint8_t* codes, long ld8, const float* scale,
                          const float* val1, const int64_t* idx, long ld_idx, int nq, int m, int d, long idx_base, long n_docs,
                          float* out_val, int64_t* out_idx, long ld_out, hipStream_t s);
 void launch_refine_check(const float* v16, int k, int kp, float margin, int nq, int* flag, hipStream_t s);
+enum { TS_COUNT = 0, TS_FEW = 1, TS_ALL = 2, TS_WORDS = 4 };
+void launch_f32_to_f16_rows_stats(const float* in, long n, int d, void* out, float* row_stats, unsigned* max_stats, hipStream_t s);
+void launch_rescore_chain(const float* q, const float* corpus, const int64_t* idx, long ld_idx, int nq, int m, int d, long idx_base,
+                          long n_docs, float* out_val, int64_t* out_idx, long ld_out, hipStream_t s);
+void launch_two_stage_check(const float* v16, int k, int kp, int d, const float* qstats, const unsigned* qmax, const unsigned* dmax,
+                            int nq, int F, int* state, int* fail_idx, hipStream_t s);
+void launch_two_stage_gather(const float* q, int d, const float* sv, const int64_t* si, int k, int n_run, int F, const unsigned* qmax,
+                             const unsigned* dmax, int* state, const int* fail_idx, int* diag, float* qc, float* cv, int64_t* ci, hipStream_t s);
+void launch_two_stage_scatter(const float* cv, const int64_t* ci, int k, const int* state, const int* fail_idx, int F, float* run_val,
+                              int64_t* run_idx, hipStream_t s);
 void launch_list_append(const float* in_val, const int64_t* in_idx, long ld_in, int n_run, int nq, float* out_val, int64_t* out_idx,
                         long ld_out, int col0, hipStream_t s);
 void launch_score_prep(const void* q, void* qpad, long q_bytes, long qpad_bytes, int* counters, long n_counters, long long* idx_list,
diff --git a/sgpt_amd/csrc/ctx.h b/sgpt_amd/csrc/ctx.h
--- a/sgpt_amd/csrc/ctx.h
+++ b/sgpt_amd/csrc/ctx.h
@@ -14,6 +14,10 @@
     void* ws4 = nullptr; size_t ws4_bytes = 0;
     void* ws5 = nullptr; size_t ws5_bytes = 0;
     void* ws6 = nullptr; size_t ws6_bytes = 0;
+    void* ws7 = nullptr; size_t ws7_bytes = 0;
+    int* ts_diag = nullptr;
+    int ts_chunks = -1;
+    int exact_scorer = 0;
     size_t filt_flag_off = 0; int filt_chunks = 0;
     void* comm = nullptr;
     int comm_rank = 0, comm_world = 0;
diff --git a/sgpt_amd/csrc/ctx.hip b/sgpt_amd/csrc/ctx.hip
--- a/sgpt_amd/csrc/ctx.hip
+++ b/sgpt_amd/csrc/ctx.hip
@@ -58,6 +58,8 @@
     if (c->ws4) (void)hipFree(c->ws4);
     if (c->ws5) (void)hipFree(c->ws5);
     if (c->ws6) (void)hipFree(c->ws6);
+    if (c->ws7) (void)hipFree(c->ws7);
+    if (c->ts_diag) (void)hipFree(c->ts_diag);
     if (c->range_flag) (void)hipFree(c->range_flag);
     for (auto& e : c->ev_pool) { (void)hipEventDestroy(e.first); (void)hipEventDestroy(e.second); }
     delete c;
@@ -131,6 +133,12 @@
     c->no_qpath = policy == 2 ? 1 : 0;
     return old;
 }
+int32_t sgpt_ctx_set_exact_scorer(sgpt_ctx* c, int32_t mode) {
+    if (!c || mode < SGPT_EXACT_AUTO || mode > SGPT_EXACT_TWO_STAGE) return -1;
+    const int old = c->exact_scorer;
+    c->exact_scorer = mode;
+    return old;
+}
 int32_t sgpt_ctx_set_query_tile(sgpt_ctx* c, int32_t k) {
     if (!c || k < 0 || k > 7) return -1;
     const int old = c->qtile;
diff --git a/sgpt_amd/csrc/elementwise.hip b/sgpt_amd/csrc/elementwise.hip
--- a/sgpt_amd/csrc/elementwise.hip
+++ b/sgpt_amd/csrc/elementwise.hip
@@ -598,6 +598,54 @@
     for (long i = (long)blockIdx.x * 256 + threadIdx.x; i < numel; i += stride) out[i] = f32_to_h<H>(in[i]);
 }
 
+__global__ __launch_bounds__(256) void cvt16_rows_stats_kernel(const float* __restrict__ in, long n, int d, uint16_t* __restrict__ out,
+                                                               float* __restrict__ row_stats, unsigned* __restrict__ max_stats) {
+    const int lane = threadIdx.x & 63;
+    const long w0 = (long)blockIdx.x * 4 + (threadIdx.x >> 6), nw = (long)gridDim.x * 4;
+    unsigned m0 = 0, m1 = 0, m2 = 0, bad = 0;
+    for (long r = w0; r < n; r += nw) {
+        typedef uint32_t u32x2_t __attribute__((ext_vector_type(2)));
+        const f32x4* src = reinterpret_cast<const f32x4*>(in + r * d);
+        u32x2_t* dst = reinterpret_cast<u32x2_t*>(out + r * d);
+        const int nch = d / 4;
+        float sx = 0.f, sh = 0.f, sr = 0.f;
+        for (int c0 = lane; c0 < nch; c0 += 256) {
+            f32x4 x[4];
+#pragma unroll
+            for (int u = 0; u < 4; ++u)
+                x[u] = c0 + 64 * u < nch ? __builtin_nontemporal_load(src + c0 + 64 * u) : f32x4{0.f, 0.f, 0.f, 0.f};
+#pragma unroll
+            for (int u = 0; u < 4; ++u) {
+                const u32x2_t p = {pack_f16x2(x[u][0], x[u][1]), pack_f16x2(x[u][2], x[u][3])};
+                if (c0 + 64 * u < nch) __builtin_nontemporal_store(p, dst + c0 + 64 * u);
+                bad |= ((p[0] & 0x7c00u) == 0x7c00u) | ((p[0] & 0x7c000000u) == 0x7c000000u) | ((p[1] & 0x7c00u) == 0x7c00u) |
+                       ((p[1] & 0x7c000000u) == 0x7c000000u);
+                const float h[4] = {Half<f16_t>::lo(p[0]), Half<f16_t>::hi(p[0]), Half<f16_t>::lo(p[1]), Half<f16_t>::hi(p[1])};
+#pragma unroll
+                for (int e = 0; e < 4; ++e) {
+                    const float rr = x[u][e] - h[e];
+                    sx = __builtin_fmaf(x[u][e], x[u][e], sx); sh = __builtin_fmaf(h[e], h[e], sh); sr = __builtin_fmaf(rr, rr, sr);
+                }
+            }
+        }
+#pragma unroll
+        for (int o = 32; o > 0; o >>= 1) { sx += __shfl_xor(sx, o, 64); sh += __shfl_xor(sh, o, 64); sr += __shfl_xor(sr, o, 64); }
+        if (row_stats != nullptr && lane == 0)
+            *reinterpret_cast<float4*>(row_stats + r * 4) = make_float4(sqrtf(sx), sqrtf(sh), sqrtf(sr), 0.f);
+        const unsigned bx = __float_as_uint(sx), bh = __float_as_uint(sh), br = __float_as_uint(sr);
+        m0 = bx > m0 ? bx : m0; m1 = bh > m1 ? bh : m1; m2 = br > m2 ? br : m2;
+    }
+    if (max_stats == nullptr) return;
+#pragma unroll
+    for (int o = 32; o > 0; o >>= 1) bad |= __shfl_xor(bad, o, 64);
+    if (lane == 0) {
+        if (m0) atomicMax(max_stats + 0, m0);
+        if (m1) atomicMax(max_stats + 1, m1);
+        if (m2) atomicMax(max_stats + 2, m2);
+        if (bad) atomicOr(max_stats + 3, 1u);
+    }
+}
+
 __global__ __launch_bounds__(256) void absmax_kernel(const float* __restrict__ in, long numel, unsigned* __restrict__ out_bits) {
     const long stride = (long)gridDim.x * 256;
     unsigned m = 0;
@@ -946,6 +994,12 @@
 }
 void launch_f32_to_bf16(const float* in, long numel, void* out, hipStream_t s) { launch_f32_to_16(in, numel, out, DT_BF16, s); }
 
+void launch_f32_to_f16_rows_stats(const float* in, long n, int d, void* out, float* row_stats, unsigned* max_stats, hipStream_t s) {
+    const long blocks = (n + 3) / 4;
+    hipLaunchKernelGGL(cvt16_rows_stats_kernel, dim3((unsigned)(blocks < 4096 ? blocks : 4096)), dim3(256), 0, s, in, n, d, (uint16_t*)out,
+                       row_stats, max_stats);
+}
+
 void launch_absmax(const float* in, long numel, unsigned* out_bits, hipStream_t s) {
     hipLaunchKernelGGL(absmax_kernel, dim3(cap_grid((numel + 255) / 256)), dim3(256), 0, s, in, numel, out_bits);
 }
diff --git a/sgpt_amd/csrc/score.hip b/sgpt_amd/csrc/score.hip
--- a/sgpt_amd/csrc/score.hip
+++ b/sgpt_amd/csrc/score.hip
@@ -169,6 +169,12 @@
 #define SGPT_CAP_SHORT 512
 #endif
 
+static const ScoreSwitches& score_switches() {
+    static const ScoreSwitches sw{exp_env("SGPT_SCORE_NO64") != nullptr, exp_env("SGPT_SCORE_CLASSIC") != nullptr, exp_env("SGPT_GEMM128") != nullptr,
+                                  SGPT_SAMPLE_MULT, SGPT_FOLD_TAIL != 0, SGPT_FOLD_TAIL_SCORE != 0, SGPT_SAMPLE_TOP2 != 0, SGPT_CAP_SHORT};
+    return sw;
+}
+
 static sgpt_status score_topk_impl(sgpt_ctx* c, const void* q, const Corpus& cp, int32_t nq, int64_t N, int32_t k, int64_t idx_base,
                                    const float* in_val, const int64_t* in_idx, float* run_val, int64_t* run_idx, int32_t n_run,
                                    int32_t* n_out, void* stream, const int* pred_all) {
@@ -182,10 +188,8 @@
         return fail(c, SGPT_ERR_INVALID, "score (fp8 corpus): shape not served by the streaming tile");
     HIPC(c, hipSetDevice(c->device));
     hipStream_t s = (hipStream_t)stream;
-    static const ScoreSwitches sw{exp_env("SGPT_SCORE_NO64") != nullptr, exp_env("SGPT_SCORE_CLASSIC") != nullptr, exp_env("SGPT_GEMM128") != nullptr,
-                                  SGPT_SAMPLE_MULT, SGPT_FOLD_TAIL != 0, SGPT_FOLD_TAIL_SCORE != 0, SGPT_SAMPLE_TOP2 != 0, SGPT_CAP_SHORT};
     ScorePlan p;
-    plan_score_topk(ScorePlanIn{nq, (long)N, d, k, n_run, cp.kind, pred_all != nullptr, sw}, p);
+    plan_score_topk(ScorePlanIn{nq, (long)N, d, k, n_run, cp.kind, pred_all != nullptr, score_switches()}, p);
 
     st = ensure(c, &c->ws2, &c->ws2_bytes, p.total);
     if (st != SGPT_OK) return st;
@@ -283,9 +287,32 @@
     return SGPT_OK;
 }
 
+static int two_stage_kp(int k, int64_t N);
+static sgpt_status score_topk_f32_two_stage(sgpt_ctx* c, const float* q, const float* corpus, int32_t nq, int64_t N, int32_t d, int32_t k,
+                                            int kp, long sc_len, int64_t idx_base, float* run_val, int64_t* run_idx, int32_t n_run,
+                                            int32_t* n_out, void* stream);
+static long two_stage_super_chunk(int64_t N, int d);
+
 sgpt_status sgpt_score_topk(sgpt_ctx* c, const void* q, const void* corpus, int32_t dtype, int32_t nq, int64_t N,
                             int32_t d, int32_t k, int64_t idx_base, float* run_val, int64_t* run_idx, int32_t n_run,
                             int32_t* n_out, void* stream) {
+    if (c && dtype == SGPT_F32) {
+        c->ts_chunks = -1;
+        if (c->exact_scorer != SGPT_EXACT_BRUTE && q && corpus && run_val && run_idx && nq > 0 && N > 0 && d > 0 && d % 8 == 0 && k > 0 &&
+            n_run >= 0 && n_run <= k && (((size_t)q | (size_t)corpus) & 15) == 0) {
+            const long sc_len = two_stage_super_chunk(N, d);
+            const int kp = two_stage_kp(k, sc_len);
+            bool take = kp > k && kp <= 1024;
+            if (take && c->exact_scorer == SGPT_EXACT_AUTO) {
+                ScorePlan p;
+                plan_score_topk(ScorePlanIn{nq, sc_len, d, kp, 0, SCORE_CORPUS_16, false, score_switches()}, p);
+                take = p.filt;
+            }
+            if (take)
+                return score_topk_f32_two_stage(c, (const float*)q, (const float*)corpus, nq, N, d, k, kp, sc_len, idx_base, run_val, run_idx,
+                                                n_run, n_out, stream);
+        }
+    }
     return score_topk_impl(c, q, corpus_rows(corpus, dtype, d), nq, N, k, idx_base, run_val, run_idx, run_val, run_idx, n_run, n_out, stream, nullptr);
 }
 
@@ -431,7 +458,7 @@
         HIPC(c, hipMemcpy2DAsync(sv, (size_t)k * 4, run_val, (size_t)k * 4, (size_t)n_run * 4, nq, hipMemcpyDeviceToDevice, s));
         HIPC(c, hipMemcpy2DAsync(si, (size_t)k * 8, run_idx, (size_t)k * 8, (size_t)n_run * 8, nq, hipMemcpyDeviceToDevice, s));
     }
-    launch_rescore(q, corpus32, t.li, kp, nq, kp, d, idx_base, N, t.cv, t.ci, t.ldc, s);
+    launch_rescore_chain(q, corpus32, t.li, kp, nq, kp, d, idx_base, N, t.cv, t.ci, t.ldc, s);
     two_stage_finish(t, run_val, run_idx, k, n_run, nq, kp, s);
     st = score_topk_impl(c, q, rows32, nq, N, k, idx_base, sv, si, run_val, run_idx, n_run, nullptr, stream, flag);
     if (st != SGPT_OK) return st;
@@ -441,6 +468,129 @@
     }
     if (n_out) *n_out = list_fill(n_run, N, k);
     HIPC(c, hipGetLastError());
+    return SGPT_OK;
+}
+
+constexpr int TS_F = 128;
+#ifndef SGPT_TS_WS_BYTES
+#define SGPT_TS_WS_BYTES ((size_t)768 << 20)
+#endif
+
+static int two_stage_kp(int k, int64_t N) {
+    int kp = k <= 56 ? 64 : k + (k / 8 > 8 ? k / 8 : 8);
+    if (kp > 1024 && k <= 1024) kp = 1024;
+    if ((int64_t)kp > N) kp = (int)N;
+    return kp;
+}
+
+static long two_stage_super_chunk(int64_t N, int d) {
+    long cap_docs = (long)(SGPT_TS_WS_BYTES / ((size_t)d * 2)) / 256 * 256;
+    if (const char* e = exp_env("SGPT_TS_SUPERCHUNK")) cap_docs = atol(e) / 256 * 256;
+    if (cap_docs < 256) cap_docs = 256;
+    const int64_t n_sc = (N + cap_docs - 1) / cap_docs;
+    const int64_t len = ((N + n_sc - 1) / n_sc + 255) / 256 * 256;
+    return (long)(len < N ? len : N);
+}
+
+static sgpt_status score_topk_f32_two_stage(sgpt_ctx* c, const float* q, const float* corpus, int32_t nq, int64_t N, int32_t d, int32_t k,
+                                            int kp, long sc_len, int64_t idx_base, float* run_val, int64_t* run_idx, int32_t n_run,
+                                            int32_t* n_out, void* stream) {
+    HIPC(c, hipSetDevice(c->device));
+    hipStream_t s = (hipStream_t)stream;
+    const bool forced = c->exact_scorer == SGPT_EXACT_TWO_STAGE;
+    const long n_sc = (long)((N + sc_len - 1) / sc_len);
+    {
+        size_t need = 0;
+        ScorePlan p;
+        plan_score_topk(ScorePlanIn{nq, sc_len, d, kp, 0, SCORE_CORPUS_16, false, score_switches()}, p); need = p.total;
+        plan_score_topk(ScorePlanIn{nq, sc_len, d, k, k, SCORE_CORPUS_F32, true, score_switches()}, p); need = p.total > need ? p.total : need;
+        plan_score_topk(ScorePlanIn{TS_F, sc_len, d, k, k, SCORE_CORPUS_F32, true, score_switches()}, p); need = p.total > need ? p.total : need;
+        sgpt_status st = ensure(c, &c->ws2, &c->ws2_bytes, need);
+        if (st != SGPT_OK) return st;
+        st = ensure(c, &c->ws7, &c->ws7_bytes, (size_t)sc_len * d * 2);
+        if (st != SGPT_OK) return st;
+        if (!c->ts_diag) HIPC(c, hipMalloc((void**)&c->ts_diag, 256));
+    }
+    const size_t q16_b = align_up((size_t)nq * d * 2, 256), qs_b = align_up((size_t)nq * 16, 256);
+    const size_t sv_b = align_up((size_t)nq * k * 4, 256), si_b = align_up((size_t)nq * k * 8, 256);
+    const size_t qc_b = align_up((size_t)TS_F * d * 4, 256), fv_b = align_up((size_t)TS_F * k * 4, 256), fi_b = align_up((size_t)TS_F * k * 8, 256);
+    const size_t fl_b = align_up((size_t)TS_F * 4, 256), zero_b = align_up((size_t)(4 + n_sc * (4 + TS_WORDS)) * 4, 256);
+    TwoStage t;
+    sgpt_status st = two_stage_carve(c, q16_b + qs_b, sv_b + si_b + qc_b + 2 * (fv_b + fi_b) + fl_b + zero_b, nq, kp, k, t);
+    if (st != SGPT_OK) return st;
+    void* q16 = t.head;
+    float* qstats = (float*)(t.head + q16_b);
+    char* b = t.tail;
+    float* sv = (float*)b; b += sv_b;
+    int64_t* si = (int64_t*)b; b += si_b;
+    float* qc = (float*)b; b += qc_b;
+    float* gv = (float*)b; b += fv_b;
+    int64_t* gi = (int64_t*)b; b += fi_b;
+    float* ov = (float*)b; b += fv_b;
+    int64_t* oi = (int64_t*)b; b += fi_b;
+    int* fail_idx = (int*)b; b += fl_b;
+    unsigned* qmax = (unsigned*)b;
+    unsigned* dstats = qmax + 4;
+    int* state = (int*)(dstats + 4 * n_sc);
+    HIPC(c, hipMemsetAsync(qmax, 0, zero_b, s));
+    HIPC(c, hipMemsetAsync(c->ts_diag, 0, 8, s));
+    launch_f32_to_f16_rows_stats(q, nq, d, q16, qstats, qmax, s);
+
+    int32_t have = n_run;
+    int pieces = 0;
+    for (long i = 0; i < n_sc; ++i) {
+        const int64_t doc0 = (int64_t)i * sc_len, n = N - doc0 < sc_len ? N - doc0 : sc_len;
+        const float* rows = corpus + (size_t)doc0 * d;
+        const Corpus rows32 = corpus_rows(rows, SGPT_F32, d);
+        bool two = n > kp;
+        if (two && !forced) {
+            ScorePlan p;
+            plan_score_topk(ScorePlanIn{nq, (long)n, d, kp, 0, SCORE_CORPUS_16, false, score_switches()}, p);
+            two = p.filt;
+        }
+        if (!two) {
+            st = score_topk_impl(c, q, rows32, nq, n, k, idx_base + doc0, run_val, run_idx, run_val, run_idx, have, &have, stream, nullptr);
+            if (st != SGPT_OK) return st;
+            continue;
+        }
+        ++pieces;
+        unsigned* dmax = dstats + 4 * i;
+        int* sti = state + TS_WORDS * i;
+        launch_f32_to_f16_rows_stats(rows, n, d, c->ws7, nullptr, dmax, s);
+        int32_t n1 = 0;
+        st = score_topk_impl(c, q16, corpus_rows(c->ws7, SGPT_F16, d), nq, n, kp, idx_base + doc0, t.lv, t.li, t.lv, t.li, 0, &n1, stream, nullptr);
+        if (st != SGPT_OK) return st;
+        launch_two_stage_check(t.lv, k, kp, d, qstats, qmax, dmax, nq, TS_F, sti, fail_idx, s);
+        if (have > 0) {
+            HIPC(c, hipMemcpy2DAsync(sv, (size_t)k * 4, run_val, (size_t)k * 4, (size_t)have * 4, nq, hipMemcpyDeviceToDevice, s));
+            HIPC(c, hipMemcpy2DAsync(si, (size_t)k * 8, run_idx, (size_t)k * 8, (size_t)have * 8, nq, hipMemcpyDeviceToDevice, s));
+        }
+        launch_two_stage_gather(q, d, sv, si, k, have, TS_F, qmax, dmax, sti, fail_idx, c->ts_diag, qc, gv, gi, s);
+        launch_rescore_chain(q, rows, t.li, kp, nq, kp, d, idx_base + doc0, n, t.cv, t.ci, t.ldc, s);
+        two_stage_finish(t, run_val, run_idx, k, have, nq, kp, s);
+        st = score_topk_impl(c, qc, rows32, TS_F, n, k, idx_base + doc0, gv, gi, ov, oi, have, nullptr, stream, sti + TS_FEW);
+        if (st != SGPT_OK) return st;
+        launch_two_stage_scatter(ov, oi, k, sti, fail_idx, TS_F, run_val, run_idx, s);
+        st = score_topk_impl(c, q, rows32, nq, n, k, idx_base + doc0, sv, si, run_val, run_idx, have, nullptr, stream, sti + TS_ALL);
+        if (st != SGPT_OK) return st;
+        have = list_fill(have, n, k);
+    }
+    c->ts_chunks = pieces;
+    if (n_out) *n_out = list_fill(n_run, N, k);
+    HIPC(c, hipGetLastError());
+    return SGPT_OK;
+}
+
+sgpt_status sgpt_score_fallback_count(sgpt_ctx* c, int32_t* n_super_chunks, int32_t* n_queries, int32_t* n_chunk_wide, void* stream) {
+    if (!c || !n_super_chunks || !n_queries || !n_chunk_wide) return fail(c, SGPT_ERR_INVALID, "sgpt_score_fallback_count: bad arguments");
+    HIPC(c, hipSetDevice(c->device));
+    *n_super_chunks = c->ts_chunks; *n_queries = 0; *n_chunk_wide = 0;
+    if (c->ts_chunks > 0 && c->ts_diag) {
+        int h[2] = {0, 0};
+        HIPC(c, hipMemcpyAsync(h, c->ts_diag, 8, hipMemcpyDeviceToHost, (hipStream_t)stream));
+        HIPC(c, hipStreamSynchronize((hipStream_t)stream));
+        *n_queries = h[0]; *n_chunk_wide = h[1];
+    }
     return SGPT_OK;
 }
 
diff --git a/sgpt_amd/csrc/score_bound.h b/sgpt_amd/csrc/score_bound.h
--- /dev/null
+++ b/sgpt_amd/csrc/score_bound.h
@@ -0,0 +1,40 @@
+#pragma once
+#include <cmath>
+
+#ifndef SGPT_BOUND_FN
+#if defined(__HIPCC__) || defined(__CUDACC__)
+#define SGPT_BOUND_FN __host__ __device__ inline
+#else
+#define SGPT_BOUND_FN inline
+#endif
+#endif
+
+struct ScoreBoundIn {
+    int d;
+    float q, q16, qr;
+    float dmax, d16max, rmax;
+};
+
+SGPT_BOUND_FN float score_bound_up(float x) { return x * (1.0f + 0x1p-22f); }
+
+SGPT_BOUND_FN float score_bound_gamma(int d) {
+    const float du = (float)d * 0x1p-24f;
+    return score_bound_up(du / score_bound_up(1.0f - du) * (1.0f + 0x1p-22f));
+}
+
+SGPT_BOUND_FN float score_norm_up(float measured, int d) {
+    const float g = score_bound_gamma(d);
+    return score_bound_up(score_bound_up(measured * (1.0f + g)) + score_bound_up(sqrtf((float)d)) * 0x1p-62f);
+}
+
+SGPT_BOUND_FN float score_bound_eps(const ScoreBoundIn& b) {
+    const float g = score_bound_gamma(b.d);
+    const float conv = score_bound_up(score_bound_up(b.q16 * b.rmax) + score_bound_up(b.qr * b.dmax));
+    const float acc = score_bound_up(g * score_bound_up(score_bound_up(b.q16 * b.d16max) + score_bound_up(b.q * b.dmax)));
+    const float rd = score_bound_up(sqrtf((float)b.d));
+    const float flush = score_bound_up(0x1p-25f * score_bound_up(rd * score_bound_up(b.q16 + b.d16max)));
+    const float sub = (float)b.d * 0x1p-148f;
+    return score_bound_up(score_bound_up(conv + acc) + score_bound_up(flush + sub));
+}
+
+SGPT_BOUND_FN bool score_bound_holds(float u, float t, float eps) { return (double)u < (double)t - 2.0 * (double)eps; }
diff --git a/sgpt_amd/csrc/topk.hip b/sgpt_amd/csrc/topk.hip
--- a/sgpt_amd/csrc/topk.hip
+++ b/sgpt_amd/csrc/topk.hip
@@ -1,6 +1,7 @@
 #include <cstdlib>
 
 #include "common.h"
+#include "score_bound.h"
 
 namespace {
 
@@ -556,10 +557,10 @@
     for (long i = (long)blockIdx.x * 256 + threadIdx.x; i < n_idx; i += stride) idx_list[i] = -1;
 }
 
-__global__ __launch_bounds__(256) void rescore_kernel(const float* __restrict__ q, const float* __restrict__ corpus,
-                                                      const int64_t* __restrict__ idx, long ld_idx, int m, int d, long idx_base,
-                                                      long n_docs, float* __restrict__ out_val, int64_t* __restrict__ out_idx, long ld_out) {
-    const int j = blockIdx.x * 4 + (threadIdx.x >> 6), qi = blockIdx.y, lane = threadIdx.x & 63;
+__global__ __launch_bounds__(64) void rescore_chain_kernel(const float* __restrict__ q, const float* __restrict__ corpus,
+                                                           const int64_t* __restrict__ idx, long ld_idx, int m, int d, long idx_base,
+                                                           long n_docs, float* __restrict__ out_val, int64_t* __restrict__ out_idx, long ld_out) {
+    const int j = blockIdx.x * 64 + threadIdx.x, qi = blockIdx.y;
     if (j >= m) return;
     const int64_t id = idx[(long)qi * ld_idx + j];
     const long row = (long)(id - idx_base);
@@ -567,19 +568,82 @@
     if (id >= 0 && row >= 0 && row < n_docs) {
         const float4* a = reinterpret_cast<const float4*>(q + (long)qi * d);
         const float4* b = reinterpret_cast<const float4*>(corpus + row * d);
+        const int nch = d / 4;
         float acc = 0.f;
-        for (int c = lane; c < d / 4; c += 64) {
-            const float4 x = a[c], y = b[c];
-            acc = __builtin_fmaf(x.x, y.x, acc); acc = __builtin_fmaf(x.y, y.y, acc);
-            acc = __builtin_fmaf(x.z, y.z, acc); acc = __builtin_fmaf(x.w, y.w, acc);
-        }
-#pragma unroll
-        for (int o = 32; o > 0; o >>= 1) acc += __shfl_xor(acc, o, 64);
+        for (int c0 = 0; c0 < nch; c0 += 4) {
+            float4 x[4], y[4];
+#pragma unroll
+            for (int g = 0; g < 4; ++g) {
+                const bool ok = c0 + g < nch;
+                x[g] = ok ? a[c0 + g] : make_float4(0.f, 0.f, 0.f, 0.f);
+                y[g] = ok ? b[c0 + g] : make_float4(0.f, 0.f, 0.f, 0.f);
+            }
+#pragma unroll
+            for (int g = 0; g < 4; ++g) acc = __builtin_fmaf(x[g].x, y[g].x, acc);
+#pragma unroll
+            for (int g = 0; g < 4; ++g) acc = __builtin_fmaf(x[g].y, y[g].y, acc);
+#pragma unroll
+            for (int g = 0; g < 4; ++g) acc = __builtin_fmaf(x[g].z, y[g].z, acc);
+#pragma unroll
+            for (int g = 0; g < 4; ++g) acc = __builtin_fmaf(x[g].w, y[g].w, acc);
+        }
         v = acc != acc ? -1.0f : acc;
     }
-    if (lane == 0) {
-        out_val[(long)qi * ld_out + j] = v;
-        out_idx[(long)qi * ld_out + j] = v > -INFINITY ? id : (int64_t)-1;
+    out_val[(long)qi * ld_out + j] = v;
+    out_idx[(long)qi * ld_out + j] = v > -INFINITY ? id : (int64_t)-1;
+}
+
+__global__ __launch_bounds__(256) void two_stage_check_kernel(const float* __restrict__ v16, int k, int kp, int d, const float* __restrict__ qstats,
+                                                              const unsigned* __restrict__ qmax, const unsigned* __restrict__ dmax, int nq, int F,
+                                                              int* __restrict__ state, int* __restrict__ fail_idx) {
+    const int qi = blockIdx.x * 256 + threadIdx.x;
+    if (qi >= nq) return;
+    if ((qmax[3] | dmax[3]) != 0) return;
+    const float4 st = *reinterpret_cast<const float4*>(qstats + (long)qi * 4);
+    ScoreBoundIn b;
+    b.d = d;
+    b.q = score_norm_up(st.x, d); b.q16 = score_norm_up(st.y, d); b.qr = score_norm_up(st.z, d);
+    b.dmax = score_norm_up(sqrtf(__uint_as_float(dmax[0])), d);
+    b.d16max = score_norm_up(sqrtf(__uint_as_float(dmax[1])), d);
+    b.rmax = score_norm_up(sqrtf(__uint_as_float(dmax[2])), d);
+    const float eps = score_bound_eps(b);
+    const float t = v16[(long)qi * kp + (k - 1)], u = v16[(long)qi * kp + (kp - 1)];
+    if (u > -INFINITY && !score_bound_holds(u, t, eps)) {
+        const int pos = atomicAdd(state + TS_COUNT, 1);
+        if (pos < F) fail_idx[pos] = qi;
+    }
+}
+
+__global__ __launch_bounds__(256) void two_stage_gather_kernel(const float* __restrict__ q, int d, const float* __restrict__ sv,
+                                                               const int64_t* __restrict__ si, int k, int n_run, int F,
+                                                               const unsigned* __restrict__ qmax, const unsigned* __restrict__ dmax,
+                                                               int* __restrict__ state, const int* __restrict__ fail_idx, int* __restrict__ diag,
+                                                               float* __restrict__ qc, float* __restrict__ cv, int64_t* __restrict__ ci) {
+    const int n = state[TS_COUNT];
+    const bool bad = (qmax[3] | dmax[3]) != 0;
+    const bool few = n > 0 && n <= F && !bad, all = n > F || bad;
+    const int b = blockIdx.x;
+    if (b == 0 && threadIdx.x == 0) {
+        state[TS_FEW] = few ? 1 : 0; state[TS_ALL] = all ? 1 : 0;
+        diag[0] += bad ? 0 : n; diag[1] += all ? 1 : 0;
+    }
+    const int src = (few && b < n) ? fail_idx[b] : -1;
+    for (int i = threadIdx.x; i < d; i += 256) qc[(long)b * d + i] = src >= 0 ? q[(long)src * d + i] : 0.f;
+    for (int j = threadIdx.x; j < k; j += 256) {
+        const bool have = src >= 0 && j < n_run;
+        cv[(long)b * k + j] = have ? sv[(long)src * k + j] : -INFINITY;
+        ci[(long)b * k + j] = have ? si[(long)src * k + j] : (int64_t)-1;
+    }
+}
+
+__global__ __launch_bounds__(256) void two_stage_scatter_kernel(const float* __restrict__ cv, const int64_t* __restrict__ ci, int k,
+                                                                const int* __restrict__ state, const int* __restrict__ fail_idx,
+                                                                float* __restrict__ run_val, int64_t* __restrict__ run_idx) {
+    if (state[TS_FEW] == 0 || (int)blockIdx.x >= state[TS_COUNT]) return;
+    const int b = blockIdx.x, dst = fail_idx[b];
+    for (int j = threadIdx.x; j < k; j += 256) {
+        run_val[(long)dst * k + j] = cv[(long)b * k + j];
+        run_idx[(long)dst * k + j] = ci[(long)b * k + j];
     }
 }
 
@@ -648,10 +712,27 @@
 
 }
 
-void launch_rescore(const float* q, const float* corpus, const int64_t* idx, long ld_idx, int nq, int m, int d, long idx_base,
-                    long n_docs, float* out_val, int64_t* out_idx, long ld_out, hipStream_t s) {
-    hipLaunchKernelGGL(rescore_kernel, dim3((m + 3) / 4, nq), dim3(256), 0, s, q, corpus, idx, ld_idx, m, d, idx_base, n_docs,
+void launch_rescore_chain(const float* q, const float* corpus, const int64_t* idx, long ld_idx, int nq, int m, int d, long idx_base,
+                          long n_docs, float* out_val, int64_t* out_idx, long ld_out, hipStream_t s) {
+    hipLaunchKernelGGL(rescore_chain_kernel, dim3((m + 63) / 64, nq), dim3(64), 0, s, q, corpus, idx, ld_idx, m, d, idx_base, n_docs,
                        out_val, out_idx, ld_out);
+}
+
+void launch_two_stage_check(const float* v16, int k, int kp, int d, const float* qstats, const unsigned* qmax, const unsigned* dmax,
+                            int nq, int F, int* state, int* fail_idx, hipStream_t s) {
+    hipLaunchKernelGGL(two_stage_check_kernel, dim3((nq + 255) / 256), dim3(256), 0, s, v16, k, kp, d, qstats, qmax, dmax, nq, F, state,
+                       fail_idx);
+}
+
+void launch_two_stage_gather(const float* q, int d, const float* sv, const int64_t* si, int k, int n_run, int F, const unsigned* qmax,
+                             const unsigned* dmax, int* state, const int* fail_idx, int* diag, float* qc, float* cv, int64_t* ci, hipStream_t s) {
+    hipLaunchKernelGGL(two_stage_gather_kernel, dim3(F), dim3(256), 0, s, q, d, sv, si, k, n_run, F, qmax, dmax, state, fail_idx, diag, qc,
+                       cv, ci);
+}
+
+void launch_two_stage_scatter(const float* cv, const int64_t* ci, int k, const int* state, const int* fail_idx, int F, float* run_val,
+                              int64_t* run_idx, hipStream_t s) {
+    hipLaunchKernelGGL(two_stage_scatter_kernel, dim3(F), dim3(256), 0, s, cv, ci, k, state, fail_idx, run_val, run_idx);
 }
 
 void launch_rescore_bits(int mode, const float* q, const uint8_t* bits, long ldb, const uint8_t* codes, long ld8, const float* scale,
diff --git a/sgpt_amd/runtime.py b/sgpt_amd/runtime.py
--- a/sgpt_amd/runtime.py
+++ b/sgpt_amd/runtime.py
@@ -201,6 +201,20 @@
 
     def set_query_tile(self, k: int) -> int:
         return int(self.lib.sgpt_ctx_set_query_tile(self.handle, int(k)))
+
+    EXACT_SCORERS = {"auto": 0, "brute": 1, "two-stage": 2}
+
+    def set_exact_scorer(self, mode: str) -> str:
+        if mode not in self.EXACT_SCORERS:
+            raise ValueError(f"exact scorer must be one of {sorted(self.EXACT_SCORERS)}, got {mode!r}")
+        old = int(self.lib.sgpt_ctx_set_exact_scorer(self.handle, self.EXACT_SCORERS[mode]))
+        return next(n for n, v in self.EXACT_SCORERS.items() if v == old)
+
+    def score_fallback_count(self) -> Tuple[int, int, int]:
+        n_sc, n_q, n_all = C.c_int32(0), C.c_int32(0), C.c_int32(0)
+        self._chk(self.lib.sgpt_score_fallback_count(self.handle, C.byref(n_sc), C.byref(n_q), C.byref(n_all), _stream_ptr(self.device)),
+                  "sgpt_score_fallback_count")
+        return int(n_q.value), int(n_all.value), int(n_sc.value)
 
     def reserve(self, encode_bytes: int = 0, score_bytes: int = 0) -> None:
         self._chk(self.lib.sgpt_ctx_reserve(self.handle, encode_bytes, score_bytes), "sgpt_ctx_reserve")
@@ -606,7 +620,7 @@
 
     def score_topk(self, q: torch.Tensor, corpus: torch.Tensor, k: int, idx_base: int = 0,
                    run: Optional[Tuple[torch.Tensor, torch.Tensor, int]] = None,
-                   dtype=None, rescore: str = "sign", rescore_multiplier=4) -> Tuple[torch.Tensor, torch.Tensor, int]:
+                   dtype=None, rescore: str = "sign", rescore_multiplier=4, report: bool = False) -> Tuple[torch.Tensor, torch.Tensor, int]:
         if isinstance(corpus, BinaryCorpus):
             return self._score_topk_bits(q, corpus, k, idx_base, run, rescore, rescore_multiplier)
         if rescore != "sign" or rescore_multiplier != 4:
@@ -650,6 +664,10 @@
         self._chk(self.lib.sgpt_score_topk(self.handle, _p(q), _p(corpus), DT_CODE[dtype], nq, N, d, k,
                                            idx_base, _p(val), _p(idx), n_run, C.byref(n_out),
                                            _stream_ptr(self.device)), "sgpt_score_topk")
+        if report:
+            if dtype != torch.float32:
+                raise ValueError("score_topk: report=True belongs to fp32 rows")
+            return val, idx, int(n_out.value), self.score_fallback_count()
         return val, idx, int(n_out.value)
 
     REFINE_MARGIN_UNIT_F16 = 2.5e-3
```

After: 38950, median of 3. Within noise of the previous version (+0.0%).
